# lambdaclass/mina_bridge

Measured on AMD Instinct MI355X. Metric: Mina state proofs verified/sec (batch), higher is better.
Workload: dtype u32x8-montgomery (255-bit prime fields, integer)

## Files before the change

### bindings/go/minaverify.go

```go
package minaverify

import "C"

import (
	"errors"
	"unsafe"
)

type Ctx struct{ p *C.mina_ctx }

func lastError() error { return errors.New(C.GoString(C.mina_last_error())) }

func New(device int) (*Ctx, error) {
	var p *C.mina_ctx
	if rc := C.mina_ctx_create(C.int(device), &p); rc != 0 {
		return nil, lastError()
	}
	return &Ctx{p}, nil
}

func (c *Ctx) Close() { C.mina_ctx_destroy(c.p) }

func (c *Ctx) SrsCreate(curve int, depth uint32) error {
	if rc := C.mina_srs_create(c.p, C.int(curve), C.uint32_t(depth)); rc != 0 {
		return lastError()
	}
	return nil
}

func (c *Ctx) SetStateDedup(on bool) error {
	v := C.int(0)
	if on {
		v = 1
	}
	if rc := C.mina_ctx_set_state_dedup(c.p, v); rc != 0 {
		return lastError()
	}
	return nil
}

func (c *Ctx) StateDedupStats() (states, distinct, collisions uint64, err error) {
	var a, b, d C.uint64_t
	if rc := C.mina_ctx_state_dedup_stats(c.p, &a, &b, &d); rc != 0 {
		return 0, 0, 0, lastError()
	}
	return uint64(a), uint64(b), uint64(d), nil
}

func ConfigureDedupStates(otherFlags uint32) { C.mina_verify_configure(C.uint32_t(otherFlags) | C.MINA_VERIFY_DEDUP_STATES) }

func ConfigurePackOnDevice(otherFlags uint32) { C.mina_verify_configure(C.uint32_t(otherFlags) | C.MINA_VERIFY_PACK_ON_DEVICE) }

func ConfigureAccountOnDevice(otherFlags uint32) { C.mina_verify_configure(C.uint32_t(otherFlags) | C.MINA_VERIFY_ACCOUNT_ON_DEVICE) }

func ConfigureGroupedSearch(otherFlags uint32) { C.mina_verify_configure(C.uint32_t(otherFlags) | C.MINA_VERIFY_GROUPED_SEARCH) }

func (c *Ctx) SetSearchGroups(groups uint32) error {
	if rc := C.mina_ctx_set_search_groups(c.p, C.uint32_t(groups)); rc != 0 {
		return lastError()
	}
	return nil
}

func (c *Ctx) SearchStats() (searches, rounds, parts uint64, err error) {
	var a, b, d C.uint64_t
	if rc := C.mina_ctx_search_stats(c.p, &a, &b, &d); rc != 0 {
		return 0, 0, 0, lastError()
	}
	return uint64(a), uint64(b), uint64(d), nil
}

func (c *Ctx) StateJobEachDev(jobs *C.mina_state_jobs, dVerdicts, dFlags unsafe.Pointer) error {
	if rc := C.mina_state_job_each_dev(c.p, jobs, dVerdicts, dFlags); rc != 0 {
		return lastError()
	}
	return nil
}

func (c *Ctx) MsmSegmentsDev(curve int, nTotal, nseg int, dBegin, dEnd, dBases, dScalars, dOut unsafe.Pointer) error {
	if rc := C.mina_msm_segments_dev(c.p, C.int(curve), C.size_t(nTotal), C.size_t(nseg), dBegin, dEnd, dBases, dScalars, dOut); rc != 0 {
		return lastError()
	}
	return nil
}

func (c *Ctx) BPolyFoldSegmentsDev(field int, k uint32, batch, nseg int, dBegin, dEnd, dChals, dWeights, dOut unsafe.Pointer) error {
	if rc := C.mina_b_poly_fold_segments_dev(c.p, C.int(field), C.uint32_t(k), C.size_t(batch), C.size_t(nseg), dBegin, dEnd, dChals, dWeights, dOut); rc != 0 {
		return lastError()
	}
	return nil
}

func (c *Ctx) SelftestFe29(field, op int, rows []uint32) ([]uint32, error) {
	n := len(rows) / (C.MINA_FE29_IN_OPERANDS*9 + 1)
	out := make([]uint32, n*(C.MINA_FE29_OUT_RESULTS*9+1)+1)
	if n == 0 {
		return out[:0], nil
	}
	if rc := C.mina_selftest_fe29(c.p, C.int(field), C.int(op), C.size_t(n), (*C.uint32_t)(unsafe.Pointer(&rows[0])), (*C.uint32_t)(unsafe.Pointer(&out[0]))); rc != 0 {
		return nil, lastError()
	}
	return out[:len(out)-1], nil
}

func (c *Ctx) SelftestFe32(field, op int, rows []uint32) ([]uint32, error) {
	n := len(rows) / (C.MINA_FE32_IN_OPERANDS*8 + 1)
	out := make([]uint32, n*(C.MINA_FE32_OUT_RESULTS*8+1)+1)
	if n == 0 {
		return out[:0], nil
	}
	if rc := C.mina_selftest_fe32(c.p, C.int(field), C.int(op), C.size_t(n), (*C.uint32_t)(unsafe.Pointer(&rows[0])), (*C.uint32_t)(unsafe.Pointer(&out[0]))); rc != 0 {
		return nil, lastError()
	}
	return out[:len(out)-1], nil
}

func (c *Ctx) AccumulatorCheckMulti(curve int, k uint32, pre, sg []byte) ([]bool, error) {
	n := len(sg) / 64
	out := make([]byte, n)
	rc := C.mina_accumulator_check_multi(c.p, C.int(curve), C.uint32_t(k), C.size_t(n),
		(*C.uint8_t)(unsafe.Pointer(&pre[0])), (*C.uint8_t)(unsafe.Pointer(&sg[0])), (*C.uint8_t)(unsafe.Pointer(&out[0])))
	if rc != 0 {
		return nil, lastError()
	}
	v := make([]bool, n)
	for i := range out {
		v[i] = out[i] != 0
	}
	return v, nil
}

func VerifyMinaState(proof, pub []byte) bool {
	if len(proof) == 0 || len(pub) == 0 {
		return false
	}
	return bool(C.mina_verify_state((*C.uint8_t)(unsafe.Pointer(&proof[0])), C.size_t(len(proof)), (*C.uint8_t)(unsafe.Pointer(&pub[0])), C.size_t(len(pub))))
}

func VerifyAccountInclusionFFI(proof, pub []byte) bool {
	if len(proof) == 0 || len(pub) == 0 {
		return false
	}
	return bool(C.mina_verify_account((*C.uint8_t)(unsafe.Pointer(&proof[0])), C.size_t(len(proof)), (*C.uint8_t)(unsafe.Pointer(&pub[0])), C.size_t(len(pub))))
}

func (c *Ctx) VerifyAccountInclusion(proof, pub, leafHash []byte) (bool, error) {
	var verdict C.uint8_t
	cp, cq := C.CBytes(proof), C.CBytes(pub)
	defer C.free(cp)
	defer C.free(cq)
	p, q := (*C.uint8_t)(cp), (*C.uint8_t)(cq)
	pl, ql := C.size_t(len(proof)), C.size_t(len(pub))
	rc := C.mina_verify_account_inclusion(c.p, 1, &p, &pl, &q, &ql, (*C.uint8_t)(unsafe.Pointer(&leafHash[0])), &verdict)
	if rc != 0 {
		return false, lastError()
	}
	return verdict == 1, nil
}
```

### bindings/rust/src/sys.rs

```rust
#![allow(non_camel_case_types)]
use std::os::raw::{c_char, c_int, c_void};

#[repr(C)] pub struct mina_ctx { _private: [u8; 0] }

#[repr(C)]
pub struct mina_ipa_opening {
    pub k: u32,
    pub lr: *const u8,
    pub delta: *const u8,
    pub sg: *const u8,
    pub z1: *const u8,
    pub z2: *const u8,
    pub n_evalpoints: u32,
    pub evalpoints: *const u8,
    pub n_comms: u32,
    pub comms: *const u8,
    pub combined_inner_product: *const u8,
    pub polyscale: *const u8,
    pub evalscale: *const u8,
    pub sponge_state: *const u8,
    pub sponge_mode: u32,
    pub sponge_count: u32,
}

// ... 125 lines not shown
    pub zk_rows: u32,
    pub n_domains: u32,
    pub domain_log2: *const u32,
    pub shifts: *const u8,
    pub constant_term: *const u8,
    pub constant_term_len: usize,
}

#[repr(C)]
pub struct mina_pickles_statements {
    pub n_old: u32,
    pub n_evals: u32,
    pub plonk: *const c_void,
    pub bulletproof_challenges: *const c_void,
    pub step_old_challenges: *const c_void,
    pub step_comms: *const c_void,
    pub wrap_old_challenges: *const c_void,
    pub wrap_sg: *const c_void,
    pub sponge_digest: *const c_void,
    pub prev_evals: *const c_void,
    pub prev_public_input: *const c_void,
    pub prev_ft_eval1: *const c_void,
    pub app_state: *const c_void,
    pub misc: *const c_void,
}

#[repr(C)]
pub struct mina_verify_tuning {
    pub struct_size: u32,
    pub chunk: u32,
    pub single_max: u32,
    pub slots: u32,
    pub window: u32,
    pub ahead: u32,
    pub early_min: u32,
    pub early_sub: u32,
    pub head_min: u32,
    pub split_max: u32,
    pub chain_cus: u32,
    pub cu_period: u32,
    pub acc_mask: u32,
    pub hash_piece_waves: u32,
    pub up_stream: u32,
    pub min_shard: u32,
    pub pace_us: u32,
    pub merge: u32,
    pub merge_batch_max: u32,
    pub linger_us: u32,
    pub max_jobs: u32,
    pub coop16_max: u32,
    pub coop8_max: u32,
    pub coop8_per_call: u32,
    pub transcript_coop8_max: u32,
    pub ipa_coop8_max: u32,
    pub kimchi_coop8_max: u32,
    pub bpoly_mfma: u32,
    pub pubcomm_direct: u32,
    pub ipa_shared_points: u32,
    pub kimchi_shared_digest: u32,
    pub ipa_side_stream: u32,
    pub search_fan: u32,
    pub search_full: u32,
    pub msm_fp29: u32,
    pub search_ctx: u32,
    pub dev_fork: u32,
    pub dev_chain_cus: u32,
    pub dev_piece_waves: u32,
    pub dev_hash_lds_kb: u32,
    pub dev_acc_lane: u32,
}

extern "C" {
    pub fn mina_ctx_create(device_id: c_int, out: *mut *mut mina_ctx) -> c_int;
    pub fn mina_ctx_destroy(ctx: *mut mina_ctx);
    pub fn mina_last_error() -> *const c_char;
    pub fn mina_ctx_synchronize(ctx: *mut mina_ctx) -> c_int;
    pub fn mina_ctx_stream(ctx: *mut mina_ctx) -> *mut c_void;
    pub fn mina_ctx_pin_lane(ctx: *mut mina_ctx, lane: c_int) -> c_int;
    pub fn mina_ctx_set_pipeline(ctx: *mut mina_ctx, lanes: c_int) -> c_int;
    pub fn mina_dev_malloc(ctx: *mut mina_ctx, bytes: usize, out: *mut *mut c_void) -> c_int;
    pub fn mina_dev_free(ctx: *mut mina_ctx, p: *mut c_void) -> c_int;
    pub fn mina_dev_upload(ctx: *mut mina_ctx, dst: *mut c_void, src: *const c_void, bytes: usize) -> c_int;
    pub fn mina_dev_download(ctx: *mut mina_ctx, dst: *mut c_void, src: *const c_void, bytes: usize) -> c_int;
    pub fn mina_prof_enable(ctx: *mut mina_ctx, stage_mask: c_int) -> c_int;
    pub fn mina_prof_read(ctx: *mut mina_ctx, buf: *mut c_char, cap: usize) -> c_int;
    pub fn mina_srs_create(ctx: *mut mina_ctx, curve: c_int, depth: u32) -> c_int;
    pub fn mina_srs_split_table(ctx: *mut mina_ctx, curve: c_int, on: c_int) -> c_int;
    pub fn mina_srs_load(ctx: *mut mina_ctx, curve: c_int, msgpack: *const u8, len: usize) -> c_int;
    pub fn mina_srs_depth(ctx: *mut mina_ctx, curve: c_int) -> u32;
    pub fn mina_srs_get_g(ctx: *mut mina_ctx, curve: c_int, first: u32, count: u32, out_affine: *mut u8) -> c_int;
    pub fn mina_srs_get_h(ctx: *mut mina_ctx, curve: c_int, out_affine: *mut u8) -> c_int;
    pub fn mina_srs_lagrange_basis(ctx: *mut mina_ctx, curve: c_int, log2_domain: u32, out_affine: *mut u8) -> c_int;
    pub fn mina_public_input_commitment(ctx: *mut mina_ctx, curve: c_int, log2_domain: u32, npub: usize, public_inputs: *const u8, out_affine: *mut u8) -> c_int;
    pub fn mina_public_input_commitment_batch(ctx: *mut mina_ctx, curve: c_int, log2_domain: u32, npub: usize, batch: usize, public_inputs: *const u8, out_affine: *mut u8) -> c_int;
    pub fn mina_srs_serialize(ctx: *mut mina_ctx, curve: c_int, out: *mut u8, cap: usize, len: *mut usize) -> c_int;
    pub fn mina_msm(ctx: *mut mina_ctx, curve: c_int, n: usize, bases_affine: *const u8, scalars: *const u8, out_affine: *mut u8) -> c_int;
    pub fn mina_msm_srs(ctx: *mut mina_ctx, curve: c_int, n: usize, scalars: *const u8, out_affine: *mut u8) -> c_int;
    pub fn mina_msm_srs_range(ctx: *mut mina_ctx, curve: c_int, first: u32, n: usize, scalars: *const u8, out_affine: *mut u8) -> c_int;
    pub fn mina_msm_srs_multi(ctx: *mut mina_ctx, curve: c_int, n: usize, nprob: usize, scalars: *const u8, out_affine: *mut u8) -> c_int;
    pub fn mina_msm_srs_dev(ctx: *mut mina_ctx, curve: c_int, n: usize, d_scalars: *const c_void, d_out: *mut c_void) -> c_int;
    pub fn mina_b_poly(ctx: *mut mina_ctx, field: c_int, k: u32, chals: *const u8, npoints: usize, xs: *const u8, out: *mut u8) -> c_int;
    pub fn mina_b_poly_coefficients(ctx: *mut mina_ctx, field: c_int, k: u32, chals: *const u8, out: *mut u8) -> c_int;
    pub fn mina_b_poly_fold(ctx: *mut mina_ctx, field: c_int, k: u32, batch: usize, chals: *const u8, weights: *const u8, out: *mut u8) -> c_int;
    pub fn mina_b_poly_fold_dev(ctx: *mut mina_ctx, field: c_int, k: u32, batch: usize, d_chals: *const c_void, d_weights: *const c_void, d_out: *mut c_void) -> c_int;
    pub fn mina_poseidon_set_params(ctx: *mut mina_ctx, field: c_int, params: *const u8) -> c_int;
    pub fn mina_poseidon_params_parse(field: c_int, text: *const c_char, len: usize, params_out: *mut u8) -> c_int;
    pub fn mina_poseidon_load_params(ctx: *mut mina_ctx, field: c_int, text: *const c_char, len: usize) -> c_int;
    pub fn mina_poseidon_load_params_file(ctx: *mut mina_ctx, field: c_int, path: *const c_char) -> c_int;
    pub fn mina_poseidon_permute(ctx: *mut mina_ctx, field: c_int, n: usize, states: *mut u8) -> c_int;
    pub fn mina_poseidon_permute_dev(ctx: *mut mina_ctx, field: c_int, n: usize, d_states: *mut c_void) -> c_int;
    pub fn mina_poseidon_hash(ctx: *mut mina_ctx, field: c_int, n: usize, len: usize, inputs: *const u8, out: *mut u8) -> c_int;
    pub fn mina_challenge_to_field(ctx: *mut mina_ctx, field: c_int, n: usize, chal128: *const u8, out: *mut u8) -> c_int;
    pub fn mina_merkle_roots(ctx: *mut mina_ctx, field: c_int, n: usize, depth: u32, leaves: *const u8, siblings: *const u8, dirs: *const u8, roots_out: *mut u8) -> c_int;
    pub fn mina_merkle_verify_batch(ctx: *mut mina_ctx, field: c_int, n: usize, depth: u32, leaves: *const u8, siblings: *const u8, dirs: *const u8, expected_roots: *const u8, verdicts: *mut u8) -> c_int;
    pub fn mina_fq_sponge_run(ctx: *mut mina_ctx, curve: c_int, batch: usize, tape: *const u8, tape_len: usize, init_state: *const u8, init_pos: *const u32, inputs: *const u8, outputs: *mut u8, final_state: *mut u8, final_pos: *mut u32) -> c_int;
    pub fn mina_to_group(ctx: *mut mina_ctx, curve: c_int, n: usize, t: *const u8, out_affine: *mut u8) -> c_int;
    pub fn mina_field_mul(ctx: *mut mina_ctx, field: c_int, n: usize, a: *const u8, b: *const u8, out: *mut u8) -> c_int;
    pub fn mina_field_inv(ctx: *mut mina_ctx, field: c_int, n: usize, a: *const u8, out: *mut u8) -> c_int;
    pub fn mina_field_sqrt(ctx: *mut mina_ctx, field: c_int, n: usize, a: *const u8, out: *mut u8, out_is_square: *mut u8) -> c_int;
    pub fn mina_selftest_group_law(ctx: *mut mina_ctx, curve: c_int, n: usize, p_affine: *const u8, q_affine: *const u8, out_serial: *mut u8, out_quad: *mut u8, same: *mut u8) -> c_int;
    pub fn mina_selftest_fe29(ctx: *mut mina_ctx, field: c_int, op: c_int, n: usize, rows_in: *const u32, rows_out: *mut u32) -> c_int;
    pub fn mina_selftest_fe32(ctx: *mut mina_ctx, field: c_int, op: c_int, n: usize, rows_in: *const u32, rows_out: *mut u32) -> c_int;
    pub fn mina_accumulator_check_batch(ctx: *mut mina_ctx, curve: c_int, k: u32, batch: usize, prechallenges: *const u8, sg: *const u8, rho: *const u8, verdicts: *mut u8) -> c_int;
    pub fn mina_accumulator_check_dev(ctx: *mut mina_ctx, curve: c_int, k: u32, batch: usize, d_prechallenges: *const c_void, d_sg: *const c_void, d_rho: *const c_void, d_verdict: *mut c_void) -> c_int;
    pub fn mina_accumulator_check_multi_dev(ctx: *mut mina_ctx, curve: c_int, k: u32, count: usize, d_prechallenges: *const c_void, d_sg: *const c_void, d_verdicts: *mut c_void) -> c_int;
    pub fn mina_accumulator_check_multi(ctx: *mut mina_ctx, curve: c_int, k: u32, count: usize, prechallenges: *const u8, sg: *const u8, verdicts: *mut u8) -> c_int;
    pub fn mina_combined_inner_product(field: c_int, n_polys: usize, n_points: usize, evals: *const u8, polyscale: *const u8, evalscale: *const u8, out: *mut u8) -> c_int;
    pub fn mina_ipa_batch_check(ctx: *mut mina_ctx, curve: c_int, batch: usize, openings: *const mina_ipa_opening, rand_base: *const u8, sg_rand_base: *const u8, verdict: *mut u8) -> c_int;
    pub fn mina_parse_state_pub_inputs(bytes: *const u8, len: usize, out: *mut mina_state_pub_inputs) -> c_int;
    pub fn mina_parse_account_pub_inputs(bytes: *const u8, len: usize, ledger_hash: *mut u8, encoded_offset: *mut usize, encoded_len: *mut usize) -> c_int;
    pub fn mina_parse_merkle_path(proof: *const u8, len: usize, max_depth: u32, siblings: *mut u8, dirs: *mut u8, depth: *mut u32, account_offset: *mut usize) -> c_int;
    pub fn mina_verify_account_inclusion(ctx: *mut mina_ctx, n: usize, proofs: *const *const u8, proof_lens: *const usize, pub_inputs: *const *const u8, pub_lens: *const usize, leaf_hashes: *const u8, verdicts: *mut u8) -> c_int;
    pub fn mina_consensus_project_window(p: *const mina_consensus_params, s: *const mina_consensus_state, next_global_slot: u32, out_window: *mut u32) -> c_int;
    pub fn mina_consensus_relative_min_window_density(p: *const mina_consensus_params, a: *const mina_consensus_state, b: *const mina_consensus_state, out: *mut u32) -> c_int;
    pub fn mina_consensus_is_short_range(a: *const mina_consensus_state, b: *const mina_consensus_state) -> c_int;
    pub fn mina_consensus_select_secure_chain(p: *const mina_consensus_params, tip: *const mina_consensus_state, candidate: *const mina_consensus_state, candidate_selected: *mut c_int) -> c_int;
    pub fn mina_protocol_state_pack(bytes: *const u8, len: usize, encoding: c_int, record: *mut u8, n_body_fields: *mut u32, info: *mut mina_protocol_state_info, consumed: *mut usize) -> c_int;
    pub fn mina_protocol_state_hash_batch(ctx: *mut mina_ctx, n: usize, records: *const u8, n_body_fields: *const u32, hashes_out: *mut u8, body_hashes_out: *mut u8) -> c_int;
    pub fn mina_protocol_state_dedup_dev(ctx: *mut mina_ctx, n: usize, d_records: *const c_void, d_nfields: *const c_void, d_rep: *mut c_void, d_counts: *mut c_void, fingerprint_bits: u32) -> c_int;
    pub fn mina_protocol_state_hash_batch_dedup(ctx: *mut mina_ctx, n: usize, records: *const u8, n_body_fields: *const u32, hashes_out: *mut u8, body_hashes_out: *mut u8, n_distinct: *mut usize) -> c_int;
    pub fn mina_ctx_set_state_dedup(ctx: *mut mina_ctx, on: c_int) -> c_int;
    pub fn mina_ctx_state_dedup_stats(ctx: *mut mina_ctx, states: *mut u64, distinct: *mut u64, collisions: *mut u64) -> c_int;
    pub fn mina_protocol_state_pack_dev(ctx: *mut mina_ctx, n: usize, d_blob: *const c_void, blob_len: usize, d_off: *const c_void, d_len: *const c_void, d_records: *mut c_void, d_nfields: *mut c_void, d_info: *mut c_void, d_status: *mut c_void) -> c_int;
    pub fn mina_state_frontend_dev(ctx: *mut mina_ctx, batch: usize, d_blob: *const c_void, blob_len: usize, d_begin: *const c_void, d_end: *const c_void, d_expected_hashes: *const c_void, d_ledger_hashes: *const c_void, d_and: *const c_void, d_records: *mut c_void, d_nfields: *mut c_void, d_precheck: *mut c_void, d_masks: *mut c_void) -> c_int;
    pub fn mina_protocol_state_hash_bytes(ctx: *mut mina_ctx, encoding: c_int, n: usize, states: *const *const u8, lens: *const usize, hashes_out: *mut u8) -> c_int;
    pub fn mina_state_jobs_prepare(ctx: *mut mina_ctx, log2_domain: u32, npub: u32) -> c_int;
    pub fn mina_state_job_batch_dev(ctx: *mut mina_ctx, jobs: *const mina_state_jobs, d_verdicts: *mut c_void, d_flags: *mut c_void) -> c_int;
    pub fn mina_state_job_fold_dev(ctx: *mut mina_ctx, jobs: *const mina_state_jobs, d_verdicts: *mut c_void, d_flags: *mut c_void, d_ipa_scalars: *mut c_void, d_ipa_point: *mut c_void, d_acc_scalars: *mut c_void, d_acc_point: *mut c_void) -> c_int;
    pub fn mina_state_job_batch(ctx: *mut mina_ctx, jobs: *const mina_state_jobs, verdicts: *mut u8) -> c_int;
    pub fn mina_state_job_each_dev(ctx: *mut mina_ctx, jobs: *const mina_state_jobs, d_verdicts: *mut c_void, d_flags: *mut c_void) -> c_int;
    pub fn mina_ctx_set_search_groups(ctx: *mut mina_ctx, groups: u32) -> c_int;
    pub fn mina_ctx_search_stats(ctx: *mut mina_ctx, searches: *mut u64, rounds: *mut u64, parts: *mut u64) -> c_int;
    pub fn mina_ctx_lane_streams(ctx: *mut mina_ctx, live: *mut u32, made_by_searches: *mut u64) -> c_int;
    pub fn mina_challenge_to_field_dev(ctx: *mut mina_ctx, field: c_int, n: usize, d_chal128: *const c_void, d_out: *mut c_void) -> c_int;
    pub fn mina_field_sum_rows_dev(ctx: *mut mina_ctx, field: c_int, rows: usize, m: usize, d_in: *const c_void, d_out: *mut c_void) -> c_int;
    pub fn mina_msm_srs_range_dev(ctx: *mut mina_ctx, curve: c_int, first: u32, n: usize, d_scalars: *const c_void, d_out: *mut c_void) -> c_int;
    pub fn mina_msm_dev(ctx: *mut mina_ctx, curve: c_int, n: usize, d_bases: *const c_void, d_scalars: *const c_void, d_out: *mut c_void) -> c_int;
    pub fn mina_points_sum_dev(ctx: *mut mina_ctx, curve: c_int, n: usize, d_records: *const c_void, d_out: *mut c_void) -> c_int;
    pub fn mina_point_records_equal_dev(ctx: *mut mina_ctx, d_a: *const c_void, d_b: *const c_void, d_verdict: *mut c_void) -> c_int;
    pub fn mina_msm_segments_dev(ctx: *mut mina_ctx, curve: c_int, n_total: usize, nseg: usize, d_seg_begin: *const c_void, d_seg_end: *const c_void, d_bases: *const c_void, d_scalars: *const c_void, d_out: *mut c_void) -> c_int;
    pub fn mina_b_poly_fold_segments_dev(ctx: *mut mina_ctx, field: c_int, k: u32, batch: usize, nseg: usize, d_seg_begin: *const c_void, d_seg_end: *const c_void, d_chals: *const c_void, d_weights: *const c_void, d_out: *mut c_void) -> c_int;
    pub fn mina_verifier_index_install(ctx: *mut mina_ctx, index: *const mina_verifier_index) -> c_int;
    pub fn mina_verifier_index_digest(ctx: *mut mina_ctx, out32: *mut u8) -> c_int;
    pub fn mina_polish_tokens_from_json(field: c_int, json: *const c_char, len: usize, enabled_features: u32, optional_present: u32, out: *mut u8, cap: usize, out_len: *mut usize) -> c_int;
    pub fn mina_verifier_index_load_json(ctx: *mut mina_ctx, index_json: *const c_char, index_len: usize, constant_term_json: *const c_char, ct_len: usize, perm_alpha_offset: u32) -> c_int;
    pub fn mina_kimchi_to_batch(ctx: *mut mina_ctx, proofs: *const mina_kimchi_proofs, out: *mut mina_kimchi_batch_out) -> c_int;
    pub fn mina_step_index_install(ctx: *mut mina_ctx, index: *const mina_step_index) -> c_int;
    pub fn mina_step_index_load_json(ctx: *mut mina_ctx, n_indexes: usize, index_jsons: *const *const c_char, index_lens: *const usize, constant_term_json: *const c_char, ct_len: usize, enabled_features: u32, optional_present: u32) -> c_int;
    pub fn mina_pickles_public_inputs_batch(ctx: *mut mina_ctx, st: *const mina_pickles_statements, batch: usize, public_inputs_out: *mut u8, ok: *mut u8) -> c_int;
    pub fn mina_pickles_public_input(ctx: *mut mina_ctx, wrap_proof: *const u8, len: usize, encoding: c_int, app_state: *const u8, public_input_out: *mut u8, derived_out: *mut u8) -> c_int;
    pub fn mina_wrap_proof_flatten(bytes: *const u8, len: usize, encoding: c_int, out: *mut u8, cap: usize, out_len: *mut usize, consumed: *mut usize) -> c_int;
    pub fn mina_state_proof_split(bytes: *const u8, len: usize, proof_len: *mut usize, state_offsets: *mut usize, state_lens: *mut usize) -> c_int;
    pub fn mina_verify_state(proof: *const u8, proof_len: usize, pub_input: *const u8, pub_len: usize) -> bool;
    pub fn mina_verify_state_batch(n: usize, proofs: *const *const u8, proof_lens: *const usize, pub_inputs: *const *const u8, pub_lens: *const usize, verdicts_out: *mut u8) -> c_int;
    pub fn mina_verify_state_checks(proof: *const u8, proof_len: usize, pub_input: *const u8, pub_len: usize, passed_mask: *mut u32, ran_mask: *mut u32) -> c_int;
    pub fn mina_verify_state_files(proof_path: *const c_char, pub_path: *const c_char) -> bool;
    pub fn mina_verify_account(proof: *const u8, proof_len: usize, pub_input: *const u8, pub_len: usize) -> bool;
    pub fn mina_verify_account_batch(n: usize, proofs: *const *const u8, proof_lens: *const usize, pub_inputs: *const *const u8, pub_lens: *const usize, verdicts_out: *mut u8) -> c_int;
    pub fn mina_verify_account_files(proof_path: *const c_char, pub_path: *const c_char) -> bool;
    pub fn verify_mina_state_ffi(proof_buffer: *const u8, proof_len: usize, pub_input_buffer: *const u8, pub_input_len: usize) -> bool;
    pub fn verify_account_inclusion_ffi(proof_buffer: *const u8, proof_len: usize, pub_input_buffer: *const u8, pub_input_len: usize) -> bool;
    pub fn verify_mina_state_ffi_u32(proof_buffer: *const u8, proof_len: u32, pub_input_buffer: *const u8, pub_input_len: u32) -> bool;
    pub fn verify_account_inclusion_ffi_u32(proof_buffer: *const u8, proof_len: u32, pub_input_buffer: *const u8, pub_input_len: u32) -> bool;
    pub fn mina_verify_account_checks(proof: *const u8, proof_len: usize, pub_input: *const u8, pub_len: usize, passed_mask: *mut u32, ran_mask: *mut u32) -> c_int;
    pub fn mina_verify_account_ctx(ctx: *mut mina_ctx, n: usize, proofs: *const *const u8, proof_lens: *const usize, pub_inputs: *const *const u8, pub_lens: *const usize, passed_masks: *mut u32, ran_masks: *mut u32) -> c_int;
    pub fn mina_account_hash_batch(ctx: *mut mina_ctx, encoding: c_int, n: usize, accounts: *const *const u8, lens: *const usize, hashes_out: *mut u8) -> c_int;
    pub fn mina_account_abi_encode(account: *const u8, len: usize, encoding: c_int, out: *mut u8, cap: usize, out_len: *mut usize) -> c_int;
    pub fn mina_account_frontend_dev(ctx: *mut mina_ctx, n: usize, d_blob: *const c_void, blob_len: usize, d_proof_off: *const c_void, d_proof_len: *const c_void, d_pub_off: *const c_void, d_pub_len: *const c_void, d_records: *mut c_void, d_nfields: *mut c_void, d_salt_idx: *mut c_void, d_siblings: *mut c_void, d_dirs: *mut c_void, d_depths: *mut c_void, d_ledger_hashes: *mut c_void, d_zk_marks: *mut c_void, d_zk_index: *mut c_void, d_zk_count: *mut c_void, d_bits: *mut c_void) -> c_int;
    pub fn mina_account_job_dev(ctx: *mut mina_ctx, n: usize, d_blob: *const c_void, blob_len: usize, d_proof_off: *const c_void, d_proof_len: *const c_void, d_pub_off: *const c_void, d_pub_len: *const c_void, d_passed: *mut c_void, d_ran: *mut c_void, d_account_hashes: *mut c_void, d_roots: *mut c_void) -> c_int;
    pub fn mina_verify_configure(flags: u32) -> c_int;
    pub fn mina_verify_tuning_default(out: *mut mina_verify_tuning);
    pub fn mina_verify_tuning_get(out: *mut mina_verify_tuning) -> c_int;
    pub fn mina_verify_configure_ex(tuning: *const mina_verify_tuning) -> c_int;
    pub fn mina_verify_retired_env() -> c_int;
    pub fn mina_verify_shutdown() -> c_int;
    pub fn mina_verify_global_ctx() -> *mut mina_ctx;
    pub fn mina_verify_set_network(devnet: c_int) -> c_int;
    pub fn mina_verify_device_count() -> c_int;
    pub fn mina_verify_device_ctx(i: c_int) -> *mut mina_ctx;
    pub fn mina_verify_install_verifier_index(index: *const mina_verifier_index) -> c_int;
    pub fn mina_verify_install_step_index(index: *const mina_step_index) -> c_int;
    pub fn mina_verify_set_poseidon_params(field: c_int, params: *const u8) -> c_int;
    pub fn mina_poseidon_params_name() -> *const c_char;
    pub fn mina_poseidon_install_default_params(ctx: *mut mina_ctx) -> c_int;
}
```

### include/mina_verify.h

```cpp
#ifndef MINA_VERIFY_H
#define MINA_VERIFY_H

#include <stddef.h>
#include <stdint.h>

#ifdef __cplusplus
extern "C" {
#endif

#define MINA_OK 0
#define MINA_ERR_ARG (-1)
#define MINA_ERR_HIP (-2)
#define MINA_ERR_STATE (-3)
#define MINA_ERR_FORMAT (-4)

#define MINA_FIELD_FP 0
#define MINA_FIELD_FQ 1
#define MINA_CURVE_PALLAS 0
#define MINA_CURVE_VESTA 1

typedef struct mina_ctx mina_ctx;

int mina_ctx_create(int device_id, mina_ctx **out);
void mina_ctx_destroy(mina_ctx *ctx);
// ... 129 lines not shown
#define MINA_FE32_MUL 5
#define MINA_FE32_SQR 6
#define MINA_FE32_DOT2 7
#define MINA_FE32_DOT3 8
#define MINA_FE32_TO_MONT 9
#define MINA_FE32_FROM_MONT 10
#define MINA_FE32_INV 11
#define MINA_FE32_SQRT 12
#define MINA_FE32_WORDS_CANONICAL 13
#define MINA_FE32_DBL_AFFINE 32
#define MINA_FE32_XYZZ_DBL 33
#define MINA_FE32_ADD_AFFINE 34
#define MINA_FE32_XYZZ_ADD 35
#define MINA_FE32_XYZZ_DBL_QUAD 36
#define MINA_FE32_XYZZ_ADD_QUAD 37
int mina_selftest_fe32(mina_ctx *ctx, int field, int op, size_t n, const uint32_t *rows_in , uint32_t *rows_out );

int mina_accumulator_check_batch(mina_ctx *ctx, int curve, uint32_t k, size_t batch,
                                 const uint8_t *prechallenges , const uint8_t *sg ,
                                 const uint8_t *rho , uint8_t *verdicts );

int mina_accumulator_check_dev(mina_ctx *ctx, int curve, uint32_t k, size_t batch, const void *d_prechallenges,
                               const void *d_sg, const void *d_rho, void *d_verdict);

int mina_accumulator_check_multi_dev(mina_ctx *ctx, int curve, uint32_t k, size_t count, const void *d_prechallenges,
                                     const void *d_sg, void *d_verdicts);
int mina_accumulator_check_multi(mina_ctx *ctx, int curve, uint32_t k, size_t count, const uint8_t *prechallenges ,
                                 const uint8_t *sg , uint8_t *verdicts );

typedef struct {
    uint32_t k;
    const uint8_t *lr;
    const uint8_t *delta;
    const uint8_t *sg;
    const uint8_t *z1, *z2;
    uint32_t n_evalpoints;
    const uint8_t *evalpoints;
    uint32_t n_comms;
    const uint8_t *comms;
    const uint8_t *combined_inner_product;
    const uint8_t *polyscale;
    const uint8_t *evalscale;
    const uint8_t *sponge_state;
    uint32_t sponge_mode;
    uint32_t sponge_count;
} mina_ipa_opening;

int mina_combined_inner_product(int field, size_t n_polys, size_t n_points, const uint8_t *evals ,
                                const uint8_t *polyscale, const uint8_t *evalscale, uint8_t *out );

int mina_ipa_batch_check(mina_ctx *ctx, int curve, size_t batch, const mina_ipa_opening *openings,
                         const uint8_t *rand_base , const uint8_t *sg_rand_base ,
                         uint8_t *verdict );

typedef struct {
    uint8_t is_state_proof_from_devnet;
    uint8_t bridge_tip_state_hash[32];
    uint8_t candidate_chain_state_hashes[16][32];
    uint8_t candidate_chain_ledger_hashes[16][32];
} mina_state_pub_inputs;
int mina_parse_state_pub_inputs(const uint8_t *bytes, size_t len, mina_state_pub_inputs *out);
int mina_parse_account_pub_inputs(const uint8_t *bytes, size_t len, uint8_t *ledger_hash , size_t *encoded_offset,
                                  size_t *encoded_len);
int mina_parse_merkle_path(const uint8_t *proof, size_t len, uint32_t max_depth, uint8_t *siblings ,
                           uint8_t *dirs , uint32_t *depth, size_t *account_offset);
int mina_verify_account_inclusion(mina_ctx *ctx, size_t n, const uint8_t *const *proofs, const size_t *proof_lens,
                                  const uint8_t *const *pub_inputs, const size_t *pub_lens, const uint8_t *leaf_hashes ,
                                  uint8_t *verdicts );

#define MINA_MAX_SUB_WINDOWS 16
typedef struct {
    uint32_t slots_per_sub_window;
    uint32_t sub_windows_per_window;
} mina_consensus_params;
typedef struct {
    uint32_t blockchain_length;
    uint32_t epoch_count;
    uint32_t curr_global_slot;
    uint32_t min_window_density;
    uint32_t sub_window_densities[MINA_MAX_SUB_WINDOWS];
    uint8_t staking_lock_checkpoint[32];
    uint8_t next_lock_checkpoint[32];
    uint8_t last_vrf_output_hash[32];
    uint8_t state_hash[32];
} mina_consensus_state;
int mina_consensus_project_window(const mina_consensus_params *p, const mina_consensus_state *s, uint32_t next_global_slot,
                                  uint32_t *out_window );
int mina_consensus_relative_min_window_density(const mina_consensus_params *p, const mina_consensus_state *a,
                                               const mina_consensus_state *b, uint32_t *out);
int mina_consensus_is_short_range(const mina_consensus_state *a, const mina_consensus_state *b);
int mina_consensus_select_secure_chain(const mina_consensus_params *p, const mina_consensus_state *tip,
                                       const mina_consensus_state *candidate, int *candidate_selected);

#define MINA_PSTATE_SLOTS 64
#define MINA_STATES_PER_PROOF 17
#define MINA_ENC_BINPROT 0
#define MINA_ENC_BINCODE 1
typedef struct {
    uint8_t previous_state_hash[32];
    uint8_t genesis_state_hash[32];
    uint8_t snarked_ledger_hash[32];
    uint32_t n_body_fields;
    uint32_t k, slots_per_epoch, slots_per_sub_window, sub_windows_per_window, grace_period_slots, delta;
    mina_consensus_state consensus;
} mina_protocol_state_info;
int mina_protocol_state_pack(const uint8_t *bytes, size_t len, int encoding, uint8_t *record ,
                             uint32_t *n_body_fields, mina_protocol_state_info *info , size_t *consumed);
int mina_protocol_state_hash_batch(mina_ctx *ctx, size_t n, const uint8_t *records ,
                                   const uint32_t *n_body_fields , uint8_t *hashes_out , uint8_t *body_hashes_out );
int mina_protocol_state_dedup_dev(mina_ctx *ctx, size_t n, const void *d_records, const void *d_nfields, void *d_rep, void *d_counts, uint32_t fingerprint_bits);
int mina_protocol_state_hash_batch_dedup(mina_ctx *ctx, size_t n, const uint8_t *records , const uint32_t *n_body_fields ,
                                         uint8_t *hashes_out , uint8_t *body_hashes_out , size_t *n_distinct);
int mina_ctx_set_state_dedup(mina_ctx *ctx, int on);
int mina_ctx_state_dedup_stats(mina_ctx *ctx, uint64_t *states, uint64_t *distinct, uint64_t *collisions);
int mina_protocol_state_pack_dev(mina_ctx *ctx, size_t n, const void *d_blob, size_t blob_len, const void *d_off , const void *d_len ,
                                 void *d_records, void *d_nfields, void *d_info , void *d_status );
int mina_state_frontend_dev(mina_ctx *ctx, size_t batch, const void *d_blob, size_t blob_len,
                            const void *d_begin, const void *d_end ,
                            const void *d_expected_hashes ,
                            const void *d_ledger_hashes , const void *d_and ,
                            void *d_records, void *d_nfields, void *d_precheck , void *d_masks );
int mina_protocol_state_hash_bytes(mina_ctx *ctx, int encoding, size_t n, const uint8_t *const *states, const size_t *lens,
                                   uint8_t *hashes_out );

struct mina_kimchi_proofs;
typedef struct {
    size_t batch;
    int with_states;
    const void *state_records;
    const void *state_nfields;
    const void *expected_hashes;
    const void *precheck;
    uint32_t log2_domain, npub, pub_comm_slot;
    const void *public_inputs;
    int with_ipa;
    uint32_t k, n_evalpoints, n_comms;
    const void *sponge_state , *sponge_pos , *cip , *lr , *delta ,
               *sg , *z1, *z2 , *evalpoints , *evalscale, *polyscale , *comms ;
    const void *rand_base, *sg_rand_base;
    const struct mina_kimchi_proofs *kimchi;
    int with_accumulator;
    uint32_t acc_k;
    const void *acc_prechallenges , *acc_sg , *acc_rho ;
} mina_state_jobs;
int mina_state_jobs_prepare(mina_ctx *ctx, uint32_t log2_domain, uint32_t npub);
int mina_state_job_batch_dev(mina_ctx *ctx, const mina_state_jobs *jobs, void *d_verdicts, void *d_flags);
int mina_state_job_fold_dev(mina_ctx *ctx, const mina_state_jobs *jobs, void *d_verdicts, void *d_flags, void *d_ipa_scalars, void *d_ipa_point,
                            void *d_acc_scalars, void *d_acc_point);
int mina_state_job_batch(mina_ctx *ctx, const mina_state_jobs *jobs, uint8_t *verdicts );
int mina_state_job_each_dev(mina_ctx *ctx, const mina_state_jobs *jobs, void *d_verdicts , void *d_flags );
int mina_ctx_set_search_groups(mina_ctx *ctx, uint32_t groups);
int mina_ctx_search_stats(mina_ctx *ctx, uint64_t *searches, uint64_t *rounds, uint64_t *parts);
int mina_ctx_lane_streams(mina_ctx *ctx, uint32_t *live, uint64_t *made_by_searches);

int mina_challenge_to_field_dev(mina_ctx *ctx, int field, size_t n, const void *d_chal128 , void *d_out );
int mina_field_sum_rows_dev(mina_ctx *ctx, int field, size_t rows, size_t m, const void *d_in , void *d_out );
int mina_msm_srs_range_dev(mina_ctx *ctx, int curve, uint32_t first, size_t n, const void *d_scalars, void *d_out );
int mina_msm_dev(mina_ctx *ctx, int curve, size_t n, const void *d_bases , const void *d_scalars , void *d_out );
int mina_points_sum_dev(mina_ctx *ctx, int curve, size_t n, const void *d_records , void *d_out );
int mina_point_records_equal_dev(mina_ctx *ctx, const void *d_a, const void *d_b, void *d_verdict );
int mina_msm_segments_dev(mina_ctx *ctx, int curve, size_t n_total, size_t nseg, const void *d_seg_begin, const void *d_seg_end ,
                          const void *d_bases , const void *d_scalars , void *d_out );
int mina_b_poly_fold_segments_dev(mina_ctx *ctx, int field, uint32_t k, size_t batch, size_t nseg, const void *d_seg_begin,
                                  const void *d_seg_end , const void *d_chals ,
                                  const void *d_weights , void *d_out );

struct mina_pickles_statements;
#define MINA_TOK_ALPHA 0
#define MINA_TOK_BETA 1
#define MINA_TOK_GAMMA 2
#define MINA_TOK_JOINT_COMBINER 3
#define MINA_TOK_ENDO_COEFFICIENT 4
#define MINA_TOK_MDS 5
#define MINA_TOK_LITERAL 6
#define MINA_TOK_CELL 7
#define MINA_TOK_DUP 8
#define MINA_TOK_POW 9
#define MINA_TOK_ADD 10
#define MINA_TOK_MUL 11
#define MINA_TOK_SUB 12
#define MINA_TOK_VANISHES_ON_ZK_ROWS 13
#define MINA_TOK_UNNORMALIZED_LAGRANGE 14
#define MINA_TOK_STORE 15
#define MINA_TOK_LOAD 16
#define MINA_TOK_SKIP_IF 17
#define MINA_TOK_SKIP_IF_NOT 18
typedef struct {
    uint32_t log2_domain;
    uint32_t zk_rows;
    uint32_t perm_alpha_offset;
    const uint8_t *shifts;
    const uint8_t *sigma_comm;
    const uint8_t *coefficients_comm;
    const uint8_t *selector_comm;
    const uint8_t *constant_term;
    size_t constant_term_len;
} mina_verifier_index;
int mina_verifier_index_install(mina_ctx *ctx, const mina_verifier_index *index);
int mina_verifier_index_digest(mina_ctx *ctx, uint8_t *out32);
#define MINA_FEATURES_RUNTIME 0xffffffffu
int mina_polish_tokens_from_json(int field, const char *json, size_t len, uint32_t enabled_features, uint32_t optional_present, uint8_t *out,
                                 size_t cap, size_t *out_len);
int mina_verifier_index_load_json(mina_ctx *ctx, const char *index_json, size_t index_len, const char *constant_term_json, size_t ct_len,
                                  uint32_t perm_alpha_offset );
typedef struct mina_kimchi_proofs {
    size_t batch;
    uint32_t n_prev, npub;
    const void *public_inputs;
    const void *prev_chals;
    const void *prev_comms;
    const void *w_comm , *z_comm , *t_comm ;
    const void *evals;
    const void *ft_eval1;
    const struct mina_pickles_statements *statements;
    const void *prev_prechallenges;
} mina_kimchi_proofs;
typedef struct {
    uint8_t *sponge_state ; uint32_t *sponge_pos ; uint8_t *cip , *evalpoints ,
            *polyscale , *evalscale , *comms , *ft_eval0 ;
    uint8_t *malformed;
} mina_kimchi_batch_out;
int mina_kimchi_to_batch(mina_ctx *ctx, const mina_kimchi_proofs *proofs, mina_kimchi_batch_out *out);

typedef struct {
    uint32_t zk_rows;
    uint32_t n_domains;
    const uint32_t *domain_log2;
    const uint8_t *shifts;
    const uint8_t *constant_term;
    size_t constant_term_len;
} mina_step_index;
int mina_step_index_install(mina_ctx *ctx, const mina_step_index *index);
int mina_step_index_load_json(mina_ctx *ctx, size_t n_indexes, const char *const *index_jsons, const size_t *index_lens, const char *constant_term_json,
                              size_t ct_len, uint32_t enabled_features, uint32_t optional_present);
typedef struct mina_pickles_statements {
    uint32_t n_old;
    uint32_t n_evals;
    const void *plonk;
    const void *bulletproof_challenges;
    const void *step_old_challenges;
    const void *step_comms;
    const void *wrap_old_challenges;
    const void *wrap_sg;
    const void *sponge_digest;
    const void *prev_evals;
    const void *prev_public_input;
    const void *prev_ft_eval1;
    const void *app_state;
    const void *misc;
} mina_pickles_statements;
int mina_pickles_public_inputs_batch(mina_ctx *ctx, const mina_pickles_statements *st, size_t batch, uint8_t *public_inputs_out ,
                                     uint8_t *ok );
int mina_pickles_public_input(mina_ctx *ctx, const uint8_t *wrap_proof, size_t len, int encoding, const uint8_t *app_state ,
                              uint8_t *public_input_out, uint8_t *derived_out);

int mina_wrap_proof_flatten(const uint8_t *bytes, size_t len, int encoding, uint8_t *out, size_t cap, size_t *out_len, size_t *consumed );
int mina_state_proof_split(const uint8_t *bytes, size_t len, size_t *proof_len, size_t *state_offsets , size_t *state_lens );

#define MINA_CHECK_FORMAT 1u
#define MINA_CHECK_LEDGER 2u
#define MINA_CHECK_CHAIN 4u
#define MINA_CHECK_CONSENSUS 8u
#define MINA_CHECK_ACCUMULATOR 16u
#define MINA_CHECK_KIMCHI 32u
#define MINA_CHECK_ACCOUNT_ABI 64u
#define MINA_CHECK_MERKLE 128u
#define MINA_VERIFY_ALLOW_MISSING_KIMCHI 1u
#define MINA_VERIFY_ALLOW_UNBOUND_STATEMENT 2u
#define MINA_VERIFY_ALLOW_SURROGATE 4u
#define MINA_VERIFY_DEDUP_STATES 8u
#define MINA_VERIFY_PACK_ON_DEVICE 16u
#define MINA_VERIFY_ACCOUNT_ON_DEVICE 32u
#define MINA_VERIFY_GROUPED_SEARCH 64u
#include <stdbool.h>
bool mina_verify_state(const uint8_t *proof, size_t proof_len, const uint8_t *pub_input, size_t pub_len);
int mina_verify_state_batch(size_t n, const uint8_t *const *proofs, const size_t *proof_lens, const uint8_t *const *pub_inputs,
                            const size_t *pub_lens, uint8_t *verdicts_out );
int mina_verify_state_checks(const uint8_t *proof, size_t proof_len, const uint8_t *pub_input, size_t pub_len, uint32_t *passed_mask, uint32_t *ran_mask);
bool mina_verify_state_files(const char *proof_path, const char *pub_path);
bool mina_verify_account(const uint8_t *proof, size_t proof_len, const uint8_t *pub_input, size_t pub_len);
int mina_verify_account_batch(size_t n, const uint8_t *const *proofs, const size_t *proof_lens, const uint8_t *const *pub_inputs,
                              const size_t *pub_lens, uint8_t *verdicts_out);
bool mina_verify_account_files(const char *proof_path, const char *pub_path);
#define MINA_FFI_MAX_PROOF_SIZE (48u * 1024u)
#define MINA_FFI_MAX_PUB_INPUT_SIZE (6u * 1024u)
bool verify_mina_state_ffi(const uint8_t *proof_buffer, size_t proof_len, const uint8_t *pub_input_buffer, size_t pub_input_len);
bool verify_account_inclusion_ffi(const uint8_t *proof_buffer, size_t proof_len, const uint8_t *pub_input_buffer, size_t pub_input_len);
bool verify_mina_state_ffi_u32(const uint8_t *proof_buffer, uint32_t proof_len, const uint8_t *pub_input_buffer, uint32_t pub_input_len);
bool verify_account_inclusion_ffi_u32(const uint8_t *proof_buffer, uint32_t proof_len, const uint8_t *pub_input_buffer, uint32_t pub_input_len);
int mina_verify_account_checks(const uint8_t *proof, size_t proof_len, const uint8_t *pub_input, size_t pub_len, uint32_t *passed_mask, uint32_t *ran_mask);
int mina_verify_account_ctx(mina_ctx *ctx, size_t n, const uint8_t *const *proofs, const size_t *proof_lens, const uint8_t *const *pub_inputs,
                            const size_t *pub_lens, uint32_t *passed_masks, uint32_t *ran_masks);
int mina_account_hash_batch(mina_ctx *ctx, int encoding, size_t n, const uint8_t *const *accounts, const size_t *lens, uint8_t *hashes_out );
int mina_account_abi_encode(const uint8_t *account, size_t len, int encoding, uint8_t *out, size_t cap, size_t *out_len);
int mina_account_frontend_dev(mina_ctx *ctx, size_t n, const void *d_blob, size_t blob_len, const void *d_proof_off, const void *d_proof_len, const void *d_pub_off,
                              const void *d_pub_len, void *d_records, void *d_nfields, void *d_salt_idx ,
                              void *d_siblings , void *d_dirs , void *d_depths , void *d_ledger_hashes ,
                              void *d_zk_marks , void *d_zk_index , void *d_zk_count , void *d_bits );
int mina_account_job_dev(mina_ctx *ctx, size_t n, const void *d_blob, size_t blob_len, const void *d_proof_off, const void *d_proof_len, const void *d_pub_off,
                         const void *d_pub_len, void *d_passed , void *d_ran , void *d_account_hashes, void *d_roots);
int mina_verify_configure(uint32_t flags);
typedef struct mina_verify_tuning {
    uint32_t struct_size;
    uint32_t chunk;
    uint32_t single_max;
    uint32_t slots;
// ... 58 lines not shown
```

### mina_bridge_amd/csrc/api_core.hip

```cpp
#include "ctx.h"
#include "sponge.cuh"
#include "msm.cuh"

#include <sys/random.h>
#include <atomic>
#include <condition_variable>
#include <deque>
#include <mutex>

template <int F> static fe_t host_modulus() { fe_t p; for (int i = 0; i < 8; ++i) p.v[i] = modulus_limb<F>(i); return p; }
static void fe_shr1(fe_t &a) { for (int i = 0; i < 7; ++i) a.v[i] = (a.v[i] >> 1) | (a.v[i + 1] << 31); a.v[7] >>= 1; }
static fe_t fe_sub_small(const fe_t &a, uint32_t k) { fe_t r = a; uint64_t br = k; for (int i = 0; i < 8 && br; ++i) { uint64_t t = (uint64_t)r.v[i] - br; r.v[i] = (uint32_t)t; br = (t >> 32) & 1u; } return r; }
static fe_t fe_div3(const fe_t &a) { fe_t r; uint64_t rem = 0; for (int i = 7; i >= 0; --i) { uint64_t cur = (rem << 32) | a.v[i]; r.v[i] = (uint32_t)(cur / 3); rem = cur % 3; } return r; }

template <int F> static FieldK make_field_consts() {
    FieldK k;
    fe_t p = host_modulus<F>();
    fe_t a = fe_zero(); a.v[0] = 1;
    for (int i = 0; i < 512; ++i) { a = fe_add<F>(a, a); if (i == 255) k.one = a; }
    k.r2 = a;
    fe_t pm1 = fe_sub_small(p, 1);
    k.pm2 = fe_sub_small(p, 2);
    k.pm1d2 = pm1; fe_shr1(k.pm1d2);
    k.half = k.pm1d2;
    fe_t t = pm1; for (int i = 0; i < 32; ++i) fe_shr1(t);
    k.tm1d2 = fe_sub_small(t, 1); fe_shr1(k.tm1d2);
    fe_t five = fe_zero(); five.v[0] = 5; k.five = fe_to_mont<F>(five, k.r2);
    k.root = fe_pow<F>(k.five, t, k.one);
    fe_t three = fe_zero(); three.v[0] = 3; three = fe_to_mont<F>(three, k.r2);
    fe_t six = fe_zero(); six.v[0] = 6; k.bw_fu = fe_to_mont<F>(six, k.r2);
    fe_t two = fe_dbl<F>(k.one);
    fe_sqrt<F>(k.bw_s, fe_neg<F>(three), k);
    k.bw_c = fe_mul<F>(fe_sub<F>(k.bw_s, k.one), fe_inv<F>(two, k));
    k.bw_inv3 = fe_inv<F>(three, k);
    fe_t w = fe_pow<F>(k.five, fe_div3(pm1), k.one);
    k.endo = fe_sqr<F>(w);
    k.inv2 = fe_inv<F>(two, k);
    k.two255 = k.one; for (int i = 0; i < 255; ++i) k.two255 = fe_dbl<F>(k.two255);
    { fe_t t = fe_zero(); t.v[0] = 32; k.m32 = fe_to_mont<F>(t, k.r2); }
    return k;
}


extern "C" int mina_ctx_create(int device_id, mina_ctx **out) {
    if (!out) return fail(MINA_ERR_ARG, "out is null");
    *out = nullptr;
    int ndev = 0;
    HIPC(hipGetDeviceCount(&ndev));
    if (ndev <= 0) return fail(MINA_ERR_HIP, "no HIP device: libminaverify has no CPU fallback");
    if (device_id < 0 || device_id >= ndev) return fail(MINA_ERR_ARG, "bad device id");
    HIPC(hipSetDevice(device_id));
    mina_ctx *c = new mina_ctx();
    c->device = device_id;
    hipError_t e = hipStreamCreateWithFlags(&c->lanes[0].stream, hipStreamNonBlocking);
    if (e != hipSuccess) { delete c; return fail(MINA_ERR_HIP, "hipStreamCreate failed"); }
    c->use_lane0();
    c->fk[FIELD_FP] = make_field_consts<FIELD_FP>();
    c->fk[FIELD_FQ] = make_field_consts<FIELD_FQ>();
    c->state_frontend = mb_state_frontend_on_lane;
    c->account_on_device = mb_verify_account_dev_on;
    c->state_job_each = mb_state_job_each_host;
    *out = c;
    return MINA_OK;
}

int mb_ctx_create_view(mina_ctx *parent, mina_ctx **out) {
    if (!parent || !out) return fail(MINA_ERR_ARG, "null argument");
    int rc = mina_ctx_create(parent->device, out);
    if (rc) return rc;
    (*out)->is_view = true;
    mb_ctx_refresh_view(*out, parent);
    return MINA_OK;
}
void mb_ctx_refresh_view(mina_ctx *v, mina_ctx *p) {
    for (int i = 0; i < 2; ++i) {
        v->fk[i] = p->fk[i];
        SrsState &a = v->srs[i]; const SrsState &b = p->srs[i];
        a.depth = b.depth; a.c = b.c; a.W = b.W;
        a.table.alias(b.table); a.table29.alias(b.table29); a.table29s.alias(b.table29s); a.h.alias(b.h);
        if (a.srs_gen != b.srs_gen || a.lagrange_log2 != b.lagrange_log2 || (a.lagrange_host.empty() && !b.lagrange_host.empty())) { a.lagrange_host = b.lagrange_host; a.lagrange_log2 = b.lagrange_log2; a.srs_gen = b.srs_gen; }
        a.lagrange_table.alias(b.lagrange_table); a.lagrange_table_n = b.lagrange_table_n; a.lagrange_table_log2 = b.lagrange_table_log2;
        a.lagrange_digits.alias(b.lagrange_digits); a.lagrange_digits29.alias(b.lagrange_digits29); a.lagrange_digits_n = b.lagrange_digits_n;
        v->pparams[i].alias(p->pparams[i]); v->have_pparams[i] = p->have_pparams[i]; v->pparams_surrogate[i] = p->pparams_surrogate[i]; v->pparams_rows1[i] = p->pparams_rows1[i];
        v->merkle_salts[i].alias(p->merkle_salts[i]); v->merkle_depth[i] = p->merkle_depth[i];
    }
    v->kimchi_index.alias(p->kimchi_index); v->kimchi_tokens.alias(p->kimchi_tokens); v->kimchi_literals.alias(p->kimchi_literals);
    v->have_kimchi = p->have_kimchi; v->kimchi_log2 = p->kimchi_log2; memcpy(v->kimchi_digest, p->kimchi_digest, sizeof v->kimchi_digest); memcpy(v->kimchi_comms_host, p->kimchi_comms_host, sizeof v->kimchi_comms_host);
    v->pickles_index.alias(p->pickles_index); v->pickles_tokens.alias(p->pickles_tokens); v->pickles_literals.alias(p->pickles_literals);
    v->have_pickles_dev = p->have_pickles_dev; v->pickles_ms_valid = p->pickles_ms_valid;
    if (v->step_host && v->step_host_free && v->step_host != p->step_host) v->step_host_free(v->step_host);
    v->step_host = p->step_host; v->step_host_free = nullptr;
    v->state_salts.alias(p->state_salts); v->have_state_salts = p->have_state_salts;
}

extern "C" void mina_ctx_destroy(mina_ctx *c) {
    if (!c) return;
    (void)hipSetDevice(c->device);
    for (int i = 0; i < MB_MAX_LANES; ++i) if (c->lanes[i].stream) (void)hipStreamSynchronize(c->lanes[i].stream);
    for (int i = 0; i < 2; ++i) { c->srs[i].table.release(); c->srs[i].table29.release(); c->srs[i].table29s.release(); c->srs[i].h.release(); c->srs[i].lagrange_table.release(); c->srs[i].lagrange_digits.release(); c->srs[i].lagrange_digits29.release(); c->pparams[i].release(); c->merkle_salts[i].release(); }
    c->state_salts.release(); c->acct_defaults.release(); c->dedup_totals.release(); c->kimchi_index.release(); c->kimchi_tokens.release(); c->kimchi_literals.release();
    c->pickles_index.release(); c->pickles_tokens.release(); c->pickles_literals.release();
    if (c->step_host && c->step_host_free) c->step_host_free(c->step_host);
    c->step_host = nullptr;
    for (int i = 0; i < MB_MAX_LANES; ++i) c->lanes[i].release_all();
    for (auto &r : c->prof.recs) { (void)hipEventDestroy(r.a); (void)hipEventDestroy(r.b); }
    for (int i = 0; i < MB_MAX_LANES; ++i) {
        Lane &L = c->lanes[i];
        if (L.aux) { (void)hipStreamSynchronize(L.aux); (void)hipStreamDestroy(L.aux); (void)hipEventDestroy(L.ev_fork); (void)hipEventDestroy(L.ev_join); }
        if (L.ev_leg) (void)hipEventDestroy(L.ev_leg);
        if (L.stream) (void)hipStreamDestroy(L.stream);
    }
    delete c;
}

__attribute__((constructor)) static void mb_default_hw_queues() { setenv("GPU_MAX_HW_QUEUES", "16", 0); }

extern "C" int mina_ctx_synchronize(mina_ctx *c) {
    if (!c) return fail(MINA_ERR_ARG, "null ctx");
    HIPC(hipSetDevice(c->device));
    for (int i = 0; i < c->nlanes; ++i) HIPC(hipStreamSynchronize(c->lanes[i].stream));
    return MINA_OK;
}
extern "C" void *mina_ctx_stream(mina_ctx *c) { return c ? (void *)c->lanes[c->pinned >= 0 ? c->pinned : 0].stream : nullptr; }
extern "C" int mina_ctx_pin_lane(mina_ctx *c, int lane) {
    if (!c) return fail(MINA_ERR_ARG, "null ctx");
    if (lane >= c->nlanes) return fail(MINA_ERR_ARG, "lane outside the pipeline (mina_ctx_set_pipeline)");
    c->pinned = lane < 0 ? -1 : lane;
    return MINA_OK;
}

extern "C" int mina_ctx_set_pipeline(mina_ctx *c, int lanes) {
    if (!c) return fail(MINA_ERR_ARG, "null ctx");
    if (lanes < 1 || lanes > MB_PIPE_LANES) return fail(MINA_ERR_ARG, "lanes must be in 1..32");
    HIPC(hipSetDevice(c->device));
    for (int i = 0; i < c->nlanes; ++i) HIPC(hipStreamSynchronize(c->lanes[i].stream));
    for (int i = 0; i < lanes; ++i)
        if (!c->lanes[i].stream) HIPC(hipStreamCreateWithFlags(&c->lanes[i].stream, hipStreamNonBlocking));
    c->nlanes = lanes; c->rr = 0; c->pinned = -1; c->use_lane0();
    return MINA_OK;
}

extern "C" int mina_to_group(mina_ctx *c, int curve, size_t n, const uint8_t *t, uint8_t *out) {
    if (!c || (n && (!t || !out))) return fail(MINA_ERR_ARG, "null argument");
    if (curve != 0 && curve != 1) return fail(MINA_ERR_ARG, "bad curve");
    if (n == 0) return MINA_OK;
    HIPC(hipSetDevice(c->device));
    c->use_lane0();
    int rc;
    if ((rc = h2d(c, c->L->tmp_a, t, n * 32))) return rc;
    if ((rc = c->L->tmp_b.ensure(n * 64))) return rc;
    const int F = base_field_of(curve);
    DISPATCH_FIELD(F, { to_group_kernel<F_><<<cdiv(n, 128), 128, 0, c->L->stream>>>((uint32_t)n, c->fk[F_], c->L->tmp_a.as<uint32_t>(), c->L->tmp_b.as<uint32_t>()); });
    return d2h_sync(c, out, c->L->tmp_b, n * 64);
}

extern "C" int mina_field_mul(mina_ctx *c, int field, size_t n, const uint8_t *a, const uint8_t *b, uint8_t *out) {
    if (!c || (n && (!a || !b || !out))) return fail(MINA_ERR_ARG, "null argument");
    if (bad_field(field)) return fail(MINA_ERR_ARG, "bad field");
    if (n == 0) return MINA_OK;
    HIPC(hipSetDevice(c->device));
    c->use_lane0();
    int rc;
    if ((rc = h2d(c, c->L->tmp_a, a, n * 32))) return rc;
    if ((rc = h2d(c, c->L->tmp_b, b, n * 32))) return rc;
    if ((rc = c->L->tmp_c.ensure(n * 32))) return rc;
    DISPATCH_FIELD(field, { field_mul_kernel<F_><<<cdiv(n, 256), 256, 0, c->L->stream>>>((uint32_t)n, c->fk[F_], c->L->tmp_a.as<uint32_t>(), c->L->tmp_b.as<uint32_t>(), c->L->tmp_c.as<uint32_t>()); });
    return d2h_sync(c, out, c->L->tmp_c, n * 32);
}
extern "C" int mina_field_inv(mina_ctx *c, int field, size_t n, const uint8_t *a, uint8_t *out) {
    if (!c || (n && (!a || !out))) return fail(MINA_ERR_ARG, "null argument");
    if (bad_field(field)) return fail(MINA_ERR_ARG, "bad field");
    if (n == 0) return MINA_OK;
    HIPC(hipSetDevice(c->device));
    c->use_lane0();
    int rc;
    if ((rc = h2d(c, c->L->tmp_a, a, n * 32))) return rc;
    if ((rc = c->L->tmp_c.ensure(n * 32))) return rc;
    DISPATCH_FIELD(field, { field_inv_kernel<F_><<<cdiv(n, 256), 256, 0, c->L->stream>>>((uint32_t)n, c->fk[F_], c->L->tmp_a.as<uint32_t>(), c->L->tmp_c.as<uint32_t>()); });
    return d2h_sync(c, out, c->L->tmp_c, n * 32);
}
extern "C" int mina_field_sqrt(mina_ctx *c, int field, size_t n, const uint8_t *a, uint8_t *out, uint8_t *ok) {
    if (!c || (n && (!a || !out || !ok))) return fail(MINA_ERR_ARG, "null argument");
    if (bad_field(field)) return fail(MINA_ERR_ARG, "bad field");
    if (n == 0) return MINA_OK;
    HIPC(hipSetDevice(c->device));
    c->use_lane0();
    int rc;
    if ((rc = h2d(c, c->L->tmp_a, a, n * 32))) return rc;
    if ((rc = c->L->tmp_c.ensure(n * 32))) return rc;
    if ((rc = c->L->tmp_d.ensure(n))) return rc;
    DISPATCH_FIELD(field, { field_sqrt_kernel<F_><<<cdiv(n, 256), 256, 0, c->L->stream>>>((uint32_t)n, c->fk[F_], c->L->tmp_a.as<uint32_t>(), c->L->tmp_c.as<uint32_t>(), c->L->tmp_d.as<uint8_t>()); });
    HIPC(hipMemcpyAsync(ok, c->L->tmp_d.p, n, hipMemcpyDeviceToHost, c->L->stream));
    return d2h_sync(c, out, c->L->tmp_c, n * 32);
}


static const char *PROF_NAMES[PS_COUNT] = {"msm_digits", "msm_scan", "msm_scatter", "msm_accumulate", "msm_bucket_sum", "msm_segsum",
                                           "msm_reduce2d", "msm_finish", "bpoly_tables", "bpoly_fold", "bpoly_finish", "pstate_hash", "ipa_transcript", "kimchi_to_batch", "pickles_statement",
                                           "pstate_hash1"};
void mb_prof_begin(mina_ctx *c, int stage) {
    ProfState &p = c->prof;
    if (p.used == p.recs.size()) {
        ProfState::Rec r; r.stage = stage;
        if (hipEventCreate(&r.a) != hipSuccess || hipEventCreate(&r.b) != hipSuccess) return;
        p.recs.push_back(r);
    }
    p.recs[p.used].stage = stage;
    (void)hipEventRecord(p.recs[p.used].a, c->L->stream);
}
void mb_prof_end(mina_ctx *c, int stage) {
    ProfState &p = c->prof;
    if (p.used >= p.recs.size() || p.recs[p.used].stage != stage) return;
    (void)hipEventRecord(p.recs[p.used].b, c->L->stream);
    ++p.used;
}
extern "C" int mina_prof_enable(mina_ctx *c, int stage_mask) {
    if (!c) return fail(MINA_ERR_ARG, "null ctx");
    c->prof.mask = stage_mask; c->prof.used = 0;
    return MINA_OK;
}
extern "C" int mina_prof_read(mina_ctx *c, char *buf, size_t cap) {
    if (!c || !buf || cap < 8) return fail(MINA_ERR_ARG, "bad argument");
    HIPC(hipSetDevice(c->device));
    for (int i = 0; i < c->nlanes; ++i) HIPC(hipStreamSynchronize(c->lanes[i].stream));
    double tot[PS_COUNT] = {0}; int cnt[PS_COUNT] = {0};
    for (size_t i = 0; i < c->prof.used; ++i) {
        float ms = 0;
        if (hipEventElapsedTime(&ms, c->prof.recs[i].a, c->prof.recs[i].b) == hipSuccess) { tot[c->prof.recs[i].stage] += ms; cnt[c->prof.recs[i].stage]++; }
    }
    c->prof.used = 0;
    std::string o = "{";
    bool first = true;
    for (int s = 0; s < PS_COUNT; ++s) {
        if (!cnt[s]) continue;
        char tmp[128]; snprintf(tmp, sizeof tmp, "%s\"%s\": [%d, %.6f]", first ? "" : ", ", PROF_NAMES[s], cnt[s], tot[s]);
        o += tmp; first = false;
    }
    o += "}";
    if (o.size() + 1 > cap) return fail(MINA_ERR_ARG, "buffer too small");
    memcpy(buf, o.c_str(), o.size() + 1);
    return MINA_OK;
}

template <int F>
__global__ void __launch_bounds__(256)
group_law_selftest_kernel(uint32_t n, FieldK fk, const uint32_t *__restrict__ pw, const uint32_t *__restrict__ qw,
                          uint32_t *__restrict__ out_serial, uint32_t *__restrict__ out_quad, uint32_t *__restrict__ same) {
    const uint32_t gid = blockIdx.x * blockDim.x + threadIdx.x, i = gid >> 2, rho = gid & 3;
    const bool live = i < n; const uint32_t ii = live ? i : 0;
    auto ld = [&](const uint32_t *w) { affine_t a; for (int k = 0; k < 8; ++k) { a.x.v[k] = w[(size_t)ii * 16 + k]; a.y.v[k] = w[(size_t)ii * 16 + 8 + k]; }
                                       a.x = fe_to_mont<F>(a.x, fk.r2); a.y = fe_to_mont<F>(a.y, fk.r2); return a; };
    const affine_t P = ld(pw), Q = ld(qw);
    const xyzz_t xp = xyzz_from_affine<F>(P, fk.one), xq = xyzz_from_affine<F>(Q, fk.one);
    auto eq = [](const xyzz_t &a, const xyzz_t &b) { return fe_eq(a.x, b.x) && fe_eq(a.y, b.y) && fe_eq(a.zz, b.zz) && fe_eq(a.zzz, b.zzz); };
    xyzz_t s = xp, c = xp; bool ok = true;
    xyzz_add<F>(s, xq);            xyzz_add_quad<F>(c, xq);            ok &= eq(s, c);
    { xyzz_t t = s; xyzz_add<F>(s, t); t = c; xyzz_add_quad<F>(c, t); } ok &= eq(s, c);
    xyzz_add<F>(s, xq);            xyzz_add_quad<F>(c, xq);            ok &= eq(s, c);
    s = xyzz_dbl<F>(s);            c = xyzz_dbl_quad<F>(c);            ok &= eq(s, c);
    { xyzz_t t = s; xyzz_add<F>(t, xp); xyzz_t u = c; xyzz_add_quad<F>(u, xp);
      xyzz_add<F>(s, t); xyzz_add_quad<F>(c, u); } ok &= eq(s, c);
    { xyzz_t t = s; t.y = fe_neg<F>(t.y); xyzz_t z = s; xyzz_add<F>(z, t); xyzz_t u = c; u.y = fe_neg<F>(u.y); xyzz_t z2 = c; xyzz_add_quad<F>(z2, u);
      ok &= xyzz_is_inf(z) && xyzz_is_inf(z2); }
    auto st = [&](const xyzz_t &t, uint32_t *o) {
        if (xyzz_is_inf(t)) { for (int k = 0; k < 16; ++k) o[(size_t)i * 16 + k] = 0; return; }
        fe_t zi = fe_inv<F>(fe_mul<F>(t.zz, t.zzz), fk);
        fe_t x = fe_from_mont<F>(fe_mul<F>(t.x, fe_mul<F>(zi, t.zzz))), y = fe_from_mont<F>(fe_mul<F>(t.y, fe_mul<F>(zi, t.zz)));
        for (int k = 0; k < 8; ++k) { o[(size_t)i * 16 + k] = x.v[k]; o[(size_t)i * 16 + 8 + k] = y.v[k]; } };
    if (live && rho == 0) { st(s, out_serial); st(c, out_quad); same[i] = ok ? 1u : 0u; }
}

extern "C" int mina_selftest_group_law(mina_ctx *c, int curve, size_t n, const uint8_t *p, const uint8_t *q, uint8_t *out_serial,
                                       uint8_t *out_quad, uint8_t *same) {
    if (!c || (n && (!p || !q || !out_serial || !out_quad || !same))) return fail(MINA_ERR_ARG, "null argument");
    if (curve != 0 && curve != 1) return fail(MINA_ERR_ARG, "bad curve");
    if (n == 0) return MINA_OK;
    HIPC(hipSetDevice(c->device));
    c->use_lane0();
    int rc;
    if ((rc = h2d(c, c->L->tmp_a, p, n * 64))) return rc;
    if ((rc = h2d(c, c->L->tmp_b, q, n * 64))) return rc;
    if ((rc = c->L->tmp_c.ensure(n * 64))) return rc;
    if ((rc = c->L->tmp_d.ensure(n * 64 + n * 4))) return rc;
    uint32_t *d_quad = c->L->tmp_d.as<uint32_t>(), *d_same = d_quad + n * 16;
    DISPATCH_FIELD(base_field_of(curve), {
        group_law_selftest_kernel<F_><<<cdiv(n * 4, 256), 256, 0, c->L->stream>>>((uint32_t)n, c->fk[F_], c->L->tmp_a.as<uint32_t>(), c->L->tmp_b.as<uint32_t>(),
                                                                              c->L->tmp_c.as<uint32_t>(), d_quad, d_same);
    });
    std::vector<uint32_t> sm(n);
    HIPC(hipMemcpyAsync(out_quad, d_quad, n * 64, hipMemcpyDeviceToHost, c->L->stream));
    HIPC(hipMemcpyAsync(sm.data(), d_same, n * 4, hipMemcpyDeviceToHost, c->L->stream));
    if ((rc = d2h_sync(c, out_serial, c->L->tmp_c, n * 64))) return rc;
    for (size_t i = 0; i < n; ++i) same[i] = sm[i] ? 1 : 0;
    return MINA_OK;
}

extern "C" int mina_dev_malloc(mina_ctx *c, size_t bytes, void **out) {
    if (!c || !out) return fail(MINA_ERR_ARG, "null argument");
    *out = nullptr;
    HIPC(hipSetDevice(c->device));
    if (hipMalloc(out, bytes ? bytes : 4) != hipSuccess) return fail(MINA_ERR_HIP, "hipMalloc failed");
    return MINA_OK;
}
extern "C" int mina_dev_free(mina_ctx *c, void *p) {
    if (!c) return fail(MINA_ERR_ARG, "null argument");
    HIPC(hipSetDevice(c->device));
    if (p) HIPC(hipFree(p));
    return MINA_OK;
}
extern "C" int mina_dev_upload(mina_ctx *c, void *dst, const void *src, size_t bytes) {
    if (!c || (bytes && (!dst || !src))) return fail(MINA_ERR_ARG, "null argument");
    HIPC(hipSetDevice(c->device));
    if (bytes) HIPC(hipMemcpy(dst, src, bytes, hipMemcpyHostToDevice));
    return MINA_OK;
}
extern "C" int mina_dev_download(mina_ctx *c, void *dst, const void *src, size_t bytes) {
    if (!c || (bytes && (!dst || !src))) return fail(MINA_ERR_ARG, "null argument");
    int rc = mina_ctx_synchronize(c);
    if (rc) return rc;
    if (bytes) HIPC(hipMemcpy(dst, src, bytes, hipMemcpyDeviceToHost));
    return MINA_OK;
}
```

### mina_bridge_amd/csrc/api_srs.hip

```cpp
#include <atomic>
#include "ctx.h"
#include "msm.cuh"
#include "lagrange.cuh"
#include <type_traits>
#include <vector>

template <int F> static int build_tables(mina_ctx *c, SrsState &s) {
    const FieldK &fk = c->fk[F];
    msm_build_table_kernel<F><<<cdiv(s.depth, 256), 256, 0, c->L->stream>>>(s.depth, s.depth, s.c, s.W, fk.one, fk.pm2, s.table.as<affine_t>());
    HIPC(hipGetLastError());
    const size_t npts = (size_t)s.W * s.depth;
    msm_table29_kernel<F><<<cdiv(npts, 256), 256, 0, c->L->stream>>>(npts, s.table.as<affine_t>(), fk.m32, s.table29.as<affine_t>());
    HIPC(hipGetLastError());
    HIPC(hipStreamSynchronize(c->L->stream));
    s.table29s.release();
    return MINA_OK;
}
extern "C" int mina_srs_split_table(mina_ctx *c, int curve, int on) {
    if (!c) return fail(MINA_ERR_ARG, "null ctx");
    if (curve != 0 && curve != 1) return fail(MINA_ERR_ARG, "bad curve");
    SrsState &s = c->srs[curve];
    if (s.depth == 0) return fail(MINA_ERR_STATE, "SRS not loaded for this curve");
    HIPC(hipSetDevice(c->device));
    for (int i = 0; i < c->nlanes; ++i) HIPC(hipStreamSynchronize(c->lanes[i].stream));
    if (!on) { s.table29s.release(); return MINA_OK; }
    if (s.table29s.p) return MINA_OK;
    c->use_lane0();
    const size_t npts = (size_t)s.W * s.depth;
    int rc;
    if ((rc = s.table29s.ensure(npts * sizeof(tab29_t)))) return rc;
    DISPATCH_FIELD(base_field_of(curve), { msm_table29s_kernel<F_><<<cdiv(npts, 256), 256, 0, c->L->stream>>>(npts, s.table.as<affine_t>(), c->fk[F_].m32, s.table29s.as<tab29_t>()); });
    HIPC(hipGetLastError());
    HIPC(hipStreamSynchronize(c->L->stream));
    return MINA_OK;
}

static int srs_alloc(mina_ctx *c, int curve, uint32_t depth) {
    SrsState &s = c->srs[curve];
    s.depth = 0; s.c = 16; s.W = 16;
    s.lagrange_log2 = -1; s.lagrange_host.clear();
    s.lagrange_table_log2 = -1; s.lagrange_table_n = 0; s.lagrange_digits_n = 0;
    static std::atomic<uint64_t> gen{0};
    s.srs_gen = ++gen;
    int rc;
    if ((rc = s.table.ensure((size_t)s.W * depth * sizeof(affine_t)))) return rc;
    if ((rc = s.table29.ensure((size_t)s.W * depth * sizeof(affine_t)))) return rc;
    if ((rc = s.h.ensure(sizeof(affine_t)))) return rc;
    return MINA_OK;
}

extern "C" int mina_srs_create(mina_ctx *c, int curve, uint32_t depth) {
    if (!c) return fail(MINA_ERR_ARG, "null ctx");
    if (curve != 0 && curve != 1) return fail(MINA_ERR_ARG, "bad curve");
    if (depth == 0 || depth > (1u << 20)) return fail(MINA_ERR_ARG, "depth must be in 1..2^20");
    HIPC(hipSetDevice(c->device));
    c->use_lane0();
    int rc = srs_alloc(c, curve, depth);
    if (rc) return rc;
    SrsState &s = c->srs[curve];
    const int F = base_field_of(curve);
    DISPATCH_FIELD(F, {
        srs_create_kernel<F_><<<cdiv((size_t)depth + 1, 256), 256, 0, c->L->stream>>>(depth, c->fk[F_], s.table.as<affine_t>(), s.h.as<affine_t>());
    });
    HIPC(hipGetLastError());
    s.depth = depth;
    DISPATCH_FIELD(F, { rc = build_tables<F_>(c, s); });
    if (rc) s.depth = 0;
    return rc;
}

extern "C" int mina_srs_load(mina_ctx *c, int curve, const uint8_t *d, size_t len) {
    if (!c || !d) return fail(MINA_ERR_ARG, "null argument");
    if (curve != 0 && curve != 1) return fail(MINA_ERR_ARG, "bad curve");
    if (len < 3 || d[0] != 0x92) return fail(MINA_ERR_FORMAT, "not an SRS MessagePack blob");
    uint32_t n; size_t hdr;
    if ((d[1] & 0xf0) == 0x90) { n = d[1] & 0x0f; hdr = 2; }
    else if (d[1] == 0xdc && len >= 4) { n = ((uint32_t)d[2] << 8) | d[3]; hdr = 4; }
    else if (d[1] == 0xdd && len >= 6) { n = ((uint32_t)d[2] << 24) | ((uint32_t)d[3] << 16) | ((uint32_t)d[4] << 8) | d[5]; hdr = 6; }
    else return fail(MINA_ERR_FORMAT, "not an SRS MessagePack blob");
    if (n == 0 || n > (1u << 20) || len != hdr + (size_t)(n + 1) * 35) return fail(MINA_ERR_FORMAT, "bad SRS length");
    std::vector<uint8_t> blobs((size_t)(n + 1) * 33);
    for (size_t i = 0; i <= n; ++i) {
        const uint8_t *e = d + hdr + i * 35;
        if (e[0] != 0xc4 || e[1] != 33) return fail(MINA_ERR_FORMAT, "bad point header");
        memcpy(&blobs[i * 33], e + 2, 33);
    }
    HIPC(hipSetDevice(c->device));
    c->use_lane0();
    int rc = srs_alloc(c, curve, n);
    if (rc) return rc;
    SrsState &s = c->srs[curve];
    if ((rc = c->L->tmp_a.ensure(blobs.size()))) return rc;
    if ((rc = c->L->tmp_b.ensure(4))) return rc;
    HIPC(hipMemcpyAsync(c->L->tmp_a.p, blobs.data(), blobs.size(), hipMemcpyHostToDevice, c->L->stream));
    HIPC(hipMemsetAsync(c->L->tmp_b.p, 0, 4, c->L->stream));
    const int F = base_field_of(curve);
    DISPATCH_FIELD(F, {
        decompress_kernel<F_><<<cdiv(n, 256), 256, 0, c->L->stream>>>(n, c->fk[F_], c->L->tmp_a.as<uint8_t>(), s.table.as<affine_t>(), c->L->tmp_b.as<uint32_t>());
        decompress_kernel<F_><<<1, 64, 0, c->L->stream>>>(1, c->fk[F_], c->L->tmp_a.as<uint8_t>() + (size_t)n * 33, s.h.as<affine_t>(), c->L->tmp_b.as<uint32_t>());
    });
    uint32_t bad = 0;
    HIPC(hipMemcpyAsync(&bad, c->L->tmp_b.p, 4, hipMemcpyDeviceToHost, c->L->stream));
    HIPC(hipStreamSynchronize(c->L->stream));
    if (bad) return fail(MINA_ERR_FORMAT, "SRS contains a point that is not on the curve");
    s.depth = n;
    DISPATCH_FIELD(F, { rc = build_tables<F_>(c, s); });
    if (rc) s.depth = 0;
    return rc;
}

extern "C" uint32_t mina_srs_depth(mina_ctx *c, int curve) {
    if (!c || (curve != 0 && curve != 1)) return 0;
    return c->srs[curve].depth;
}

extern "C" int mina_srs_get_g(mina_ctx *c, int curve, uint32_t first, uint32_t count, uint8_t *out) {
    if (!c || !out) return fail(MINA_ERR_ARG, "null argument");
    if (curve != 0 && curve != 1) return fail(MINA_ERR_ARG, "bad curve");
    SrsState &s = c->srs[curve];
    if (s.depth == 0) return fail(MINA_ERR_STATE, "SRS not loaded");
    if ((uint64_t)first + count > s.depth) return fail(MINA_ERR_ARG, "range outside SRS");
    if (count == 0) return MINA_OK;
    HIPC(hipSetDevice(c->device));
    c->use_lane0();
    int rc;
    if ((rc = c->L->tmp_a.ensure((size_t)count * 64))) return rc;
    const int F = base_field_of(curve);
    DISPATCH_FIELD(F, { points_from_mont_kernel<F_><<<cdiv(count, 256), 256, 0, c->L->stream>>>(count, s.table.as<affine_t>() + first, c->L->tmp_a.as<uint32_t>()); });
    HIPC(hipMemcpyAsync(out, c->L->tmp_a.p, (size_t)count * 64, hipMemcpyDeviceToHost, c->L->stream));
    HIPC(hipStreamSynchronize(c->L->stream));
    return MINA_OK;
}

extern "C" int mina_srs_get_h(mina_ctx *c, int curve, uint8_t *out) {
    if (!c || !out) return fail(MINA_ERR_ARG, "null argument");
    if (curve != 0 && curve != 1) return fail(MINA_ERR_ARG, "bad curve");
    SrsState &s = c->srs[curve];
    if (s.depth == 0) return fail(MINA_ERR_STATE, "SRS not loaded");
    HIPC(hipSetDevice(c->device));
    c->use_lane0();
    int rc;
    if ((rc = c->L->tmp_a.ensure(64))) return rc;
    const int F = base_field_of(curve);
    DISPATCH_FIELD(F, { points_from_mont_kernel<F_><<<1, 64, 0, c->L->stream>>>(1, s.h.as<affine_t>(), c->L->tmp_a.as<uint32_t>()); });
    HIPC(hipMemcpyAsync(out, c->L->tmp_a.p, 64, hipMemcpyDeviceToHost, c->L->stream));
    HIPC(hipStreamSynchronize(c->L->stream));
    return MINA_OK;
}

extern "C" int mina_srs_serialize(mina_ctx *c, int curve, uint8_t *out, size_t cap, size_t *len) {
    if (!c || !len) return fail(MINA_ERR_ARG, "null argument");
    if (curve != 0 && curve != 1) return fail(MINA_ERR_ARG, "bad curve");
    SrsState &s = c->srs[curve];
    if (s.depth == 0) return fail(MINA_ERR_STATE, "SRS not loaded");
    const size_t hdr = s.depth < 16 ? 2 : (s.depth < 65536 ? 4 : 6);
    const size_t need = hdr + (size_t)(s.depth + 1) * 35;
    *len = need;
    if (!out || cap < need) return fail(MINA_ERR_ARG, "output buffer too small");
    HIPC(hipSetDevice(c->device));
    c->use_lane0();
    int rc;
    if ((rc = c->L->tmp_a.ensure((size_t)(s.depth + 1) * 33))) return rc;
    const int F = base_field_of(curve);
    DISPATCH_FIELD(F, {
        compress_kernel<F_><<<cdiv(s.depth, 256), 256, 0, c->L->stream>>>(s.depth, c->fk[F_], s.table.as<affine_t>(), c->L->tmp_a.as<uint8_t>());
        compress_kernel<F_><<<1, 64, 0, c->L->stream>>>(1, c->fk[F_], s.h.as<affine_t>(), c->L->tmp_a.as<uint8_t>() + (size_t)s.depth * 33);
    });
    std::vector<uint8_t> blobs((size_t)(s.depth + 1) * 33);
    HIPC(hipMemcpyAsync(blobs.data(), c->L->tmp_a.p, blobs.size(), hipMemcpyDeviceToHost, c->L->stream));
    HIPC(hipStreamSynchronize(c->L->stream));
    out[0] = 0x92;
    if (hdr == 2) out[1] = (uint8_t)(0x90 | s.depth);
    else if (hdr == 4) { out[1] = 0xdc; out[2] = (uint8_t)(s.depth >> 8); out[3] = (uint8_t)s.depth; }
    else { out[1] = 0xdd; out[2] = (uint8_t)(s.depth >> 24); out[3] = (uint8_t)(s.depth >> 16); out[4] = (uint8_t)(s.depth >> 8); out[5] = (uint8_t)s.depth; }
    for (size_t i = 0; i <= s.depth; ++i) {
        uint8_t *e = out + hdr + i * 35;
        e[0] = 0xc4; e[1] = 33; memcpy(e + 2, &blobs[i * 33], 33);
// ... 191 lines not shown
```

### mina_bridge_amd/csrc/api_state.hip

```cpp
#include <chrono>
#include <optional>
#include "ctx.h"
#include "msm.cuh"
#include "sponge.cuh"
#include "lagrange.cuh"
#include "wire_state.h"
#include "state_dedup.cuh"

namespace mb {

template <int F> __device__ __forceinline__ fe_t ld_fe(const uint32_t *p) { fe_t r; for (int i = 0; i < 8; ++i) r.v[i] = p[i]; return r; }

template <int F, int LANES>
__device__ __forceinline__ void pstate_sponge(const bool live, const bool writer, const uint32_t e, const uint32_t sp, const uint32_t *__restrict__ rec, const uint32_t nf,
                                              const FieldK &fk, const PoseidonParams *__restrict__ pp, const fe_t *__restrict__ salts, uint32_t *__restrict__ out_hash,
                                              uint32_t *__restrict__ out_body) {
#if defined(__HIP_DEVICE_COMPILE__)
    if constexpr (LANES == 3) {
        const TriPos tp = tri_pos();
        const PoseidonParams29 *__restrict__ q = pparams29_of(pp);
        auto field29 = [&](const uint32_t *w, bool take) {
            fe_t v = fe_zero();
            if (take) v = ld_fe<F>(w);
            return fe29_mul_sg<F>(fe29_from_words(v), q->absorb);
// ... 327 lines not shown
    if ((rc = d2h_sync(c, hashes_out, L.tmp_c, n * 32))) return rc;
    if (n_distinct) *n_distinct = m;
    return MINA_OK;
}
extern "C" int mina_protocol_state_hash_batch_dedup(mina_ctx *c, size_t n, const uint8_t *records, const uint32_t *n_body_fields, uint8_t *hashes_out,
                                                    uint8_t *body_hashes_out, size_t *n_distinct) {
    return pstate_hash_batch(c, n, records, n_body_fields, hashes_out, body_hashes_out, true, n_distinct);
}
extern "C" int mina_protocol_state_hash_batch(mina_ctx *c, size_t n, const uint8_t *records, const uint32_t *n_body_fields, uint8_t *hashes_out,
                                              uint8_t *body_hashes_out) {
    return pstate_hash_batch(c, n, records, n_body_fields, hashes_out, body_hashes_out, false, nullptr);
}

extern "C" int mina_protocol_state_hash_bytes(mina_ctx *c, int encoding, size_t n, const uint8_t *const *states, const size_t *lens, uint8_t *hashes_out) {
    if (!c || (n && (!states || !lens || !hashes_out))) return fail(MINA_ERR_ARG, "null argument");
    std::vector<uint8_t> rec(n * MINA_PSTATE_SLOTS * 32); std::vector<uint32_t> nf(n);
    for (size_t i = 0; i < n; ++i) {
        if (!states[i]) return fail(MINA_ERR_ARG, "null state");
        int rc = mina_protocol_state_pack(states[i], lens[i], encoding, &rec[i * MINA_PSTATE_SLOTS * 32], &nf[i], nullptr, nullptr);
        if (rc) return rc;
    }
    return mina_protocol_state_hash_batch(c, n, rec.data(), nf.data(), hashes_out, nullptr);
}

int mb_pickles_check(mina_ctx *c, const mina_pickles_statements *s);
int mb_pickles_statements_dev(mina_ctx *c, size_t batch, const mina_pickles_statements *s, uint32_t *d_pub, uint32_t *d_ok);
size_t mb_pickles_sections(const mina_pickles_statements *s, const void ***slots, size_t *strides, mina_pickles_statements *copy);
static int check_jobs(mina_ctx *c, const mina_state_jobs *j) {
    if (!c || !j) return fail(MINA_ERR_ARG, "null argument");
    if (j->batch == 0 || j->batch > 65536) return fail(MINA_ERR_ARG, "batch must be in 1..65536");
    if (j->with_states && (!j->state_records || !j->state_nfields || !j->expected_hashes)) return fail(MINA_ERR_ARG, "null protocol-state section");
    if (j->with_ipa) {
        if (!j->lr || !j->delta || !j->sg || !j->z1 || !j->z2 || !j->rand_base || !j->sg_rand_base) return fail(MINA_ERR_ARG, "null IPA section");
        if (j->kimchi) {
            const mina_kimchi_proofs &kp = *j->kimchi;
            if (!c->have_kimchi) return fail(MINA_ERR_STATE, "no verifier index installed");
            if (kp.batch != j->batch || j->k != c->kimchi_log2 || j->log2_domain != c->kimchi_log2 || j->n_evalpoints != 2 || j->n_comms != kp.n_prev + 45 || kp.npub != j->npub || kp.n_prev > 8)
                return fail(MINA_ERR_ARG, "kimchi section does not match the installed index / the job's shape");
            if ((kp.n_prev && ((!kp.prev_chals && !kp.prev_prechallenges && !(kp.statements && kp.n_prev == 2 && j->k == 15)) || !kp.prev_comms)) || !kp.w_comm || !kp.z_comm || !kp.t_comm || !kp.evals || !kp.ft_eval1 || (kp.npub && !kp.public_inputs && !kp.statements)) return fail(MINA_ERR_ARG, "null kimchi section");
            if (kp.statements) { if (kp.npub != 40) return fail(MINA_ERR_ARG, "statements derive exactly 40 public inputs"); int prc = mb_pickles_check(c, kp.statements); if (prc) return prc; }
        } else if (!j->sponge_state || !j->sponge_pos || !j->cip || !j->evalscale || !j->polyscale || (j->n_evalpoints && !j->evalpoints) || (j->n_comms && !j->comms))
            return fail(MINA_ERR_ARG, "null IPA section");
        if (j->k < 1 || j->k > 20 || ((size_t)1 << j->k) > c->srs[CURVE_PALLAS].depth) return fail(c->srs[CURVE_PALLAS].depth ? MINA_ERR_ARG : MINA_ERR_STATE, "Pallas SRS missing or 2^k exceeds its depth");
        if (j->n_comms > 4096 || j->n_evalpoints > 64) return fail(MINA_ERR_ARG, "too many commitments / evaluation points");
        if (!c->have_pparams[FIELD_FP]) return fail(MINA_ERR_STATE, "Poseidon constants not installed for Fp");
    }
    if (j->npub) {
        if (!j->public_inputs && !(j->kimchi && j->kimchi->statements)) return fail(MINA_ERR_ARG, "null public inputs");
        if (!j->with_ipa || (!j->kimchi && j->pub_comm_slot >= j->n_comms)) return fail(MINA_ERR_ARG, "public-input commitment needs an IPA section and a valid commitment slot");
        if (j->log2_domain > 20 || ((uint64_t)1 << j->log2_domain) > c->srs[CURVE_PALLAS].depth || j->npub > 4096 || j->npub > ((uint64_t)1 << j->log2_domain)) return fail(MINA_ERR_ARG, "bad domain / npub");
    }
    if (j->with_accumulator) {
        if (!j->acc_prechallenges || !j->acc_sg || (j->batch > 1 && !j->acc_rho)) return fail(MINA_ERR_ARG, "null accumulator section");
        if (j->acc_k < 1 || j->acc_k > 20 || ((size_t)1 << j->acc_k) > c->srs[CURVE_VESTA].depth) return fail(c->srs[CURVE_VESTA].depth ? MINA_ERR_ARG : MINA_ERR_STATE, "Vesta SRS missing or 2^k exceeds its depth");
    }
    return MINA_OK;
}

int mb_ensure_lagrange_table(mina_ctx *c, int curve, uint32_t log2_domain, uint32_t npub);
int mb_lagrange_sums_dev(mina_ctx *c, int curve, uint32_t npub, size_t batch, const uint32_t *d_scalars, void *d_out_xyzz);
namespace mb {
struct KimchiIn { const uint32_t *pub, *prev_chals, *prev_comms, *w_comm, *z_comm, *t_comm, *evals, *ft_eval1, *pubcomm; };
struct KimchiOut { uint32_t *sponge_state, *sponge_pos, *cip, *evalpoints, *polyscale, *evalscale, *comms, *ft_eval0; };
}
int mb_kimchi_to_batch_dev(mina_ctx *c, size_t batch, uint32_t n_prev, uint32_t npub, const mb::KimchiIn &in, const mb::KimchiOut &out, uint32_t *d_bad, mb::IpaExpand *expand,
                           const void *pf_digest, uint32_t pf_stride);
void mb_pickles_kimchi_digest(mina_ctx *c, const mina_pickles_statements *s, const void **first, uint32_t *stride);

int mb_pubcomm_dev(mina_ctx *c, size_t batch, uint32_t log2_domain, uint32_t npub, const uint32_t *d_pub, uint32_t *d_out16) {
    Lane &L = *c->L;
    SrsState &s = c->srs[CURVE_PALLAS];
    int rc;
    if ((rc = L.st_pub_xyzz.ensure(batch * sizeof(xyzz_t)))) return rc;
    if (npub == 0) {
        HIPC(hipMemsetAsync(L.st_pub_xyzz.p, 0, batch * sizeof(xyzz_t), L.stream));
    } else {
        if (s.lagrange_table_log2 != (int)log2_domain || s.lagrange_table_n < npub) return fail(MINA_ERR_STATE, "call mina_state_jobs_prepare(log2_domain, npub) first");
        if ((rc = mb_lagrange_sums_dev(c, CURVE_PALLAS, npub, batch, d_pub, L.st_pub_xyzz.p))) return rc;
    }
    mb::pubcomm_finish16_kernel<FIELD_FP><<<cdiv(batch, 64), 64, 0, L.stream>>>((uint32_t)batch, c->fk[FIELD_FP], s.h.as<affine_t>(), L.st_pub_xyzz.as<xyzz_t>(), d_out16);
    HIPC(hipGetLastError());
    return MINA_OK;
}

extern "C" int mina_state_jobs_prepare(mina_ctx *c, uint32_t log2_domain, uint32_t npub) {
    if (!c) return fail(MINA_ERR_ARG, "null argument");
    HIPC(hipSetDevice(c->device));
    c->use_lane0();
    int rc;
    if ((rc = ensure_state_salts(c))) return rc;
    if (npub && (rc = mb_ensure_lagrange_table(c, CURVE_PALLAS, log2_domain, npub))) return rc;
    return MINA_OK;
}

static int leg_fork(Lane &from, Lane &to) {
    if (!to.stream) HIPC(hipStreamCreateWithFlags(&to.stream, hipStreamNonBlocking));
    if (!from.ev_leg) HIPC(hipEventCreateWithFlags(&from.ev_leg, hipEventDisableTiming));
    HIPC(hipEventRecord(from.ev_leg, from.stream));
    HIPC(hipStreamWaitEvent(to.stream, from.ev_leg, 0));
    return MINA_OK;
}
static int leg_join(Lane &leg, Lane &into) {
    if (!leg.ev_leg) HIPC(hipEventCreateWithFlags(&leg.ev_leg, hipEventDisableTiming));
    HIPC(hipEventRecord(leg.ev_leg, leg.stream));
    HIPC(hipStreamWaitEvent(into.stream, leg.ev_leg, 0));
    return MINA_OK;
}
int mb_state_hashes_early(mina_ctx *c, Lane *LS, size_t ns_total, size_t lo, size_t cnt, const uint32_t *d_records, const uint32_t *d_nfields, hipEvent_t after, HashLaunch hash) {
    if (!LS || lo + cnt > ns_total) return fail(MINA_ERR_ARG, "bad early state range");
    if (!c->have_state_salts) return fail(MINA_ERR_STATE, "call mina_state_jobs_prepare first");
    if (!LS->stream) HIPC(hipStreamCreateWithFlags(&LS->stream, hipStreamNonBlocking));
    int rc;
    if ((rc = LS->st_hashes.ensure(ns_total * 32))) return rc;
    if (after) HIPC(hipStreamWaitEvent(LS->stream, after, 0));
    Lane *const L0 = c->L;
    c->L = LS;
    rc = pstate_hash_dev(c, cnt, ns_total, hash, d_records + lo * MINA_PSTATE_SLOTS * 8, d_nfields + lo, LS->st_hashes.as<uint32_t>() + lo * 8, nullptr);
    c->L = L0;
    return rc;
}


static int state_leg(mina_ctx *c, const mina_state_jobs *j, Lane &S, const StateJobPlan &plan) {
    c->L = &S;
    const size_t B = j->batch;
    int rc;
    if (j->with_states) {
        const size_t ns = B * MINA_STATES_PER_PROOF;
        if ((rc = S.st_hashes.ensure(ns * 32))) return rc;
        const size_t early = std::min(plan.hashed_early, ns);
        const uint32_t *rec = (const uint32_t *)j->state_records, *nf = (const uint32_t *)j->state_nfields;
        if (c->state_dedup && early == 0) {
            if ((rc = pstate_hash_dedup_dev(c, ns, ns, plan.hash, rec, nf, S.st_hashes.as<uint32_t>(), nullptr, true))) return rc;
        } else if (early < ns && (rc = pstate_hash_dev(c, ns - early, ns, plan.hash, rec + early * MINA_PSTATE_SLOTS * 8, nf + early, S.st_hashes.as<uint32_t>() + early * 8, nullptr))) return rc;
        mb::pstate_chain_check_kernel<<<cdiv(B, 64), 64, 0, S.stream>>>((uint32_t)B, S.st_hashes.as<uint32_t>(), (const uint32_t *)j->expected_hashes, rec, (const uint8_t *)j->precheck, S.st_ok.as<uint32_t>());
    } else {
        if (j->precheck) return fail(MINA_ERR_ARG, "precheck needs the protocol-state section");
        mb::fill_u32_kernel<<<cdiv(B, 256), 256, 0, S.stream>>>((uint32_t)B, 1u, S.st_ok.as<uint32_t>());
    }
    HIPC(hipGetLastError());
    return MINA_OK;
}

static int accumulator_leg(mina_ctx *c, const mina_state_jobs *j, Lane &A, const FoldExport *fx, StateJobCarry &v) {
    c->L = &A;
    if (!j->with_accumulator) return MINA_OK;
    const size_t B = j->batch;
    int rc;
    if ((rc = A.st_flags.ensure(16 * 4))) return rc;
    v.acc_v = A.st_flags.as<uint32_t>() + 8;
    return mb_accumulator_check_dev(c, CURVE_VESTA, j->acc_k, B, (const uint32_t *)j->acc_prechallenges, (const uint32_t *)j->acc_sg, B > 1 ? (const uint32_t *)j->acc_rho : nullptr, v.acc_v, fx);
}

static int wrap_leg(mina_ctx *c, const mina_state_jobs *j, Lane &L, const FoldExport *fx, StateJobCarry &v) {
    c->L = &L;
    const size_t B = j->batch;
    int rc;
    if ((rc = L.st_flags.ensure(16 * 4))) return rc;
    const uint32_t *pub = (const uint32_t *)j->public_inputs, *comm_override = nullptr;
    if (j->kimchi && j->kimchi->statements) {
        if ((rc = L.pk_pub.ensure(B * 40 * 32)) || (rc = L.pk_ok.ensure(B * 4))) return rc;
        if ((rc = mb_pickles_statements_dev(c, B, j->kimchi->statements, L.pk_pub.as<uint32_t>(), L.pk_ok.as<uint32_t>()))) return rc;
        pub = L.pk_pub.as<uint32_t>(); v.stmt_ok = L.pk_ok.as<uint32_t>();
    }
    if (j->npub || j->kimchi) {
        if ((rc = L.st_pubcomm.ensure(B * 64))) return rc;
        if ((rc = mb_pubcomm_dev(c, B, j->log2_domain, j->npub, pub, L.st_pubcomm.as<uint32_t>()))) return rc;
        comm_override = L.st_pubcomm.as<uint32_t>();
    }
    if (!j->with_ipa) return MINA_OK;
    mb::IpaShape sh; sh.batch = (uint32_t)B; sh.k = j->k; sh.npts = j->n_evalpoints; sh.ncomms = j->n_comms; sh.per = 2 * j->k + j->n_comms + 4;
    auto W = [](const void *p) { return (const uint32_t *)p; };
    v.ipa_v = L.st_flags.as<uint32_t>() + 4;
    if (!j->kimchi) {
        sh.override_slot = j->npub ? j->pub_comm_slot : 0xffffffffu;
        mb::IpaDevIn in{W(j->sponge_state), W(j->sponge_pos), W(j->cip), W(j->lr), W(j->delta), W(j->sg), W(j->z1), W(j->z2), W(j->evalpoints), W(j->evalscale),
                        W(j->polyscale), W(j->comms), comm_override, W(j->rand_base), W(j->sg_rand_base)};
        return mb_ipa_batch_check_dev(c, CURVE_PALLAS, sh, in, v.ipa_v, fx);
    }
    const mina_kimchi_proofs &kp = *j->kimchi;
    if ((rc = L.kc_state.ensure(B * 96)) || (rc = L.kc_pos.ensure(B * 8)) || (rc = L.kc_cip.ensure(B * 32)) || (rc = L.kc_pts.ensure(B * 64)) ||
        (rc = L.kc_v.ensure(B * 32)) || (rc = L.kc_u.ensure(B * 32)) || (rc = L.kc_comms.ensure(B * (size_t)j->n_comms * 64))) return rc;
    v.kimchi_bad = L.st_flags.as<uint32_t>() + 12;
    HIPC(hipMemsetAsync(v.kimchi_bad, 0, 4, L.stream));
    const uint32_t *prev_chals = W(kp.prev_chals);
    const bool from_statement = !kp.prev_chals && !kp.prev_prechallenges && kp.statements && kp.n_prev == 2 && j->k == 15;
    const void *pre = from_statement ? kp.statements->wrap_old_challenges : kp.prev_prechallenges;
    const void *pf_digest = nullptr; uint32_t pf_stride = 0;
    if (from_statement && mb_tune().kimchi_shared_digest) mb_pickles_kimchi_digest(c, kp.statements, &pf_digest, &pf_stride);
    if (pre && kp.n_prev) {
        const size_t cnt = B * kp.n_prev * j->k;
        if ((rc = L.kc_pch.ensure(cnt * 32))) return rc;
        challenge_to_field_kernel<FIELD_FQ><<<cdiv(cnt, 64), 64, 0, L.stream>>>((uint32_t)cnt, c->fk[FIELD_FQ], W(pre), L.kc_pch.as<uint32_t>());
        prev_chals = L.kc_pch.as<uint32_t>();
    }
    mb::KimchiIn in{pub, prev_chals, W(kp.prev_comms), W(kp.w_comm), W(kp.z_comm), W(kp.t_comm), W(kp.evals), W(kp.ft_eval1), comm_override};
    mb::KimchiOut out{L.kc_state.as<uint32_t>(), L.kc_pos.as<uint32_t>(), L.kc_cip.as<uint32_t>(), L.kc_pts.as<uint32_t>(), L.kc_v.as<uint32_t>(), L.kc_u.as<uint32_t>(),
                      L.kc_comms.as<uint32_t>(), nullptr};
    mb::IpaExpand ex;
    if ((rc = mb_kimchi_to_batch_dev(c, B, kp.n_prev, kp.npub, in, out, v.kimchi_bad, &ex, pf_digest, pf_stride))) return rc;
    sh.expand_slot = kp.n_prev + 1; sh.per += mb::IPA_EXPAND - 1;
    if (mb_tune().ipa_shared_points && kp.n_prev + 45 <= 64) {
        uint64_t m = 0;
        for (uint32_t i = kp.n_prev + 3; i < kp.n_prev + 9; ++i) m |= (uint64_t)1 << i;
        for (uint32_t i = kp.n_prev + 24; i < kp.n_prev + 45; ++i) m |= (uint64_t)1 << i;
        sh.shared_lo = (uint32_t)m; sh.shared_hi = (uint32_t)(m >> 32); sh.shared_h = 1; sh.shared_expand0 = 1; sh.nshared = 29;
    }
    mb::IpaDevIn iin{out.sponge_state, out.sponge_pos, out.cip, W(j->lr), W(j->delta), W(j->sg), W(j->z1), W(j->z2), out.evalpoints, out.evalscale, out.polyscale,
                     out.comms, nullptr, W(j->rand_base), W(j->sg_rand_base)};
    iin.expand = ex;
    return mb_ipa_batch_check_dev(c, CURVE_PALLAS, sh, iin, v.ipa_v, fx);
}

int mb_state_jobs_on_lane(mina_ctx *c, const mina_state_jobs *j, uint32_t *d_verdicts, uint32_t *d_flags, const StateJobPlan &plan) {
    const uint32_t phase = plan.phase;
    if (phase != MB_JOB_ALL && !plan.carry) return fail(MINA_ERR_ARG, "a split job needs a carry");
    Lane *const L0 = c->L;
    struct Restore { mina_ctx *c; Lane *l0; ~Restore() { c->L = l0; } } restore{c, L0};
    Lane *LI = L0, *LA = L0, *LS = L0;
    int rc;
    if (plan.wrap && plan.acc && plan.wrap != L0 && plan.acc != L0 && plan.wrap != plan.acc) {
        LI = plan.wrap; LA = plan.acc;
        if (plan.states && plan.states != L0 && plan.states != LI) LS = plan.states;
        if ((phase & MB_JOB_LEGS) && ((rc = leg_fork(*L0, *LI)) || (rc = leg_fork(*L0, *LA)))) return rc;
        if ((phase & MB_JOB_FINISH) && LS != L0 && (rc = leg_fork(*L0, *LS))) return rc;
    }
    const size_t B = j->batch;
    StateJobCarry v;
    const bool acc_ahead = plan.acc_first && LA == LS && LS != L0 && phase == MB_JOB_ALL;
    if (acc_ahead && (rc = accumulator_leg(c, j, *LA, plan.fold_export, v))) return rc;
    if ((rc = LS->st_ok.ensure(B * 4))) return rc;
    if ((phase & MB_JOB_FINISH) && (rc = state_leg(c, j, *LS, plan))) return rc;
    if (phase & MB_JOB_LEGS) {
        if (LA == LI && (rc = accumulator_leg(c, j, *LA, plan.fold_export, v))) return rc;
        if ((rc = wrap_leg(c, j, *LI, plan.fold_export, v))) return rc;
        if (LA != LI && !acc_ahead && (rc = accumulator_leg(c, j, *LA, plan.fold_export, v))) return rc;
    }
    if (phase == MB_JOB_LEGS) { *plan.carry = v; return MINA_OK; }
    if (phase == MB_JOB_FINISH) v = *plan.carry;
    if (LI != L0 && ((rc = leg_join(*LI, *L0)) || (rc = leg_join(*LA, *L0)) || (LS != L0 && (rc = leg_join(*LS, *L0))))) return rc;
    mb::state_job_verdict_kernel<<<cdiv(B, 64), 64, 0, L0->stream>>>((uint32_t)B, LS->st_ok.as<uint32_t>(), v.ipa_v, v.acc_v, v.kimchi_bad, v.stmt_ok, d_verdicts, d_flags, plan.d_stmt_out);
    HIPC(hipGetLastError());
    return MINA_OK;
}

static int dev_fork_lanes(mina_ctx *c, size_t leg_states, StateJobPlan &plan) {
    const mina_verify_tuning tu = mb_tune();
    const int li = (int)(c->L - c->lanes);
    if (!(tu.dev_fork & 1u) || c->nlanes > MB_DEV_FORK_MAX || li < 0 || li >= MB_DEV_FORK_MAX) return MINA_OK;
    const int in_flight = c->pinned >= 0 ? 1 : c->nlanes;
    Lane *h = &c->lanes[MB_DEV_HELPER0 + 3 * li];
    if (!h[0].stream || !h[1].stream || !h[2].stream) {
        const uint32_t mode = c->dev_fork_made ? c->dev_fork_made : tu.dev_fork;
        c->dev_fork_made = mode;
        int ncu = 0; (void)hipDeviceGetAttribute(&ncu, hipDeviceAttributeMultiprocessorCount, c->device);
        int prio_lo = 0, prio_hi = 0; (void)hipDeviceGetStreamPriorityRange(&prio_lo, &prio_hi);
        auto make = [&](Lane &ln, bool chain, bool masked, int prio) -> int {
            if (ln.stream) return MINA_OK;
            if (masked && tu.dev_chain_cus > 0 && tu.dev_chain_cus < (uint32_t)ncu && ncu <= 256) {
                uint32_t mk[8] = {0, 0, 0, 0, 0, 0, 0, 0};
                for (uint32_t b2 = 0; b2 < (uint32_t)ncu; ++b2) if ((b2 < tu.dev_chain_cus) == chain) mk[b2 >> 5] |= 1u << (b2 & 31);
                if (hipExtStreamCreateWithCUMask(&ln.stream, 8, mk) == hipSuccess) return MINA_OK;
                (void)hipGetLastError(); ln.stream = nullptr;
            }
            if (prio_lo != prio_hi && (mode & 4u)) HIPC(hipStreamCreateWithPriority(&ln.stream, hipStreamNonBlocking, prio));
            else HIPC(hipStreamCreateWithFlags(&ln.stream, hipStreamNonBlocking));
            return MINA_OK;
        };
        int rc;
        if ((rc = make(h[0], true, (mode & 2u) != 0, prio_hi)) || (rc = make(h[1], true, false, (prio_lo + prio_hi) / 2)) || (rc = make(h[2], false, (mode & 2u) != 0, prio_lo))) return rc;
    }
    plan.wrap = &h[0]; plan.acc = tu.dev_acc_lane ? &h[2] : &h[1]; plan.states = &h[2];
    plan.acc_first = tu.dev_acc_lane == 2;
    uint32_t piece = tu.dev_piece_waves;
    if (piece == 0 && in_flight >= 2) piece = (hash_one_lane(c, leg_states) ? 12288u : 6144u) / (uint32_t)in_flight;
    if (piece == 0xffffffffu) piece = 0;
    plan.hash.piece_waves = piece;
    uint32_t lds_kb = tu.dev_hash_lds_kb;
    if (lds_kb == 0 && in_flight == 1) lds_kb = 41;
    if (lds_kb == 0xffffffffu || lds_kb > 160) lds_kb = 0;
    plan.hash.lds_bytes = lds_kb * 1024u;
    return MINA_OK;
}

extern "C" int mina_state_job_batch_dev(mina_ctx *c, const mina_state_jobs *jobs, void *d_verdicts, void *d_flags) {
    int rc = check_jobs(c, jobs);
    if (rc) return rc;
    if (!d_verdicts) return fail(MINA_ERR_ARG, "null argument");
    if (!c->have_state_salts && jobs->with_states) return fail(MINA_ERR_STATE, "call mina_state_jobs_prepare first");
    HIPC(hipSetDevice(c->device));
    c->next_lane();
    StateJobPlan plan;
    if ((rc = dev_fork_lanes(c, jobs->with_states ? jobs->batch * MINA_STATES_PER_PROOF : 0, plan))) return rc;
    return mb_state_jobs_on_lane(c, jobs, (uint32_t *)d_verdicts, (uint32_t *)d_flags, plan);
}

extern "C" int mina_state_job_fold_dev(mina_ctx *c, const mina_state_jobs *jobs, void *d_verdicts, void *d_flags, void *d_ipa_scalars, void *d_ipa_point,
                                       void *d_acc_scalars, void *d_acc_point) {
    int rc = check_jobs(c, jobs);
    if (rc) return rc;
    if (!d_verdicts || !d_ipa_scalars || !d_ipa_point || !d_acc_scalars || !d_acc_point) return fail(MINA_ERR_ARG, "null argument");
    if (jobs->batch < 2 || !jobs->with_ipa || !jobs->with_accumulator || !jobs->acc_rho) return fail(MINA_ERR_ARG, "the exchange variant needs >= 2 proofs and both folded legs");
    if (!c->have_state_salts && jobs->with_states) return fail(MINA_ERR_STATE, "call mina_state_jobs_prepare first");
    HIPC(hipSetDevice(c->device));
    c->next_lane();
    const FoldExport fe{(uint32_t *)d_ipa_scalars, (uint32_t *)d_ipa_point, (uint32_t *)d_acc_scalars, (uint32_t *)d_acc_point};
    StateJobPlan plan; plan.fold_export = &fe;
    if ((rc = dev_fork_lanes(c, jobs->with_states ? jobs->batch * MINA_STATES_PER_PROOF : 0, plan))) return rc;
    return mb_state_jobs_on_lane(c, jobs, (uint32_t *)d_verdicts, (uint32_t *)d_flags, plan);
}

namespace {
struct Section { const void **slot; size_t bytes; };
}
static int state_job_each(mina_ctx *c, Lane &L, const mina_state_jobs &d, uint8_t *verdicts, uint32_t *flags) {
    c->L = &L;
    const size_t B = d.batch, k = d.k, m = d.n_comms, np = d.n_evalpoints;
    int rc;
    if ((rc = L.st_verdicts.ensure(2 * B * 4 + 16))) return rc;
    uint32_t *dv = L.st_verdicts.as<uint32_t>(), *df = dv + B, *ds = df + 4;
    StateJobPlan plan; plan.d_stmt_out = ds;
    if (B <= 1024 && c->nlanes == 1 && &L == &c->lanes[0]) { plan.wrap = &c->lanes[1]; plan.acc = &c->lanes[2]; }
    if ((rc = mb_state_jobs_on_lane(c, &d, dv, df, plan))) return rc;
    std::vector<uint32_t> hv(2 * B + 4);
    if ((rc = d2h_sync(c, hv.data(), L.st_verdicts, (2 * B + 4) * 4))) return rc;
    if (flags) memcpy(flags, &hv[B], 16);
    std::vector<uint8_t> stmt_each(B); for (size_t b = 0; b < B; ++b) stmt_each[b] = hv[B + 4 + b] ? 1 : 0;
    const bool ipa_ok = hv[B] != 0, acc_ok = hv[B + 2] != 0;
    if (ipa_ok && acc_ok) { for (size_t b = 0; b < B; ++b) verdicts[b] = hv[b] ? 1 : 0; return MINA_OK; }
    std::vector<uint8_t> ipa_each(B, 1), acc_each(B, 1), chain_each(B, 1);
    {
        mina_state_jobs only = d; only.with_ipa = 0; only.with_accumulator = 0; only.npub = 0; only.kimchi = nullptr;
        if (only.with_states) {
            if ((rc = mb_state_jobs_on_lane(c, &only, dv, df))) return rc;
            if ((rc = d2h_sync(c, hv.data(), L.st_verdicts, B * 4))) return rc;
            for (size_t b = 0; b < B; ++b) chain_each[b] = hv[b] ? 1 : 0;
        }
    }
    mina_kimchi_proofs kslice{}; mina_pickles_statements sslice{};
    auto slice = [&](const mina_state_jobs &src, size_t lo, size_t cnt) {
        mina_state_jobs s = src; s.batch = cnt; s.with_states = 0; s.precheck = nullptr;
        auto adv = [&](const void *&p, size_t stride) { if (p) p = (const uint8_t *)p + lo * stride; };
        if (s.kimchi) {
            kslice = *s.kimchi; kslice.batch = cnt; s.kimchi = &kslice;
            adv(kslice.public_inputs, (size_t)kslice.npub * 32); adv(kslice.prev_chals, (size_t)kslice.n_prev * k * 32); adv(kslice.prev_prechallenges, (size_t)kslice.n_prev * k * 16); adv(kslice.prev_comms, (size_t)kslice.n_prev * 64);
            adv(kslice.w_comm, 15 * 64); adv(kslice.z_comm, 64); adv(kslice.t_comm, 7 * 64); adv(kslice.evals, 43 * 64); adv(kslice.ft_eval1, 32);
            if (kslice.statements) {
                const void **slots[12]; size_t strides[12];
                mb_pickles_sections(kslice.statements, slots, strides, &sslice);
                kslice.statements = &sslice;
                for (int i = 0; i < 12; ++i) adv(*slots[i], strides[i]);
            }
        }
        adv(s.public_inputs, (size_t)s.npub * 32);
        adv(s.sponge_state, 96); adv(s.sponge_pos, 8); adv(s.cip, 32); adv(s.lr, 2 * k * 64); adv(s.delta, 64); adv(s.sg, 64); adv(s.z1, 32); adv(s.z2, 32);
        adv(s.evalpoints, np * 32); adv(s.evalscale, 32); adv(s.polyscale, 32); adv(s.comms, m * 64);
        adv(s.acc_prechallenges, (size_t)s.acc_k * 16); adv(s.acc_sg, 64); adv(s.acc_rho, 32);
        return s;
    };
    const bool rows_ok = hv[B + 1] == 0 && c->ipa_rows && c->ipa_rows_batch == B && !mb_tune().search_full;
    auto search = [&](bool ipa_leg, std::vector<uint8_t> &each) -> int {
        const size_t FAN = std::min<size_t>(MB_PIPE_LANES, std::max<size_t>(2, (size_t)mb_tune().search_fan));
        static const bool timing = getenv("MINA_VERIFY_TIMING") != nullptr;
        struct Restore {
            mina_ctx *c; std::vector<size_t> made;
            ~Restore() { for (size_t i : made) if (c->lanes[i].stream) { (void)hipStreamSynchronize(c->lanes[i].stream); (void)hipStreamDestroy(c->lanes[i].stream); c->lanes[i].stream = nullptr; } c->use_lane0(); }
        } restore{c, {}};
        for (size_t i = 0; i < FAN; ++i)
            if (!c->lanes[i].stream) { HIPC(hipStreamCreateWithFlags(&c->lanes[i].stream, hipStreamNonBlocking)); restore.made.push_back(i); ++c->search_streams_made; }
        std::vector<std::pair<size_t, size_t>> failing{{0, B}};
        while (!failing.empty()) {
            std::vector<std::pair<size_t, size_t>> parts;
            for (auto [lo, cnt] : failing) {
                if (cnt == 1) { each[lo] = 0; continue; }
                const size_t np_ = std::min(FAN, cnt);
                for (size_t q = 0; q < np_; ++q) { const size_t a = lo + cnt * q / np_, e = lo + cnt * (q + 1) / np_; parts.push_back({a, e - a}); }
            }
            failing.clear();
            const auto t_round = std::chrono::steady_clock::now();
            for (size_t base = 0; base < parts.size(); base += FAN) {
                const size_t w = std::min(FAN, parts.size() - base);
                uint32_t *flags_at[MB_PIPE_LANES];
                for (size_t q = 0; q < w; ++q) {
                    const auto [lo, cnt] = parts[base + q];
                    c->L = &c->lanes[q];
                    int r = c->L->st_verdicts.ensure(2 * cnt * 4 + 16);
                    if (r) return r;
                    uint32_t *v = c->L->st_verdicts.as<uint32_t>();
                    flags_at[q] = v + cnt;
                    if (ipa_leg && rows_ok) { if ((r = mb_ipa_recheck_rows(c, lo, cnt, flags_at[q]))) return r; continue; }
                    mina_state_jobs sj = slice(d, lo, cnt);
                    if (ipa_leg) sj.with_accumulator = 0; else { sj.with_ipa = 0; sj.npub = 0; sj.kimchi = nullptr; }
                    if ((r = mb_state_jobs_on_lane(c, &sj, v, flags_at[q]))) return r;
                }
                for (size_t q = 0; q < w; ++q) {
                    uint32_t f[4];
                    HIPC(hipStreamSynchronize(c->lanes[q].stream));
                    HIPC(hipMemcpy(f, flags_at[q], 16, hipMemcpyDeviceToHost));
                    if (!(ipa_leg ? f[0] != 0 : f[2] != 0)) failing.push_back(parts[base + q]);
                }
            }
            if (timing) fprintf(stderr, "mina_state_job_batch: culprit search (%s), %zu parts -> %zu failing, %.2f ms\n", ipa_leg ? "opening" : "accumulator", parts.size(), failing.size(),
                                std::chrono::duration<double, std::milli>(std::chrono::steady_clock::now() - t_round).count());
        }
        return MINA_OK;
    };
    auto grouped = [&](bool ipa_leg, std::vector<uint8_t> &each) -> int {
        c->L = &L;
        const size_t G = c->search_groups;
        const int curve = ipa_leg ? CURVE_PALLAS : CURVE_VESTA;
        const size_t cap = mb_search_parts_cap(c, curve, ipa_leg ? d.k : d.acc_k);
        const uint32_t per = ipa_leg ? c->ipa_rows_per : 1;
        int r;
        if (!ipa_leg && (r = mb_accumulator_parts_prepare(c, CURVE_VESTA, d.acc_k, B, (const uint32_t *)d.acc_prechallenges, (const uint32_t *)d.acc_sg))) return r;
        ++c->gs_searches;
        std::vector<std::pair<size_t, size_t>> failing{{0, B}};
        while (!failing.empty()) {
            std::vector<uint32_t> lo, cnt;
            for (auto [l, n] : failing) {
                if (n == 1) { each[l] = 0; continue; }
                const size_t g = std::min(G, n);
                for (size_t q = 0; q < g; ++q) { const size_t a = l + n * q / g, e = l + n * (q + 1) / g; lo.push_back((uint32_t)a); cnt.push_back((uint32_t)(e - a)); }
            }
            failing.clear();
            const size_t nparts = lo.size();
            if (nparts == 0) break;
            ++c->gs_rounds; c->gs_parts += nparts;
            if ((r = L.gs_flags.ensure(nparts * 4)) || (r = L.host_stage.ensure(nparts * 16))) return r;
            uint32_t *fl = L.gs_flags.as<uint32_t>();
            for (size_t base = 0; base < nparts;) {
                size_t w = std::min(cap, nparts - base);
                auto longest = [&](size_t w_) { uint32_t x = 0; for (size_t q = 0; q < w_; ++q) x = std::max(x, cnt[base + q]); return x; };
                while (w > 1 && !mb_msm_segments_fit(longest(w) * per, w)) w = (w + 1) / 2;
                r = ipa_leg ? mb_ipa_recheck_rows_parts(c, w, &lo[base], &cnt[base], fl + base, base * 16)
                            : mb_accumulator_check_parts(c, CURVE_VESTA, d.acc_k, B, (const uint32_t *)d.acc_rho, w, &lo[base], &cnt[base], fl + base, base * 16);
                if (r) return r;
                base += w;
            }
            std::vector<uint32_t> f(nparts);
            if ((r = d2h_sync(c, f.data(), L.gs_flags, nparts * 4))) return r;
            for (size_t p = 0; p < nparts; ++p) if (!f[p]) failing.push_back({lo[p], cnt[p]});
        }
        return MINA_OK;
    };
    const bool in_groups = c->search_groups >= 2 && !mb_tune().search_full;
    if (!ipa_ok) { rc = (in_groups && rows_ok) ? grouped(true, ipa_each) : search(true, ipa_each); c->L = &L; if (rc) return rc; }
    if (!acc_ok) { rc = (in_groups && B > 1 && d.acc_rho) ? grouped(false, acc_each) : search(false, acc_each); c->L = &L; if (rc) return rc; }
    for (size_t b = 0; b < B; ++b) verdicts[b] = (chain_each[b] && ipa_each[b] && acc_each[b] && stmt_each[b]) ? 1 : 0;
    return MINA_OK;
}

extern "C" int mina_state_job_batch(mina_ctx *c, const mina_state_jobs *jobs, uint8_t *verdicts) {
    int rc = check_jobs(c, jobs);
    if (rc) return rc;
    if (!verdicts) return fail(MINA_ERR_ARG, "null argument");
    HIPC(hipSetDevice(c->device));
    c->use_lane0();
    if ((rc = mina_state_jobs_prepare(c, jobs->log2_domain, jobs->npub))) return rc;
    c->use_lane0();
    Lane &L = *c->L;
    mina_state_jobs d = *jobs;
    const size_t B = jobs->batch, k = jobs->k, m = jobs->n_comms, np = jobs->n_evalpoints, S = MINA_STATES_PER_PROOF;
    std::vector<Section> secs;
    auto add = [&](const void *&slot, size_t bytes) { if (slot && bytes) secs.push_back({&slot, bytes}); };
    if (d.with_states) { add(d.state_records, B * S * MINA_PSTATE_SLOTS * 32); add(d.state_nfields, B * S * 4); add(d.expected_hashes, B * S * 32); add(d.precheck, B); }
    if (d.npub) add(d.public_inputs, B * d.npub * 32);
    mina_kimchi_proofs kd{}; mina_pickles_statements sd{};
    if (d.with_ipa && d.kimchi) {
        kd = *d.kimchi; d.kimchi = &kd;
        kd.public_inputs = nullptr;
        add(kd.prev_chals, B * kd.n_prev * k * 32); add(kd.prev_prechallenges, B * kd.n_prev * k * 16); add(kd.prev_comms, B * kd.n_prev * 64); add(kd.w_comm, B * 15 * 64); add(kd.z_comm, B * 64);
        add(kd.t_comm, B * 7 * 64); add(kd.evals, B * 43 * 64); add(kd.ft_eval1, B * 32);
        if (kd.statements) {
            const void **slots[12]; size_t strides[12];
            mb_pickles_sections(kd.statements, slots, strides, &sd);
            kd.statements = &sd;
            for (int i = 0; i < 12; ++i) add(*slots[i], B * strides[i]);
        }
        d.sponge_state = d.sponge_pos = d.cip = d.evalpoints = d.evalscale = d.polyscale = d.comms = nullptr;
    }
    if (d.with_ipa) {
        add(d.sponge_state, B * 96); add(d.sponge_pos, B * 8); add(d.cip, B * 32); add(d.lr, B * 2 * k * 64); add(d.delta, B * 64); add(d.sg, B * 64);
        add(d.z1, B * 32); add(d.z2, B * 32); add(d.evalpoints, B * np * 32); add(d.evalscale, B * 32); add(d.polyscale, B * 32); add(d.comms, B * m * 64);
        add(d.rand_base, 32); add(d.sg_rand_base, 32);
    }
    if (d.with_accumulator) { add(d.acc_prechallenges, B * d.acc_k * 16); add(d.acc_sg, B * 64); add(d.acc_rho, B * 32); }
    size_t total = 0;
    std::vector<size_t> offs;
    for (auto &s : secs) { offs.push_back(total); total += (s.bytes + 255) & ~(size_t)255; }
    if ((rc = L.host_stage.ensure(total + B * 4))) return rc;
    uint8_t *blob = (uint8_t *)L.host_stage.p;
    for (size_t i = 0; i < secs.size(); ++i) memcpy(blob + offs[i], *secs[i].slot, secs[i].bytes);
    if ((rc = L.st_in.ensure(total))) return rc;
    HIPC(hipMemcpyAsync(L.st_in.p, blob, total, hipMemcpyHostToDevice, L.stream));
    for (size_t i = 0; i < secs.size(); ++i) *secs[i].slot = L.st_in.as<uint8_t>() + offs[i];
    if (d.kimchi) kd.public_inputs = d.public_inputs;
    return state_job_each(c, L, d, verdicts, nullptr);
}

int mb_state_job_each_host(mina_ctx *c, const mina_state_jobs *jobs, uint8_t *verdicts) {
    int rc = check_jobs(c, jobs);
    if (rc) return rc;
    if (!verdicts) return fail(MINA_ERR_ARG, "null argument");
    HIPC(hipSetDevice(c->device));
    c->use_lane0();
    if ((rc = mina_state_jobs_prepare(c, jobs->log2_domain, jobs->npub))) return rc;
    c->use_lane0();
    return state_job_each(c, *c->L, *jobs, verdicts, nullptr);
}

extern "C" int mina_state_job_each_dev(mina_ctx *c, const mina_state_jobs *jobs, void *d_verdicts, void *d_flags) {
    int rc = check_jobs(c, jobs);
    if (rc) return rc;
    if (!d_verdicts) return fail(MINA_ERR_ARG, "null argument");
    if (((uintptr_t)d_verdicts | (uintptr_t)d_flags) & 3u) return fail(MINA_ERR_ARG, "verdicts and flags are 32-bit words: 4-byte alignment");
    if (!c->have_state_salts && jobs->with_states) return fail(MINA_ERR_STATE, "call mina_state_jobs_prepare first");
    HIPC(hipSetDevice(c->device));
    c->next_lane();
    Lane &L = *c->L;
    const size_t B = jobs->batch;
    std::vector<uint8_t> each(B);
    std::vector<uint32_t> words(B + 4);
    if ((rc = state_job_each(c, L, *jobs, each.data(), &words[B]))) { c->L = &L; return rc; }
    c->L = &L;
    for (size_t b = 0; b < B; ++b) words[b] = each[b];
    HIPC(hipMemcpyAsync(d_verdicts, words.data(), B * 4, hipMemcpyHostToDevice, L.stream));
    if (d_flags) HIPC(hipMemcpyAsync(d_flags, &words[B], 16, hipMemcpyHostToDevice, L.stream));
    HIPC(hipStreamSynchronize(L.stream));
    return MINA_OK;
}

extern "C" int mina_ctx_set_search_groups(mina_ctx *c, uint32_t groups) {
    if (!c) return fail(MINA_ERR_ARG, "null argument");
    if (groups == 1 || groups > 128) return fail(MINA_ERR_ARG, "search groups: 0 (off) or 2 .. 128");
    c->search_groups = groups;
    return MINA_OK;
}

extern "C" int mina_ctx_lane_streams(mina_ctx *c, uint32_t *live, uint64_t *made_by_searches) {
    if (!c || !live || !made_by_searches) return fail(MINA_ERR_ARG, "null argument");
    uint32_t n = 0;
    for (int i = 0; i < MB_MAX_LANES; ++i) n += (c->lanes[i].stream ? 1u : 0u) + (c->lanes[i].aux ? 1u : 0u);
    *live = n; *made_by_searches = c->search_streams_made;
    return MINA_OK;
}

extern "C" int mina_ctx_search_stats(mina_ctx *c, uint64_t *searches, uint64_t *rounds, uint64_t *parts) {
    if (!c || !searches || !rounds || !parts) return fail(MINA_ERR_ARG, "null argument");
    *searches = c->gs_searches; *rounds = c->gs_rounds; *parts = c->gs_parts;
    return MINA_OK;
}
```

### mina_bridge_amd/csrc/ctx.h

```cpp
#pragma once
#include <hip/hip_runtime.h>

#include <cstdio>
#include <cstdlib>
#include <cstring>
#include <array>
#include <functional>
#include <memory>
#include <mutex>
#include <thread>
#include <algorithm>
#include <string>
#include <type_traits>
#include <utility>
#include <vector>

#include "../../include/mina_verify.h"
#include "groupmap.cuh"

using namespace mb;

struct mina_ctx;
int mb_ctx_create_view(mina_ctx *parent, mina_ctx **out);
void mb_ctx_refresh_view(mina_ctx *view, mina_ctx *parent);
int mb_fail(int code, const std::string &msg);
mina_verify_tuning mb_tune();
#define fail mb_fail

#define HIPC(expr)                                                                                 \
    do {                                                                                           \
        hipError_t e__ = (expr);                                                                   \
        if (e__ != hipSuccess)                                                                     \
            return fail(MINA_ERR_HIP, std::string(#expr) + ": " + hipGetErrorString(e__));         \
    } while (0)

struct DevBuf {
    void *p = nullptr; size_t cap = 0;
    bool borrowed = false;
    int ensure(size_t bytes) {
        if (bytes <= cap) return MINA_OK;
        if (p) { if (!borrowed && hipFree(p) != hipSuccess) return MINA_ERR_HIP; p = nullptr; cap = 0; borrowed = false; }
        size_t want = bytes + bytes / 8 + 256;
        if (hipMalloc(&p, want) != hipSuccess) return fail(MINA_ERR_HIP, "hipMalloc failed");
        cap = want; return MINA_OK;
    }
    void release() { if (p && !borrowed) (void)hipFree(p); p = nullptr; cap = 0; borrowed = false; }
    void alias(const DevBuf &o) { release(); p = o.p; cap = o.cap; borrowed = o.p != nullptr; }
    template <class T> T *as() { return reinterpret_cast<T *>(p); }
};

struct PinnedBuf {
    void *p = nullptr; size_t cap = 0;
    int ensure(size_t bytes) {
        if (bytes <= cap) return MINA_OK;
        if (p) { (void)hipHostFree(p); p = nullptr; cap = 0; }
        size_t want = bytes + bytes / 4 + 4096;
        if (hipHostMalloc(&p, want, hipHostMallocDefault) != hipSuccess) return fail(MINA_ERR_HIP, "hipHostMalloc failed");
        cap = want; return MINA_OK;
    }
    void release() { if (p) (void)hipHostFree(p); p = nullptr; cap = 0; }
};

struct SrsState {
    uint32_t depth = 0;
    uint32_t c = 16, W = 16;
    DevBuf table;
    DevBuf table29;
    DevBuf table29s;
    DevBuf h;
    int lagrange_log2 = -1;
    std::vector<uint8_t> lagrange_host;
    uint64_t srs_gen = 0;
    DevBuf lagrange_table;
    uint32_t lagrange_table_n = 0;
    int lagrange_table_log2 = -1;
    DevBuf lagrange_digits;
    uint32_t lagrange_digits_n = 0;
    DevBuf lagrange_digits29;
};

struct MsmWorkspace {
    DevBuf scalars, points, points29 , ekey, eval, eoff, count, start, task_start, rem_pos, rem_bucket, info, sorted, partial, heavy, order, redo, ghist, stage, buckets, red_r, red_ws, red2_r, red2_w, set_total, out_words, out_xyzz, buckets29, seg_bad;
};

enum ProfStage : int { PS_DIGITS = 0, PS_SCAN, PS_SCATTER, PS_ACCUMULATE, PS_BUCKET_SUM, PS_REDUCE_A, PS_REDUCE_BC, PS_FINISH,
                       PS_BPOLY_TABLES, PS_BPOLY_FOLD, PS_BPOLY_FINISH, PS_STATE_HASH, PS_IPA_TRANSCRIPT, PS_KIMCHI, PS_PICKLES,
                       PS_STATE_HASH1 , PS_COUNT };
struct ProfState {
    int mask = 0;
    struct Rec { hipEvent_t a, b; int stage; };
    std::vector<Rec> recs; size_t used = 0;
};

struct Lane {
    hipStream_t stream = nullptr;
    hipStream_t aux = nullptr;
    hipEvent_t ev_fork = nullptr, ev_join = nullptr, ev_leg = nullptr;
    MsmWorkspace ws;
    DevBuf tmp_a, tmp_b, tmp_c, tmp_d;
    PinnedBuf host_stage;
    DevBuf bp_ltab, bp_htab, bp_partial, bp_ldig, bp_hdig, bp_colsum;
    DevBuf ipa_chals, ipa_folded, ipa_xyzz_a, ipa_xyzz_b, ipa_points, ipa_scalars, ipa_sigma, ipa_in_a, ipa_in_b, ipa_in_c, ipa_verdict, ipa_xfer, ipa_shared, ipa_shared_off, acc_rho_scaled ;
    DevBuf st_ok, st_hashes, st_pub_xyzz, st_pubcomm, st_flags, st_in, st_verdicts;
    DevBuf dd_rep, dd_uniq, dd_table, dd_counts;
    DevBuf pk_off, pk_len, pk_status, pk_info, pk_fmt;
    DevBuf ac_ws, ac_in;
    DevBuf gs_tab, gs_folded, gs_xa, gs_xb, gs_chals, gs_points, gs_bad, gs_flags;
    DevBuf kc_state, kc_pos, kc_cip, kc_pts, kc_v, kc_u, kc_comms, kc_xfer, kc_pch, pk_xe, pk_pub, pk_ok;
    void release_all() {
        MsmWorkspace &w = ws;
        DevBuf *all[] = {&w.scalars, &w.points, &w.points29, &w.ekey, &w.eval, &w.eoff, &w.count, &w.start, &w.task_start, &w.rem_pos, &w.rem_bucket, &w.info, &w.sorted, &w.partial, &w.heavy, &w.order, &w.redo, &w.ghist, &w.stage,
                         &w.buckets, &w.buckets29, &w.seg_bad, &w.red_r, &w.red_ws, &w.red2_r, &w.red2_w, &w.set_total, &w.out_words, &w.out_xyzz, &tmp_a, &tmp_b, &tmp_c, &tmp_d,
                         &bp_ltab, &bp_htab, &bp_partial, &bp_ldig, &bp_hdig, &bp_colsum, &ipa_chals, &ipa_folded, &ipa_xyzz_a, &ipa_xyzz_b, &ipa_points, &ipa_scalars,
                         &ipa_sigma, &ipa_in_a, &ipa_in_b, &ipa_in_c, &ipa_verdict, &ipa_xfer, &ipa_shared, &ipa_shared_off, &acc_rho_scaled,
                         &st_ok, &st_hashes, &st_pub_xyzz, &st_pubcomm, &st_flags, &st_in, &st_verdicts,
                         &dd_rep, &dd_uniq, &dd_table, &dd_counts, &pk_off, &pk_len, &pk_status, &pk_info, &pk_fmt, &ac_ws, &ac_in,
                         &gs_tab, &gs_folded, &gs_xa, &gs_xb, &gs_chals, &gs_points, &gs_bad, &gs_flags,
                         &kc_state, &kc_pos, &kc_cip, &kc_pts, &kc_v, &kc_u, &kc_comms, &kc_xfer, &kc_pch, &pk_xe, &pk_pub, &pk_ok};
        for (DevBuf *b : all) b->release();
        host_stage.release();
    }
};
static constexpr int MB_PIPE_LANES = 32;
static constexpr int MB_DEV_FORK_MAX = 8;
static constexpr int MB_DEV_HELPER0 = MB_PIPE_LANES + 3 * 16;
static constexpr int MB_MAX_LANES = MB_DEV_HELPER0 + 3 * MB_DEV_FORK_MAX;
enum : int { MB_SALT_PSTATE_BODY = 0, MB_SALT_PSTATE, MB_SALT_ACCOUNT, MB_SALT_ZKAPP_ACCOUNT, MB_SALT_ZKAPP_URI, MB_SALT_SIDE_LOADED_VK, MB_N_PREFIX_SALTS };

struct mina_ctx {
    int device = 0;
    ProfState prof;
    Lane lanes[MB_MAX_LANES];
    int nlanes = 1;
    unsigned rr = 0;
    int pinned = -1;
    Lane *L = nullptr;
    Lane *ipa_rows = nullptr; uint32_t ipa_rows_batch = 0, ipa_rows_k = 0, ipa_rows_per = 0, ipa_rows_nshared = 0; int ipa_rows_curve = -1;
    FieldK fk[2];
    SrsState srs[2];
    DevBuf pparams[2]; bool have_pparams[2] = {false, false};
    DevBuf merkle_salts[2]; uint32_t merkle_depth[2] = {0, 0};
    DevBuf kimchi_index, kimchi_tokens, kimchi_literals; bool have_kimchi = false; uint32_t kimchi_log2 = 0; uint8_t kimchi_digest[32] = {0};
    uint8_t kimchi_comms_host[28 * 64] = {0};
    DevBuf pickles_index, pickles_tokens, pickles_literals; bool have_pickles_dev = false, pickles_ms_valid = false;
    void *step_host = nullptr; void (*step_host_free)(void *) = nullptr;
    bool pparams_surrogate[2] = {false, false};
    bool pparams_rows1[2] = {false, false};
    DevBuf state_salts; bool have_state_salts = false;
    bool is_view = false;
    bool state_dedup = false;
    DevBuf dedup_totals; uint64_t dedup_states = 0;
    int (*state_frontend)(mina_ctx *c, size_t batch, const void *d_blob, size_t blob_len, const void *d_begin, const void *d_end, const void *d_expected_hashes,
                          const void *d_ledger_hashes, const void *d_and, void *d_records, void *d_nfields, void *d_precheck, void *d_masks) = nullptr;
    DevBuf acct_defaults; bool have_acct_defaults = false;
    int (*account_on_device)(mina_ctx *c, size_t n, const uint8_t *const *proofs, const size_t *proof_lens, const uint8_t *const *pubs, const size_t *pub_lens,
                             uint32_t *passed, uint32_t *ran, Lane *lane, std::mutex *enq_mu) = nullptr;
    uint32_t search_groups = 0; uint64_t gs_searches = 0, gs_rounds = 0, gs_parts = 0;
    uint64_t search_streams_made = 0;
    int (*state_job_each)(mina_ctx *c, const mina_state_jobs *dev_jobs, uint8_t *verdicts) = nullptr;
    uint32_t dev_fork_made = 0;
    void use_lane0() { L = &lanes[0]; }
    void next_lane() { L = pinned >= 0 ? &lanes[pinned] : &lanes[rr++ % (unsigned)nlanes]; }
};

static inline int mb_ctx_state_dedup(mina_ctx *c, bool on) {
    if (on && !c->state_dedup) {
        for (int i = 0; i < c->nlanes; ++i) if (c->lanes[i].stream && hipStreamSynchronize(c->lanes[i].stream) != hipSuccess) return MINA_ERR_HIP;
        int rc = c->dedup_totals.ensure(16);
        if (rc) return rc;
        if (hipMemsetAsync(c->dedup_totals.p, 0, 16, c->lanes[0].stream) != hipSuccess || hipStreamSynchronize(c->lanes[0].stream) != hipSuccess) return MINA_ERR_HIP;
        c->dedup_states = 0;
    }
    c->state_dedup = on;
    return MINA_OK;
}

static constexpr size_t COOP8_MAX_GROUPS = 8192;
static inline bool use_coop8(const mina_ctx *c, size_t groups) {
    const mina_verify_tuning t = mb_tune();
    return groups * (size_t)((c && !t.coop8_per_call) ? c->nlanes : 1) <= (size_t)t.coop8_max;
}

static inline bool use_coop16(const mina_ctx *c, size_t proofs) {
    return proofs * (size_t)(c ? c->nlanes : 1) <= (size_t)mb_tune().coop16_max;
}

static inline bool use_coop8_transcripts(const mina_ctx *c, size_t batch, size_t per_call_limit) {
    const size_t lim = (size_t)mb_tune().transcript_coop8_max;
    const size_t in_flight = batch * (size_t)(c ? c->nlanes : 1);
    return lim ? in_flight <= lim : ((batch <= per_call_limit && in_flight <= 2048) || in_flight <= 2560);
}

static constexpr size_t HASH1_MIN_STATES = 65536;
static inline int hash_jobs_in_flight(const mina_ctx *c) { return c->pinned >= 0 ? 1 : c->nlanes; }
static inline bool hash_one_lane(const mina_ctx *c, size_t leg_states) {
    const int jobs = hash_jobs_in_flight(c);
    return c->pparams_rows1[FIELD_FP] && jobs >= 2 && leg_states * (size_t)jobs >= HASH1_MIN_STATES;
}
static inline size_t hash_piece_states(const mina_ctx *c, size_t leg_states, uint32_t piece_waves) { return (size_t)piece_waves * (hash_one_lane(c, leg_states) ? 64u : 21u); }

static inline int hash_lanes(const mina_ctx *c, size_t proofs, size_t sponges) { return use_coop16(c, proofs) ? 16 : (use_coop8(c, sponges) ? 8 : 3); }
static inline int pstate_hash_lanes(const mina_ctx *c, size_t n, size_t leg_states) {
    return hash_one_lane(c, leg_states) ? 1 : hash_lanes(c, (n + MINA_STATES_PER_PROOF - 1) / MINA_STATES_PER_PROOF, n);
}
static inline int transcript_lanes(const mina_ctx *c, size_t batch, size_t per_call_limit) {
    return use_coop16(c, batch) ? 16 : (use_coop8_transcripts(c, batch, per_call_limit) ? 8 : 3);
}
static inline int sponge_batch_lanes(size_t n) { return n <= COOP8_MAX_GROUPS ? 8 : 3; }
static inline int merkle_lanes(const mina_ctx *c, size_t paths) { return use_coop16(c, paths) ? 16 : sponge_batch_lanes(paths); }

enum : uint32_t { MB_JOB_LEGS = 1, MB_JOB_FINISH = 2, MB_JOB_ALL = 3 };
struct StateJobCarry { uint32_t *ipa_v = nullptr, *acc_v = nullptr, *kimchi_bad = nullptr; const uint32_t *stmt_ok = nullptr; };
struct HashLaunch { uint32_t piece_waves = 0, lds_bytes = 0; };
struct FoldExport { uint32_t *ipa_scalars = nullptr, *ipa_point = nullptr, *acc_scalars = nullptr, *acc_point = nullptr; };
struct StateJobPlan {
    Lane *wrap = nullptr, *acc = nullptr, *states = nullptr;
    uint32_t phase = MB_JOB_ALL; StateJobCarry *carry = nullptr;
    uint32_t *d_stmt_out = nullptr;
    size_t hashed_early = 0;
    HashLaunch hash;
    bool acc_first = false;
    const FoldExport *fold_export = nullptr;
};
int mb_state_jobs_on_lane(mina_ctx *c, const mina_state_jobs *j, uint32_t *d_verdicts, uint32_t *d_flags, const StateJobPlan &plan = {});
int mb_verify_account_on(mina_ctx *c, size_t n, const uint8_t *const *proofs, const size_t *proof_lens, const uint8_t *const *pubs, const size_t *pub_lens,
                         uint32_t *passed, uint32_t *ran, Lane *lane, std::mutex *enq_mu);
int mb_state_frontend_on_lane(mina_ctx *c, size_t batch, const void *d_blob, size_t blob_len, const void *d_begin, const void *d_end, const void *d_expected_hashes,
                              const void *d_ledger_hashes, const void *d_and, void *d_records, void *d_nfields, void *d_precheck, void *d_masks);
int mb_verify_account_dev_on(mina_ctx *c, size_t n, const uint8_t *const *proofs, const size_t *proof_lens, const uint8_t *const *pubs, const size_t *pub_lens,
                             uint32_t *passed, uint32_t *ran, Lane *lane, std::mutex *enq_mu);
int mb_state_job_each_host(mina_ctx *c, const mina_state_jobs *dev_jobs, uint8_t *verdicts);
int mb_state_hashes_early(mina_ctx *c, Lane *LS, size_t ns_total, size_t lo, size_t cnt, const uint32_t *d_records, const uint32_t *d_nfields, hipEvent_t after, HashLaunch hash);

struct MbPoolJob;
std::shared_ptr<MbPoolJob> mb_pool_submit(size_t n, std::function<void(size_t)> fn);
void mb_pool_wait(const std::shared_ptr<MbPoolJob> &job);
size_t mb_pool_threads();
template <class Fn> static inline void mb_parallel_for(size_t n, Fn fn) {
    if (n < 128 || mb_pool_threads() <= 1) { for (size_t i = 0; i < n; ++i) fn(i); return; }
    mb_pool_wait(mb_pool_submit(n, std::function<void(size_t)>(fn)));
}
bool mb_secure_random(void *buf, size_t n);

static inline int base_field_of(int curve) { return curve == CURVE_PALLAS ? FIELD_FP : FIELD_FQ; }
static inline int scalar_field_of(int curve) { return curve == CURVE_PALLAS ? FIELD_FQ : FIELD_FP; }
static inline bool bad_field(int f) { return f != 0 && f != 1; }

#define DISPATCH_FIELD(field, ...)                           \
    do { if ((field) == FIELD_FP) { constexpr int F_ = FIELD_FP; __VA_ARGS__; } else { constexpr int F_ = FIELD_FQ; __VA_ARGS__; } } while (0)
#define DISPATCH_CURVE(curve, ...)                           \
    do { if ((curve) == CURVE_PALLAS) { constexpr int C_ = CURVE_PALLAS; __VA_ARGS__; } else { constexpr int C_ = CURVE_VESTA; __VA_ARGS__; } } while (0)

template <int LN, int... FORMS, class Fn> static inline int with_lanes(int lanes, Fn &&f) {
    if (lanes == LN) return f(std::integral_constant<int, LN>{});
    if constexpr (sizeof...(FORMS) > 0) return with_lanes<FORMS...>(lanes, std::forward<Fn>(f));
    else return fail(MINA_ERR_ARG, "no kernel of the " + std::to_string(lanes) + "-lane form at this site");
}

static inline uint32_t cdiv(size_t a, size_t b) { return (uint32_t)((a + b - 1) / b); }


static inline int h2d(mina_ctx *c, DevBuf &b, const void *src, size_t bytes) {
    int rc = b.ensure(bytes ? bytes : 4);
    if (rc) return rc;
    if (bytes) HIPC(hipMemcpyAsync(b.p, src, bytes, hipMemcpyHostToDevice, c->L->stream));
    return MINA_OK;
}
static inline int d2h_sync(mina_ctx *c, void *dst, const DevBuf &b, size_t bytes) {
    if (bytes) HIPC(hipMemcpyAsync(dst, b.p, bytes, hipMemcpyDeviceToHost, c->L->stream));
    HIPC(hipGetLastError());
    HIPC(hipStreamSynchronize(c->L->stream));
    return MINA_OK;
}

static inline bool scalars_below_2_255(const uint8_t *scalars, size_t n) { for (size_t i = 0; i < n; ++i) if (scalars[i * 32 + 31] & 0x80) return false; return true; }

void mb_prof_begin(mina_ctx *c, int stage);
void mb_prof_end(mina_ctx *c, int stage);
struct ProfScope {
    mina_ctx *c; int stage;
    ProfScope(mina_ctx *c_, int s_) : c(c_), stage(s_) { if (c->prof.mask & (1 << stage)) mb_prof_begin(c, stage); }
    ~ProfScope() { if (c->prof.mask & (1 << stage)) mb_prof_end(c, stage); }
};

namespace mb {
struct IpaShape { uint32_t batch, k, npts, ncomms, per; uint32_t override_slot = 0xffffffffu, expand_slot = 0xffffffffu;
                  uint32_t shared_lo = 0, shared_hi = 0, shared_h = 0, shared_expand0 = 0, nshared = 0;
                  uint32_t pow_first = 0; };
static constexpr uint32_t IPA_EXPAND = 8;
struct IpaExpand {
    const affine_t *p0 = nullptr; const uint32_t *pts = nullptr; const fe_t *sc = nullptr; uint32_t stride = 0;
};
struct IpaDevIn {
    const uint32_t *state , *pos , *cip , *lr , *delta , *sg , *z1, *z2 ,
                   *pts , *r , *xi , *comms , *comm_override , *rb , *sb ;
    IpaExpand expand;
};
}
int mb_ipa_batch_check_dev(mina_ctx *c, int curve, mb::IpaShape sh, const mb::IpaDevIn &in, uint32_t *d_verdict , const FoldExport *fx = nullptr);
int mb_ipa_recheck_rows(mina_ctx *c, size_t lo, size_t cnt, uint32_t *d_verdict );
int mb_ipa_recheck_rows_parts(mina_ctx *c, size_t np, const uint32_t *lo, const uint32_t *cnt, uint32_t *d_flags, size_t stage_off );
int mb_accumulator_parts_prepare(mina_ctx *c, int curve, uint32_t k, size_t batch, const uint32_t *d_prechal, const uint32_t *d_sg_words);
int mb_accumulator_check_parts(mina_ctx *c, int curve, uint32_t k, size_t batch, const uint32_t *d_rho, size_t np, const uint32_t *lo, const uint32_t *cnt, uint32_t *d_flags, size_t stage_off);
size_t mb_search_parts_cap(mina_ctx *c, int curve, uint32_t k);
int mb_accumulator_check_dev(mina_ctx *c, int curve, uint32_t k, size_t batch, const uint32_t *d_prechal, const uint32_t *d_sg_words, const uint32_t *d_rho, uint32_t *d_verdict, const FoldExport *fx = nullptr);

struct xyzz_dev;
int mb_msm_fixed(mina_ctx *c, int curve, uint32_t n, const uint32_t *d_scalars, uint32_t *d_out_words, void *d_out_xyzz, uint32_t first = 0);
int mb_msm_table(mina_ctx *c, int curve, const void *d_table, uint32_t stride, uint32_t cbits, uint32_t W, uint32_t first, uint32_t n,
                 uint32_t nprob, const uint32_t *d_scalars, uint32_t *d_out_words, void *d_out_xyzz);
int mb_bpoly_single_from_prechallenges(mina_ctx *c, int field, uint32_t k, const uint32_t *d_prechal, uint32_t *d_out, uint32_t count);
int mb_bpoly_fold(mina_ctx *c, int field, uint32_t k, size_t batch, const uint32_t *d_chals, const uint32_t *d_weights, uint32_t *d_out);
int mb_msm_variable(mina_ctx *c, int curve, uint32_t n, const uint32_t *d_scalars, const void *d_points_mont,
                    uint32_t *d_out_words, void *d_out_xyzz);
int mb_read_segments(mina_ctx *c, size_t nseg, const void *d_begin, const void *d_end, size_t limit, uint32_t *max_len);
bool mb_msm_segments_fit(uint32_t max_len, size_t nseg);
int mb_msm_segments(mina_ctx *c, int curve, uint32_t n_total, size_t nseg, uint32_t max_len, const uint32_t *d_begin, const uint32_t *d_end,
                    const uint32_t *d_scalars, const void *d_points_mont, uint32_t *d_out_words, void *d_out_xyzz);
int mb_bpoly_fold_segments(mina_ctx *c, int field, uint32_t k, size_t batch, size_t nseg, uint32_t max_len, const uint32_t *d_begin, const uint32_t *d_end,
                           const uint32_t *d_chals, const uint32_t *d_weights, uint32_t *d_out);
```

### mina_bridge_amd/lib.py

```python
from __future__ import annotations

import ctypes
import os

import numpy as np

HERE = os.path.dirname(os.path.abspath(__file__))
LIB_PATH = os.path.join(HERE, "libminaverify.so")

FIELD_FP, FIELD_FQ = 0, 1
CURVE_PALLAS, CURVE_VESTA = 0, 1

EXPORTS = [
    "mina_ctx_create", "mina_ctx_destroy", "mina_last_error", "mina_ctx_synchronize", "mina_ctx_stream", "mina_ctx_pin_lane", "mina_ctx_set_pipeline", "mina_prof_enable", "mina_prof_read",
    "mina_dev_malloc", "mina_dev_free", "mina_dev_upload", "mina_dev_download",
    "mina_srs_create", "mina_srs_split_table", "mina_srs_load", "mina_srs_depth", "mina_srs_get_g", "mina_srs_get_h", "mina_srs_lagrange_basis", "mina_public_input_commitment", "mina_public_input_commitment_batch", "mina_combined_inner_product", "mina_srs_serialize",
    "mina_msm", "mina_msm_srs", "mina_msm_srs_range", "mina_msm_srs_multi", "mina_msm_srs_dev",
    "mina_b_poly", "mina_b_poly_coefficients", "mina_b_poly_fold", "mina_b_poly_fold_dev",
    "mina_poseidon_set_params", "mina_poseidon_params_parse", "mina_poseidon_load_params", "mina_poseidon_load_params_file", "mina_poseidon_permute", "mina_poseidon_permute_dev", "mina_poseidon_hash",
    "mina_challenge_to_field", "mina_fq_sponge_run", "mina_to_group", "mina_merkle_roots", "mina_merkle_verify_batch",
    "mina_field_mul", "mina_field_inv", "mina_field_sqrt", "mina_selftest_group_law", "mina_selftest_fe29", "mina_selftest_fe32",
    "mina_accumulator_check_batch", "mina_accumulator_check_dev", "mina_accumulator_check_multi_dev", "mina_accumulator_check_multi", "mina_ipa_batch_check",
    "mina_consensus_project_window", "mina_consensus_relative_min_window_density", "mina_consensus_is_short_range",
    "mina_protocol_state_pack", "mina_protocol_state_hash_batch", "mina_protocol_state_hash_bytes",
    "mina_protocol_state_dedup_dev", "mina_protocol_state_hash_batch_dedup", "mina_ctx_set_state_dedup", "mina_ctx_state_dedup_stats",
    "mina_protocol_state_pack_dev", "mina_state_frontend_dev", "mina_account_frontend_dev", "mina_account_job_dev",
    "mina_state_jobs_prepare", "mina_state_job_batch_dev", "mina_state_job_batch", "mina_state_job_fold_dev",
    "mina_challenge_to_field_dev", "mina_field_sum_rows_dev", "mina_msm_srs_range_dev", "mina_msm_dev", "mina_points_sum_dev", "mina_point_records_equal_dev",
    "mina_msm_segments_dev", "mina_b_poly_fold_segments_dev", "mina_state_job_each_dev", "mina_ctx_set_search_groups", "mina_ctx_search_stats", "mina_ctx_lane_streams",
    "mina_step_index_install", "mina_step_index_load_json", "mina_polish_tokens_from_json", "mina_verifier_index_load_json", "mina_pickles_public_input",
    "mina_verifier_index_install", "mina_verifier_index_digest", "mina_kimchi_to_batch", "mina_pickles_public_inputs_batch", "mina_wrap_proof_flatten", "mina_state_proof_split",
    "mina_verify_state", "mina_verify_state_batch", "mina_verify_state_checks", "mina_verify_state_files", "mina_verify_account", "mina_verify_account_batch",
    "mina_verify_account_files", "mina_verify_account_checks", "mina_verify_account_ctx", "mina_account_hash_batch", "mina_account_abi_encode", "mina_verify_configure", "mina_verify_shutdown", "mina_verify_global_ctx", "mina_poseidon_params_name",
    "mina_verify_device_count", "mina_verify_device_ctx", "mina_verify_set_network", "mina_verify_install_verifier_index", "mina_verify_install_step_index", "mina_verify_set_poseidon_params",
    "mina_poseidon_install_default_params",
    "verify_mina_state_ffi", "verify_account_inclusion_ffi", "verify_mina_state_ffi_u32", "verify_account_inclusion_ffi_u32",
    "mina_verify_tuning_default", "mina_verify_tuning_get", "mina_verify_configure_ex", "mina_verify_retired_env",
    "mina_consensus_select_secure_chain", "mina_parse_state_pub_inputs", "mina_parse_account_pub_inputs", "mina_parse_merkle_path", "mina_verify_account_inclusion",
]


class MinaError(RuntimeError):
    pass


class StatePubInputs(ctypes.Structure):
    _fields_ = [("is_state_proof_from_devnet", ctypes.c_uint8), ("bridge_tip_state_hash", ctypes.c_uint8 * 32),
                ("candidate_chain_state_hashes", (ctypes.c_uint8 * 32) * 16), ("candidate_chain_ledger_hashes", (ctypes.c_uint8 * 32) * 16)]


def combined_inner_product(field: int, evals, polyscale, evalscale, n_polys: int, n_points: int) -> np.ndarray:
    lib = load_library()
    ev = _u8(evals) if n_polys * n_points else np.zeros(32, np.uint8)
    out = np.empty(32, np.uint8)
    rc = lib.mina_combined_inner_product(field, ctypes.c_size_t(n_polys), ctypes.c_size_t(n_points), _p(ev), _p(_u8(polyscale)), _p(_u8(evalscale)), _p(out))
    if rc != 0:
        raise MinaError(f"mina_combined_inner_product failed ({rc}): {lib.mina_last_error().decode()}")
    return out


def parse_state_pub_inputs(data: bytes) -> dict:
    lib = load_library()
    out = StatePubInputs()
    b = _u8(data) if len(data) else np.zeros(1, np.uint8)
    rc = lib.mina_parse_state_pub_inputs(_p(b), ctypes.c_size_t(len(data)), ctypes.byref(out))
    if rc != 0:
        raise MinaError(f"mina_parse_state_pub_inputs failed ({rc}): {lib.mina_last_error().decode()}")
    return {"is_state_proof_from_devnet": bool(out.is_state_proof_from_devnet), "bridge_tip_state_hash": bytes(out.bridge_tip_state_hash),
            "candidate_chain_state_hashes": [bytes(h) for h in out.candidate_chain_state_hashes],
            "candidate_chain_ledger_hashes": [bytes(h) for h in out.candidate_chain_ledger_hashes]}


def parse_account_pub_inputs(data: bytes):
    lib = load_library()
    b = _u8(data) if len(data) else np.zeros(1, np.uint8)
    lh = np.empty(32, np.uint8); off = ctypes.c_size_t(0); ln = ctypes.c_size_t(0)
    rc = lib.mina_parse_account_pub_inputs(_p(b), ctypes.c_size_t(len(data)), _p(lh), ctypes.byref(off), ctypes.byref(ln))
    if rc != 0:
        raise MinaError(f"mina_parse_account_pub_inputs failed ({rc}): {lib.mina_last_error().decode()}")
    return lh.tobytes(), data[off.value: off.value + ln.value]


def parse_merkle_path(proof: bytes, max_depth: int = 64):
    lib = load_library()
    b = _u8(proof) if len(proof) else np.zeros(1, np.uint8)
    sib = np.empty(max_depth * 32, np.uint8); dirs = np.empty(max_depth, np.uint8)
    depth = ctypes.c_uint32(0); off = ctypes.c_size_t(0)
    rc = lib.mina_parse_merkle_path(_p(b), ctypes.c_size_t(len(proof)), ctypes.c_uint32(max_depth), _p(sib), _p(dirs), ctypes.byref(depth), ctypes.byref(off))
    if rc != 0:
        raise MinaError(f"mina_parse_merkle_path failed ({rc}): {lib.mina_last_error().decode()}")
    d = depth.value
    return sib[: d * 32].reshape(d, 32).copy(), dirs[:d].copy(), off.value


class ConsensusParams(ctypes.Structure):
    _fields_ = [("slots_per_sub_window", ctypes.c_uint32), ("sub_windows_per_window", ctypes.c_uint32)]


class ConsensusState(ctypes.Structure):
    _fields_ = [("blockchain_length", ctypes.c_uint32), ("epoch_count", ctypes.c_uint32), ("curr_global_slot", ctypes.c_uint32),
                ("min_window_density", ctypes.c_uint32), ("sub_window_densities", ctypes.c_uint32 * 16),
                ("staking_lock_checkpoint", ctypes.c_uint8 * 32), ("next_lock_checkpoint", ctypes.c_uint8 * 32),
                ("last_vrf_output_hash", ctypes.c_uint8 * 32), ("state_hash", ctypes.c_uint8 * 32)]

    @classmethod
    def make(cls, length, epoch, slot, min_density, window, staking_cp=b"", next_cp=b"", vrf=b"", state_hash=b""):
        s = cls()
        s.blockchain_length, s.epoch_count, s.curr_global_slot, s.min_window_density = length, epoch, slot, min_density
        for i, d in enumerate(window):
            s.sub_window_densities[i] = d
        for name, val in (("staking_lock_checkpoint", staking_cp), ("next_lock_checkpoint", next_cp), ("last_vrf_output_hash", vrf), ("state_hash", state_hash)):
            buf = bytes(val).ljust(32, b"\0")[:32]
            ctypes.memmove(getattr(s, name), buf, 32)
        return s


MAINNET_CONSENSUS = ConsensusParams(7, 11)


def consensus_project_window(state, next_slot, params=MAINNET_CONSENSUS):
    lib = load_library()
    out = (ctypes.c_uint32 * 16)()
    rc = lib.mina_consensus_project_window(ctypes.byref(params), ctypes.byref(state), ctypes.c_uint32(next_slot), out)
    if rc != 0:
        raise MinaError(f"mina_consensus_project_window failed ({rc}): {lib.mina_last_error().decode()}")
    return list(out)[: params.sub_windows_per_window]


def consensus_relative_min_window_density(a, b, params=MAINNET_CONSENSUS) -> int:
    lib = load_library()
    out = ctypes.c_uint32(0)
    rc = lib.mina_consensus_relative_min_window_density(ctypes.byref(params), ctypes.byref(a), ctypes.byref(b), ctypes.byref(out))
    if rc != 0:
        raise MinaError(f"mina_consensus_relative_min_window_density failed ({rc}): {lib.mina_last_error().decode()}")
    return out.value


def consensus_is_short_range(a, b) -> bool:
    return bool(load_library().mina_consensus_is_short_range(ctypes.byref(a), ctypes.byref(b)))


def consensus_select_secure_chain(tip, candidate, params=MAINNET_CONSENSUS) -> bool:
    lib = load_library()
    out = ctypes.c_int(0)
    rc = lib.mina_consensus_select_secure_chain(ctypes.byref(params), ctypes.byref(tip), ctypes.byref(candidate), ctypes.byref(out))
    if rc != 0:
        raise MinaError(f"mina_consensus_select_secure_chain failed ({rc}): {lib.mina_last_error().decode()}")
    return bool(out.value)


class IpaOpening(ctypes.Structure):
    _fields_ = [
        ("k", ctypes.c_uint32),
        ("lr", ctypes.c_void_p), ("delta", ctypes.c_void_p), ("sg", ctypes.c_void_p),
        ("z1", ctypes.c_void_p), ("z2", ctypes.c_void_p),
        ("n_evalpoints", ctypes.c_uint32), ("evalpoints", ctypes.c_void_p),
        ("n_comms", ctypes.c_uint32), ("comms", ctypes.c_void_p),
        ("combined_inner_product", ctypes.c_void_p), ("polyscale", ctypes.c_void_p), ("evalscale", ctypes.c_void_p),
        ("sponge_state", ctypes.c_void_p), ("sponge_mode", ctypes.c_uint32), ("sponge_count", ctypes.c_uint32),
    ]


PSTATE_SLOTS, STATES_PER_PROOF = 64, 17
ENC_BINPROT, ENC_BINCODE = 0, 1


class ProtocolStateInfo(ctypes.Structure):
    _fields_ = [("previous_state_hash", ctypes.c_uint8 * 32), ("genesis_state_hash", ctypes.c_uint8 * 32), ("snarked_ledger_hash", ctypes.c_uint8 * 32),
                ("n_body_fields", ctypes.c_uint32), ("k", ctypes.c_uint32), ("slots_per_epoch", ctypes.c_uint32), ("slots_per_sub_window", ctypes.c_uint32),
                ("sub_windows_per_window", ctypes.c_uint32), ("grace_period_slots", ctypes.c_uint32), ("delta", ctypes.c_uint32),
                ("consensus", ConsensusState)]


class StateJobs(ctypes.Structure):
    _fields_ = [
        ("batch", ctypes.c_size_t),
        ("with_states", ctypes.c_int), ("state_records", ctypes.c_void_p), ("state_nfields", ctypes.c_void_p), ("expected_hashes", ctypes.c_void_p),
        ("precheck", ctypes.c_void_p),
        ("log2_domain", ctypes.c_uint32), ("npub", ctypes.c_uint32), ("pub_comm_slot", ctypes.c_uint32), ("public_inputs", ctypes.c_void_p),
        ("with_ipa", ctypes.c_int), ("k", ctypes.c_uint32), ("n_evalpoints", ctypes.c_uint32), ("n_comms", ctypes.c_uint32),
        ("sponge_state", ctypes.c_void_p), ("sponge_pos", ctypes.c_void_p), ("cip", ctypes.c_void_p), ("lr", ctypes.c_void_p), ("delta", ctypes.c_void_p),
        ("sg", ctypes.c_void_p), ("z1", ctypes.c_void_p), ("z2", ctypes.c_void_p), ("evalpoints", ctypes.c_void_p), ("evalscale", ctypes.c_void_p),
# ... 712 lines not shown

    @staticmethod
    def pack_ipa_openings(openings: list):
        keep = []
        arr = (IpaOpening * len(openings))()

        def ptr(x):
            a = _u8(x)
            keep.append(a)
            return a.ctypes.data

        for i, o in enumerate(openings):
            e = arr[i]
            e.k = int(o["k"])
            e.lr, e.delta, e.sg = ptr(o["lr"]), ptr(o["delta"]), ptr(o["sg"])
            e.z1, e.z2 = ptr(o["z1"]), ptr(o["z2"])
            e.n_evalpoints = int(o["n_evalpoints"])
            e.evalpoints = ptr(o["evalpoints"])
            e.n_comms = int(o["n_comms"])
            e.comms = ptr(o["comms"])
            e.combined_inner_product = ptr(o["combined_inner_product"])
            e.polyscale, e.evalscale = ptr(o["polyscale"]), ptr(o["evalscale"])
            e.sponge_state = ptr(o["sponge_state"])
            e.sponge_mode, e.sponge_count = int(o["sponge_mode"]), int(o["sponge_count"])
        return arr, keep

    def ipa_batch_check(self, curve: int, openings, rand_base, sg_rand_base) -> bool:
        arr, keep = openings if isinstance(openings, tuple) else self.pack_ipa_openings(openings)
        rb, sb = _u8(rand_base), _u8(sg_rand_base)
        v = np.zeros(1, np.uint8)
        self._ck(self._lib.mina_ipa_batch_check(self._h, curve, ctypes.c_size_t(len(arr)), arr, _p(rb), _p(sb), _p(v)), "mina_ipa_batch_check")
        return bool(v[0])

    def protocol_state_hash_batch(self, records, nfields, want_body: bool = False):
        rec = _u8(records); nf = np.ascontiguousarray(nfields, dtype=np.uint32)
        n = nf.size
        assert rec.size == n * PSTATE_SLOTS * 32
        out = np.empty((n, 32), np.uint8); body = np.empty((n, 32), np.uint8) if want_body else None
        self._ck(self._lib.mina_protocol_state_hash_batch(self._h, ctypes.c_size_t(n), _p(rec), nf.ctypes.data_as(ctypes.c_void_p), _p(out), _p(body)),
                 "mina_protocol_state_hash_batch")
        return (out, body) if want_body else out

    def protocol_state_hash_batch_dedup(self, records, nfields, want_body: bool = False):
        rec = _u8(records); nf = np.ascontiguousarray(nfields, dtype=np.uint32)
        n = nf.size
        assert rec.size == n * PSTATE_SLOTS * 32
        out = np.empty((n, 32), np.uint8); body = np.empty((n, 32), np.uint8) if want_body else None
        m = ctypes.c_size_t(0)
        self._ck(self._lib.mina_protocol_state_hash_batch_dedup(self._h, ctypes.c_size_t(n), _p(rec), nf.ctypes.data_as(ctypes.c_void_p), _p(out), _p(body), ctypes.byref(m)),
                 "mina_protocol_state_hash_batch_dedup")
        return (out, body, int(m.value)) if want_body else (out, int(m.value))

    def protocol_state_dedup_dev(self, n: int, d_records: int, d_nfields: int, d_rep: int, d_counts: int, fingerprint_bits: int = 0):
        self._ck(self._lib.mina_protocol_state_dedup_dev(self._h, ctypes.c_size_t(n), ctypes.c_void_p(d_records), ctypes.c_void_p(d_nfields), ctypes.c_void_p(d_rep),
                                                         ctypes.c_void_p(d_counts), ctypes.c_uint32(fingerprint_bits)), "mina_protocol_state_dedup_dev")

    def protocol_state_pack_dev(self, n: int, d_blob: int, blob_len: int, d_off: int, d_len: int, d_records: int, d_nfields: int, d_info: int, d_status: int):
        self._ck(self._lib.mina_protocol_state_pack_dev(self._h, ctypes.c_size_t(n), ctypes.c_void_p(d_blob), ctypes.c_size_t(blob_len), ctypes.c_void_p(d_off), ctypes.c_void_p(d_len),
                                                        ctypes.c_void_p(d_records), ctypes.c_void_p(d_nfields), ctypes.c_void_p(d_info or None), ctypes.c_void_p(d_status)),
                 "mina_protocol_state_pack_dev")

    def state_frontend_dev(self, batch: int, d_blob: int, blob_len: int, d_begin: int, d_end: int, d_expected_hashes: int, d_ledger_hashes: int, d_and: int,
                           d_records: int, d_nfields: int, d_precheck: int, d_masks: int = 0):
        self._ck(self._lib.mina_state_frontend_dev(self._h, ctypes.c_size_t(batch), ctypes.c_void_p(d_blob), ctypes.c_size_t(blob_len), ctypes.c_void_p(d_begin), ctypes.c_void_p(d_end),
                                                   ctypes.c_void_p(d_expected_hashes), ctypes.c_void_p(d_ledger_hashes), ctypes.c_void_p(d_and or None), ctypes.c_void_p(d_records),
                                                   ctypes.c_void_p(d_nfields), ctypes.c_void_p(d_precheck), ctypes.c_void_p(d_masks or None)), "mina_state_frontend_dev")

    def set_state_dedup(self, on: bool = True):
        self._ck(self._lib.mina_ctx_set_state_dedup(self._h, 1 if on else 0), "mina_ctx_set_state_dedup")

    def state_dedup_stats(self):
        from collections import namedtuple
        a, b, c_ = ctypes.c_uint64(0), ctypes.c_uint64(0), ctypes.c_uint64(0)
        self._ck(self._lib.mina_ctx_state_dedup_stats(self._h, ctypes.byref(a), ctypes.byref(b), ctypes.byref(c_)), "mina_ctx_state_dedup_stats")
        return namedtuple("StateDedupStats", "states distinct collisions")(int(a.value), int(b.value), int(c_.value))

    def protocol_state_hash_bytes(self, states: list, encoding: int = ENC_BINPROT) -> np.ndarray:
        n = len(states)
        arrs = [_u8(s) for s in states]
        PP = (ctypes.c_void_p * n)(*[a.ctypes.data for a in arrs]); PL = (ctypes.c_size_t * n)(*[len(s) for s in states])
        out = np.empty((n, 32), np.uint8)
        self._ck(self._lib.mina_protocol_state_hash_bytes(self._h, int(encoding), ctypes.c_size_t(n), PP, PL, _p(out)), "mina_protocol_state_hash_bytes")
        return out

    def account_hash_batch(self, accounts: list, encoding: int = ENC_BINPROT) -> np.ndarray:
        n = len(accounts)
        arrs, PP, PL = _ptr_arrays(accounts)
        out = np.empty((n, 32), np.uint8)
        self._ck(self._lib.mina_account_hash_batch(self._h, int(encoding), ctypes.c_size_t(n), PP, PL, _p(out)), "mina_account_hash_batch")
        return out

    def account_frontend_dev(self, n: int, d_blob: int, blob_len: int, d_proof_off: int, d_proof_len: int, d_pub_off: int, d_pub_len: int, d_records: int, d_nfields: int,
                             d_salt_idx: int, d_siblings: int, d_dirs: int, d_depths: int, d_ledger_hashes: int, d_zk_marks: int, d_zk_index: int, d_zk_count: int, d_bits: int):
        v = ctypes.c_void_p
        self._ck(self._lib.mina_account_frontend_dev(self._h, ctypes.c_size_t(n), v(d_blob), ctypes.c_size_t(blob_len), v(d_proof_off), v(d_proof_len), v(d_pub_off), v(d_pub_len),
                                                     v(d_records), v(d_nfields), v(d_salt_idx), v(d_siblings), v(d_dirs), v(d_depths), v(d_ledger_hashes), v(d_zk_marks), v(d_zk_index),
                                                     v(d_zk_count), v(d_bits)), "mina_account_frontend_dev")

    def account_job_dev(self, n: int, d_blob: int, blob_len: int, d_proof_off: int, d_proof_len: int, d_pub_off: int, d_pub_len: int, d_passed: int, d_ran: int,
                        d_account_hashes: int = 0, d_roots: int = 0):
        v = ctypes.c_void_p
        self._ck(self._lib.mina_account_job_dev(self._h, ctypes.c_size_t(n), v(d_blob), ctypes.c_size_t(blob_len), v(d_proof_off), v(d_proof_len), v(d_pub_off), v(d_pub_len),
                                                v(d_passed), v(d_ran), v(d_account_hashes or None), v(d_roots or None)), "mina_account_job_dev")

    def verify_account_checks(self, proofs: list, pubs: list):
        n = len(proofs)
        pa, PP, PL = _ptr_arrays(proofs); qa, QQ, QL = _ptr_arrays(pubs)
        passed = np.zeros(n, np.uint32); ran = np.zeros(n, np.uint32)
        self._ck(self._lib.mina_verify_account_ctx(self._h, ctypes.c_size_t(n), PP, PL, QQ, QL, passed.ctypes.data_as(ctypes.c_void_p), ran.ctypes.data_as(ctypes.c_void_p)),
                 "mina_verify_account_ctx")
        return passed, ran

    def challenge_to_field_dev(self, field: int, n: int, d_chal: int, d_out: int):
        self._ck(self._lib.mina_challenge_to_field_dev(self._h, field, ctypes.c_size_t(n), ctypes.c_void_p(d_chal), ctypes.c_void_p(d_out)), "mina_challenge_to_field_dev")

    def field_sum_rows_dev(self, field: int, rows: int, m: int, d_in: int, d_out: int):
        self._ck(self._lib.mina_field_sum_rows_dev(self._h, field, ctypes.c_size_t(rows), ctypes.c_size_t(m), ctypes.c_void_p(d_in), ctypes.c_void_p(d_out)), "mina_field_sum_rows_dev")

    def msm_srs_range_dev(self, curve: int, first: int, n: int, d_scalars: int, d_out: int):
        self._ck(self._lib.mina_msm_srs_range_dev(self._h, curve, ctypes.c_uint32(first), ctypes.c_size_t(n), ctypes.c_void_p(d_scalars), ctypes.c_void_p(d_out)), "mina_msm_srs_range_dev")

    def msm_dev(self, curve: int, n: int, d_bases: int, d_scalars: int, d_out: int):
        self._ck(self._lib.mina_msm_dev(self._h, curve, ctypes.c_size_t(n), ctypes.c_void_p(d_bases), ctypes.c_void_p(d_scalars), ctypes.c_void_p(d_out)), "mina_msm_dev")

    def points_sum_dev(self, curve: int, n: int, d_records: int, d_out: int):
        self._ck(self._lib.mina_points_sum_dev(self._h, curve, ctypes.c_size_t(n), ctypes.c_void_p(d_records), ctypes.c_void_p(d_out)), "mina_points_sum_dev")

    def point_records_equal_dev(self, d_a: int, d_b: int, d_verdict: int):
        self._ck(self._lib.mina_point_records_equal_dev(self._h, ctypes.c_void_p(d_a), ctypes.c_void_p(d_b), ctypes.c_void_p(d_verdict)), "mina_point_records_equal_dev")

    def msm_segments_dev(self, curve: int, n_total: int, nseg: int, d_seg_begin: int, d_seg_end: int, d_bases: int, d_scalars: int, d_out: int):
        v = ctypes.c_void_p
        self._ck(self._lib.mina_msm_segments_dev(self._h, curve, ctypes.c_size_t(n_total), ctypes.c_size_t(nseg), v(d_seg_begin), v(d_seg_end), v(d_bases or None),
                                                 v(d_scalars or None), v(d_out)), "mina_msm_segments_dev")

    def b_poly_fold_segments_dev(self, field: int, k: int, batch: int, nseg: int, d_seg_begin: int, d_seg_end: int, d_chals: int, d_weights: int, d_out: int):
        v = ctypes.c_void_p
        self._ck(self._lib.mina_b_poly_fold_segments_dev(self._h, field, ctypes.c_uint32(k), ctypes.c_size_t(batch), ctypes.c_size_t(nseg), v(d_seg_begin), v(d_seg_end),
                                                         v(d_chals), v(d_weights or None), v(d_out)), "mina_b_poly_fold_segments_dev")

    def set_search_groups(self, groups: int):
        self._ck(self._lib.mina_ctx_set_search_groups(self._h, ctypes.c_uint32(groups)), "mina_ctx_set_search_groups")

    def search_stats(self) -> dict:
        a, b, c = ctypes.c_uint64(0), ctypes.c_uint64(0), ctypes.c_uint64(0)
        self._ck(self._lib.mina_ctx_search_stats(self._h, ctypes.byref(a), ctypes.byref(b), ctypes.byref(c)), "mina_ctx_search_stats")
        return {"searches": a.value, "rounds": b.value, "parts": c.value}

    def lane_streams(self) -> dict:
        a, b = ctypes.c_uint32(0), ctypes.c_uint64(0)
        self._ck(self._lib.mina_ctx_lane_streams(self._h, ctypes.byref(a), ctypes.byref(b)), "mina_ctx_lane_streams")
        return {"live": a.value, "made_by_searches": b.value}

    def state_job_each_dev(self, jobs, d_verdicts: int, d_flags: int = 0):
        self._ck(self._lib.mina_state_job_each_dev(self._h, ctypes.byref(jobs), ctypes.c_void_p(d_verdicts), ctypes.c_void_p(d_flags or None)), "mina_state_job_each_dev")

    def state_jobs_prepare(self, log2_domain: int, npub: int):
        self._ck(self._lib.mina_state_jobs_prepare(self._h, ctypes.c_uint32(log2_domain), ctypes.c_uint32(npub)), "mina_state_jobs_prepare")

    @staticmethod
    def make_state_jobs(batch: int, arrays: dict, **scalars):
        j = StateJobs(); keep = []
        j.batch = batch
        kimchi = scalars.pop("kimchi", None)
        if kimchi is not None:
            j.kimchi = ctypes.addressof(kimchi[0]); keep.append(kimchi)
        for name, val in scalars.items():
            setattr(j, name, val)
        for name in StateJobs.POINTER_FIELDS:
            a = arrays.get(name)
            if a is None:
                continue
            a = np.ascontiguousarray(a); keep.append(a)
            setattr(j, name, a.ctypes.data)
        return j, keep

    @staticmethod
    def make_kimchi_proofs(batch: int, n_prev: int, npub: int, arrays: dict, statements=None):
        kp = KimchiProofs(); keep = []
        kp.batch, kp.n_prev, kp.npub = batch, n_prev, npub
        for name in KimchiProofs.POINTER_FIELDS:
            a = arrays.get(name)
            if a is None:
                continue
            a = np.ascontiguousarray(a); keep.append(a)
            setattr(kp, name, a.ctypes.data)
        if statements is not None:
            st, skeep = statements
            kp.statements = ctypes.addressof(st); keep.append((st, skeep))
        return kp, keep

    @staticmethod
    def make_pickles_statements(n_old: int, n_evals: int, arrays: dict):
        st = PicklesStatements(); keep = []
        st.n_old, st.n_evals = n_old, n_evals
        for name in PicklesStatements.POINTER_FIELDS:
            a = arrays.get(name)
            if a is None:
                continue
            if isinstance(a, int):
                setattr(st, name, a); continue
            a = np.ascontiguousarray(a); keep.append(a)
            setattr(st, name, a.ctypes.data)
        return st, keep

    def pickles_public_inputs_batch(self, statements, batch: int):
        st, _keep = statements
        pub = np.zeros((batch, 40, 32), np.uint8); ok = np.zeros(batch, np.uint8)
        self._ck(self._lib.mina_pickles_public_inputs_batch(self._h, ctypes.byref(st), ctypes.c_size_t(batch), _p(pub), _p(ok)), "mina_pickles_public_inputs_batch")
        return pub, ok

    @staticmethod
    def _verifier_index_struct(log2_domain: int, zk_rows: int, perm_alpha_offset: int, shifts, sigma_comm, coefficients_comm, selector_comm, constant_term: bytes):
        vi = VerifierIndex(); arrs = [_u8(shifts), _u8(sigma_comm), _u8(coefficients_comm), _u8(selector_comm), _u8(constant_term) if len(constant_term) else np.zeros(1, np.uint8)]
        vi.log2_domain, vi.zk_rows, vi.perm_alpha_offset = log2_domain, zk_rows, perm_alpha_offset
        vi.shifts, vi.sigma_comm, vi.coefficients_comm, vi.selector_comm, vi.constant_term = (a.ctypes.data for a in arrs)
        vi.constant_term_len = len(constant_term)
        return vi, arrs

    def verifier_index_install(self, *a):
        vi, keep = self._verifier_index_struct(*a)
        self._ck(self._lib.mina_verifier_index_install(self._h, ctypes.byref(vi)), "mina_verifier_index_install")

    @staticmethod
    def _step_index_struct(zk_rows: int, domains: list, shifts, constant_term: bytes):
        class StepIndex(ctypes.Structure):
            _fields_ = [("zk_rows", ctypes.c_uint32), ("n_domains", ctypes.c_uint32), ("domain_log2", ctypes.c_void_p), ("shifts", ctypes.c_void_p),
                        ("constant_term", ctypes.c_void_p), ("constant_term_len", ctypes.c_size_t)]
        d = np.ascontiguousarray(domains, dtype=np.uint32); sh = _u8(shifts); ct = _u8(constant_term) if len(constant_term) else np.zeros(1, np.uint8)
        return StepIndex(zk_rows, len(domains), d.ctypes.data, sh.ctypes.data, ct.ctypes.data, len(constant_term)), (d, sh, ct)

    def step_index_install(self, *a):
        si, keep = self._step_index_struct(*a)
        self._ck(self._lib.mina_step_index_install(self._h, ctypes.byref(si)), "mina_step_index_install")

    def verifier_index_load_json(self, index_json: str, constant_term_json: str, perm_alpha_offset: int = 21):
        a, b = index_json.encode(), constant_term_json.encode()
        self._ck(self._lib.mina_verifier_index_load_json(self._h, ctypes.c_char_p(a), ctypes.c_size_t(len(a)), ctypes.c_char_p(b), ctypes.c_size_t(len(b)), ctypes.c_uint32(perm_alpha_offset)),
                 "mina_verifier_index_load_json")

    def step_index_load_json(self, index_jsons: list, constant_term_json: str, enabled_features: int = 0, optional_present: int = 0):
        enc = [j.encode() for j in index_jsons]; ct = constant_term_json.encode()
        arr = (ctypes.c_char_p * len(enc))(*enc); lens = (ctypes.c_size_t * len(enc))(*map(len, enc))
        self._ck(self._lib.mina_step_index_load_json(self._h, ctypes.c_size_t(len(enc)), arr, lens, ctypes.c_char_p(ct), ctypes.c_size_t(len(ct)), ctypes.c_uint32(enabled_features),
                                                     ctypes.c_uint32(optional_present)), "mina_step_index_load_json")

    def poseidon_load_params(self, field: int, text: str):
        t = text.encode()
        self._ck(self._lib.mina_poseidon_load_params(self._h, int(field), ctypes.c_char_p(t), ctypes.c_size_t(len(t))), "mina_poseidon_load_params")

    def pickles_public_input(self, wrap_proof: bytes, encoding: int, app_state):
        b = _u8(wrap_proof); a = _u8(app_state)
        pub = np.zeros((40, 32), np.uint8); der = np.zeros((7, 32), np.uint8)
        self._ck(self._lib.mina_pickles_public_input(self._h, _p(b), ctypes.c_size_t(len(wrap_proof)), int(encoding), _p(a), _p(pub), _p(der)), "mina_pickles_public_input")
        return pub, der

    def verifier_index_digest(self) -> np.ndarray:
        out = np.empty(32, np.uint8)
        self._ck(self._lib.mina_verifier_index_digest(self._h, _p(out)), "mina_verifier_index_digest")
        return out

    def kimchi_to_batch(self, kimchi, k: int) -> dict:
        kp, keep = kimchi
        B, nc = kp.batch, kp.n_prev + 45
        o = {"sponge_state": np.zeros((B, 96), np.uint8), "sponge_pos": np.zeros((B, 2), np.uint32), "cip": np.zeros((B, 32), np.uint8),
             "evalpoints": np.zeros((B, 64), np.uint8), "polyscale": np.zeros((B, 32), np.uint8), "evalscale": np.zeros((B, 32), np.uint8),
             "comms": np.zeros((B, nc, 64), np.uint8), "ft_eval0": np.zeros((B, 32), np.uint8), "malformed": np.zeros(1, np.uint8)}
        out = KimchiBatchOut()
        for name in o:
            setattr(out, name, o[name].ctypes.data)
        self._ck(self._lib.mina_kimchi_to_batch(self._h, ctypes.byref(kp), ctypes.byref(out)), "mina_kimchi_to_batch")
        return o

    def state_job_batch(self, jobs) -> np.ndarray:
        j, keep = jobs
        out = np.zeros(j.batch, np.uint8)
        self._ck(self._lib.mina_state_job_batch(self._h, ctypes.byref(j), _p(out)), "mina_state_job_batch")
        return out

    def state_jobs_to_device(self, jobs):
        j, keep = jobs
        d = StateJobs(); ptrs = []
        ctypes.memmove(ctypes.byref(d), ctypes.byref(j), ctypes.sizeof(StateJobs))
        flat = []
        for x in keep:
            flat.extend(x[1] if isinstance(x, tuple) else [x])
        by_addr = {a.ctypes.data: a for a in flat}

        def up(addr):
            a = by_addr[addr]
            p = self.dev_malloc(max(a.nbytes, 4)); ptrs.append(p)
            self.dev_upload(p, a.view(np.uint8).reshape(-1))
            return p

        for name in StateJobs.POINTER_FIELDS:
            addr = getattr(j, name)
            if addr:
                setattr(d, name, up(addr))
        if j.kimchi:
            src = ctypes.cast(j.kimchi, ctypes.POINTER(KimchiProofs)).contents
            dk = KimchiProofs()
            ctypes.memmove(ctypes.byref(dk), ctypes.byref(src), ctypes.sizeof(KimchiProofs))
            for name in KimchiProofs.POINTER_FIELDS:
                addr = getattr(src, name)
                if addr:
                    setattr(dk, name, d.public_inputs if name == "public_inputs" and j.public_inputs == addr else up(addr))
# ... 13 lines not shown
```

Before: 280,900.

## Fit device-fork helper streams to hardware queue budget via shared role streams

Adds a stream budget, taken from GPU_MAX_HW_QUEUES (default 4, less one) or set through a new API. When the in-flight lanes times three helper streams would exceed that budget, whole state jobs run on a small shared set of role streams (hash, two wrap/accumulator streams) instead of per-lane helper streams. The aim is to avoid oversubscribing hardware queues, which would otherwise multiplex streams and serialize work. The trade-off is extra event chaining between lanes and less per-lane concurrency, and per-lane hash piece splitting is disabled in role mode.

```diff
diff --git a/bindings/go/minaverify.go b/bindings/go/minaverify.go
--- a/bindings/go/minaverify.go
+++ b/bindings/go/minaverify.go
@@ -57,6 +57,13 @@
 
 func (c *Ctx) SetSearchGroups(groups uint32) error {
 	if rc := C.mina_ctx_set_search_groups(c.p, C.uint32_t(groups)); rc != 0 {
+		return lastError()
+	}
+	return nil
+}
+
+func (c *Ctx) SetStreamBudget(n int) error {
+	if rc := C.mina_ctx_set_stream_budget(c.p, C.int(n)); rc != 0 {
 		return lastError()
 	}
 	return nil
diff --git a/bindings/rust/src/sys.rs b/bindings/rust/src/sys.rs
--- a/bindings/rust/src/sys.rs
+++ b/bindings/rust/src/sys.rs
@@ -301,6 +301,7 @@
     pub fn mina_ctx_set_search_groups(ctx: *mut mina_ctx, groups: u32) -> c_int;
     pub fn mina_ctx_search_stats(ctx: *mut mina_ctx, searches: *mut u64, rounds: *mut u64, parts: *mut u64) -> c_int;
     pub fn mina_ctx_lane_streams(ctx: *mut mina_ctx, live: *mut u32, made_by_searches: *mut u64) -> c_int;
+    pub fn mina_ctx_set_stream_budget(ctx: *mut mina_ctx, n: c_int) -> c_int;
     pub fn mina_challenge_to_field_dev(ctx: *mut mina_ctx, field: c_int, n: usize, d_chal128: *const c_void, d_out: *mut c_void) -> c_int;
     pub fn mina_field_sum_rows_dev(ctx: *mut mina_ctx, field: c_int, rows: usize, m: usize, d_in: *const c_void, d_out: *mut c_void) -> c_int;
     pub fn mina_msm_srs_range_dev(ctx: *mut mina_ctx, curve: c_int, first: u32, n: usize, d_scalars: *const c_void, d_out: *mut c_void) -> c_int;
diff --git a/include/mina_verify.h b/include/mina_verify.h
--- a/include/mina_verify.h
+++ b/include/mina_verify.h
@@ -305,6 +305,7 @@
 int mina_ctx_set_search_groups(mina_ctx *ctx, uint32_t groups);
 int mina_ctx_search_stats(mina_ctx *ctx, uint64_t *searches, uint64_t *rounds, uint64_t *parts);
 int mina_ctx_lane_streams(mina_ctx *ctx, uint32_t *live, uint64_t *made_by_searches);
+int mina_ctx_set_stream_budget(mina_ctx *ctx, int n);
 
 int mina_challenge_to_field_dev(mina_ctx *ctx, int field, size_t n, const void *d_chal128 , void *d_out );
 int mina_field_sum_rows_dev(mina_ctx *ctx, int field, size_t rows, size_t m, const void *d_in , void *d_out );
diff --git a/mina_bridge_amd/csrc/api_core.hip b/mina_bridge_amd/csrc/api_core.hip
--- a/mina_bridge_amd/csrc/api_core.hip
+++ b/mina_bridge_amd/csrc/api_core.hip
@@ -96,7 +96,9 @@
 extern "C" void mina_ctx_destroy(mina_ctx *c) {
     if (!c) return;
     (void)hipSetDevice(c->device);
-    for (int i = 0; i < MB_MAX_LANES; ++i) if (c->lanes[i].stream) (void)hipStreamSynchronize(c->lanes[i].stream);
+    for (int i = 0; i < MB_DEV_HELPER0; ++i) if (c->lanes[i].stream) (void)hipStreamSynchronize(c->lanes[i].stream);
+    for (hipStream_t s : c->fork_own) if (s) (void)hipStreamSynchronize(s);
+    for (hipStream_t s : c->role) if (s) (void)hipStreamSynchronize(s);
     for (int i = 0; i < 2; ++i) { c->srs[i].table.release(); c->srs[i].table29.release(); c->srs[i].table29s.release(); c->srs[i].h.release(); c->srs[i].lagrange_table.release(); c->srs[i].lagrange_digits.release(); c->srs[i].lagrange_digits29.release(); c->pparams[i].release(); c->merkle_salts[i].release(); }
     c->state_salts.release(); c->acct_defaults.release(); c->dedup_totals.release(); c->kimchi_index.release(); c->kimchi_tokens.release(); c->kimchi_literals.release();
     c->pickles_index.release(); c->pickles_tokens.release(); c->pickles_literals.release();
@@ -108,8 +110,11 @@
         Lane &L = c->lanes[i];
         if (L.aux) { (void)hipStreamSynchronize(L.aux); (void)hipStreamDestroy(L.aux); (void)hipEventDestroy(L.ev_fork); (void)hipEventDestroy(L.ev_join); }
         if (L.ev_leg) (void)hipEventDestroy(L.ev_leg);
-        if (L.stream) (void)hipStreamDestroy(L.stream);
-    }
+        if (L.ev_done) (void)hipEventDestroy(L.ev_done);
+        if (L.stream && i < MB_DEV_HELPER0) (void)hipStreamDestroy(L.stream);
+    }
+    for (hipStream_t s : c->fork_own) if (s) (void)hipStreamDestroy(s);
+    for (hipStream_t s : c->role) if (s) (void)hipStreamDestroy(s);
     delete c;
 }
 
@@ -118,7 +123,15 @@
 extern "C" int mina_ctx_synchronize(mina_ctx *c) {
     if (!c) return fail(MINA_ERR_ARG, "null ctx");
     HIPC(hipSetDevice(c->device));
-    for (int i = 0; i < c->nlanes; ++i) HIPC(hipStreamSynchronize(c->lanes[i].stream));
+    HIPC(mb_ctx_wait_all(c));
+    return MINA_OK;
+}
+extern "C" int mina_ctx_set_stream_budget(mina_ctx *c, int n) {
+    if (!c) return fail(MINA_ERR_ARG, "null ctx");
+    if (n > 31) return fail(MINA_ERR_ARG, "stream budget: at most 31 (32 hardware queues less the null stream's); <= 0 = the environment's");
+    HIPC(hipSetDevice(c->device));
+    HIPC(mb_ctx_wait_all(c));
+    c->stream_budget = n > 0 ? n : 0;
     return MINA_OK;
 }
 extern "C" void *mina_ctx_stream(mina_ctx *c) { return c ? (void *)c->lanes[c->pinned >= 0 ? c->pinned : 0].stream : nullptr; }
@@ -133,7 +146,7 @@
     if (!c) return fail(MINA_ERR_ARG, "null ctx");
     if (lanes < 1 || lanes > MB_PIPE_LANES) return fail(MINA_ERR_ARG, "lanes must be in 1..32");
     HIPC(hipSetDevice(c->device));
-    for (int i = 0; i < c->nlanes; ++i) HIPC(hipStreamSynchronize(c->lanes[i].stream));
+    HIPC(mb_ctx_wait_all(c));
     for (int i = 0; i < lanes; ++i)
         if (!c->lanes[i].stream) HIPC(hipStreamCreateWithFlags(&c->lanes[i].stream, hipStreamNonBlocking));
     c->nlanes = lanes; c->rr = 0; c->pinned = -1; c->use_lane0();
@@ -222,7 +235,7 @@
 extern "C" int mina_prof_read(mina_ctx *c, char *buf, size_t cap) {
     if (!c || !buf || cap < 8) return fail(MINA_ERR_ARG, "bad argument");
     HIPC(hipSetDevice(c->device));
-    for (int i = 0; i < c->nlanes; ++i) HIPC(hipStreamSynchronize(c->lanes[i].stream));
+    HIPC(mb_ctx_wait_all(c));
     double tot[PS_COUNT] = {0}; int cnt[PS_COUNT] = {0};
     for (size_t i = 0; i < c->prof.used; ++i) {
         float ms = 0;
diff --git a/mina_bridge_amd/csrc/api_srs.hip b/mina_bridge_amd/csrc/api_srs.hip
--- a/mina_bridge_amd/csrc/api_srs.hip
+++ b/mina_bridge_amd/csrc/api_srs.hip
@@ -22,7 +22,7 @@
     SrsState &s = c->srs[curve];
     if (s.depth == 0) return fail(MINA_ERR_STATE, "SRS not loaded for this curve");
     HIPC(hipSetDevice(c->device));
-    for (int i = 0; i < c->nlanes; ++i) HIPC(hipStreamSynchronize(c->lanes[i].stream));
+    HIPC(mb_ctx_wait_all(c));
     if (!on) { s.table29s.release(); return MINA_OK; }
     if (s.table29s.p) return MINA_OK;
     c->use_lane0();
diff --git a/mina_bridge_amd/csrc/api_state.hip b/mina_bridge_amd/csrc/api_state.hip
--- a/mina_bridge_amd/csrc/api_state.hip
+++ b/mina_bridge_amd/csrc/api_state.hip
@@ -503,10 +503,18 @@
     return mb_accumulator_check_dev(c, CURVE_VESTA, j->acc_k, B, (const uint32_t *)j->acc_prechallenges, (const uint32_t *)j->acc_sg, B > 1 ? (const uint32_t *)j->acc_rho : nullptr, v.acc_v, fx);
 }
 
-static int wrap_leg(mina_ctx *c, const mina_state_jobs *j, Lane &L, const FoldExport *fx, StateJobCarry &v) {
+static int wrap_leg(mina_ctx *c, const mina_state_jobs *j, Lane &L, const FoldExport *fx, StateJobCarry &v, hipStream_t stage2 = nullptr) {
     c->L = &L;
     const size_t B = j->batch;
     int rc;
+    auto to_stage2 = [&]() -> int {
+        if (!stage2 || stage2 == L.stream) return MINA_OK;
+        if (!L.ev_leg) HIPC(hipEventCreateWithFlags(&L.ev_leg, hipEventDisableTiming));
+        HIPC(hipEventRecord(L.ev_leg, L.stream));
+        HIPC(hipStreamWaitEvent(stage2, L.ev_leg, 0));
+        L.stream = stage2;
+        return MINA_OK;
+    };
     if ((rc = L.st_flags.ensure(16 * 4))) return rc;
     const uint32_t *pub = (const uint32_t *)j->public_inputs, *comm_override = nullptr;
     if (j->kimchi && j->kimchi->statements) {
@@ -519,7 +527,7 @@
         if ((rc = mb_pubcomm_dev(c, B, j->log2_domain, j->npub, pub, L.st_pubcomm.as<uint32_t>()))) return rc;
         comm_override = L.st_pubcomm.as<uint32_t>();
     }
-    if (!j->with_ipa) return MINA_OK;
+    if (!j->with_ipa) return to_stage2();
     mb::IpaShape sh; sh.batch = (uint32_t)B; sh.k = j->k; sh.npts = j->n_evalpoints; sh.ncomms = j->n_comms; sh.per = 2 * j->k + j->n_comms + 4;
     auto W = [](const void *p) { return (const uint32_t *)p; };
     v.ipa_v = L.st_flags.as<uint32_t>() + 4;
@@ -527,6 +535,7 @@
         sh.override_slot = j->npub ? j->pub_comm_slot : 0xffffffffu;
         mb::IpaDevIn in{W(j->sponge_state), W(j->sponge_pos), W(j->cip), W(j->lr), W(j->delta), W(j->sg), W(j->z1), W(j->z2), W(j->evalpoints), W(j->evalscale),
                         W(j->polyscale), W(j->comms), comm_override, W(j->rand_base), W(j->sg_rand_base)};
+        if ((rc = to_stage2())) return rc;
         return mb_ipa_batch_check_dev(c, CURVE_PALLAS, sh, in, v.ipa_v, fx);
     }
     const mina_kimchi_proofs &kp = *j->kimchi;
@@ -560,7 +569,36 @@
     mb::IpaDevIn iin{out.sponge_state, out.sponge_pos, out.cip, W(j->lr), W(j->delta), W(j->sg), W(j->z1), W(j->z2), out.evalpoints, out.evalscale, out.polyscale,
                      out.comms, nullptr, W(j->rand_base), W(j->sg_rand_base)};
     iin.expand = ex;
+    if ((rc = to_stage2())) return rc;
     return mb_ipa_batch_check_dev(c, CURVE_PALLAS, sh, iin, v.ipa_v, fx);
+}
+
+static int state_job_on_roles(mina_ctx *c, const mina_state_jobs *j, uint32_t *d_verdicts, uint32_t *d_flags, const StateJobPlan &plan, Lane &L0) {
+    Lane &LI = *plan.wrap, &LA = *plan.acc, &LS = *plan.states;
+    const hipStream_t H = plan.role_h, W1 = plan.role_w1, W2 = plan.role_w2;
+    int rc;
+    if (!L0.ev_done) HIPC(hipEventCreateWithFlags(&L0.ev_done, hipEventDisableTiming));
+    if (!L0.on_roles) {
+        HIPC(hipEventRecord(L0.ev_done, L0.stream));
+        L0.on_roles = true;
+    }
+    for (hipStream_t s : {H, W1, W2}) HIPC(hipStreamWaitEvent(s, L0.ev_done, 0));
+    LS.stream = H; LI.stream = W1; LA.stream = W2;
+    const size_t B = j->batch;
+    StateJobCarry v;
+    if ((rc = LS.st_ok.ensure(B * 4))) return rc;
+    if ((rc = state_leg(c, j, LS, plan))) return rc;
+    if ((rc = accumulator_leg(c, j, LA, plan.fold_export, v))) return rc;
+    if ((rc = wrap_leg(c, j, LI, plan.fold_export, v, W2))) return rc;
+    if (H != W2) {
+        if (!LS.ev_leg) HIPC(hipEventCreateWithFlags(&LS.ev_leg, hipEventDisableTiming));
+        HIPC(hipEventRecord(LS.ev_leg, H));
+        HIPC(hipStreamWaitEvent(W2, LS.ev_leg, 0));
+    }
+    mb::state_job_verdict_kernel<<<cdiv(B, 64), 64, 0, W2>>>((uint32_t)B, LS.st_ok.as<uint32_t>(), v.ipa_v, v.acc_v, v.kimchi_bad, v.stmt_ok, d_verdicts, d_flags, plan.d_stmt_out);
+    HIPC(hipGetLastError());
+    HIPC(hipEventRecord(L0.ev_done, W2));
+    return MINA_OK;
 }
 
 int mb_state_jobs_on_lane(mina_ctx *c, const mina_state_jobs *j, uint32_t *d_verdicts, uint32_t *d_flags, const StateJobPlan &plan) {
@@ -570,6 +608,11 @@
     struct Restore { mina_ctx *c; Lane *l0; ~Restore() { c->L = l0; } } restore{c, L0};
     Lane *LI = L0, *LA = L0, *LS = L0;
     int rc;
+    if (plan.role_h) {
+        if (phase != MB_JOB_ALL || !plan.role_w1 || !plan.role_w2 || !plan.wrap || !plan.acc || !plan.states || plan.wrap == plan.acc || plan.wrap == plan.states || plan.acc == plan.states ||
+            plan.wrap == L0 || plan.acc == L0 || plan.states == L0) return fail(MINA_ERR_ARG, "the role plan queues whole jobs on three helper lanes");
+        return state_job_on_roles(c, j, d_verdicts, d_flags, plan, *L0);
+    }
     if (plan.wrap && plan.acc && plan.wrap != L0 && plan.acc != L0 && plan.wrap != plan.acc) {
         LI = plan.wrap; LA = plan.acc;
         if (plan.states && plan.states != L0 && plan.states != LI) LS = plan.states;
@@ -601,30 +644,47 @@
     if (!(tu.dev_fork & 1u) || c->nlanes > MB_DEV_FORK_MAX || li < 0 || li >= MB_DEV_FORK_MAX) return MINA_OK;
     const int in_flight = c->pinned >= 0 ? 1 : c->nlanes;
     Lane *h = &c->lanes[MB_DEV_HELPER0 + 3 * li];
-    if (!h[0].stream || !h[1].stream || !h[2].stream) {
-        const uint32_t mode = c->dev_fork_made ? c->dev_fork_made : tu.dev_fork;
-        c->dev_fork_made = mode;
+    Lane &L0 = *c->L;
+    if (c->stream_budget_env < 0) c->stream_budget_env = env_stream_budget();
+    const StreamPlan sp = stream_plan(in_flight, c->stream_budget > 0 ? c->stream_budget : c->stream_budget_env);
+    const uint32_t mode = c->dev_fork_made ? c->dev_fork_made : tu.dev_fork;
+    c->dev_fork_made = mode;
+    int prio_lo = 0, prio_hi = 0;
+    auto make = [&](hipStream_t &st, bool chain, bool masked, int prio) -> int {
+        if (st) return MINA_OK;
         int ncu = 0; (void)hipDeviceGetAttribute(&ncu, hipDeviceAttributeMultiprocessorCount, c->device);
-        int prio_lo = 0, prio_hi = 0; (void)hipDeviceGetStreamPriorityRange(&prio_lo, &prio_hi);
-        auto make = [&](Lane &ln, bool chain, bool masked, int prio) -> int {
-            if (ln.stream) return MINA_OK;
-            if (masked && tu.dev_chain_cus > 0 && tu.dev_chain_cus < (uint32_t)ncu && ncu <= 256) {
-                uint32_t mk[8] = {0, 0, 0, 0, 0, 0, 0, 0};
-                for (uint32_t b2 = 0; b2 < (uint32_t)ncu; ++b2) if ((b2 < tu.dev_chain_cus) == chain) mk[b2 >> 5] |= 1u << (b2 & 31);
-                if (hipExtStreamCreateWithCUMask(&ln.stream, 8, mk) == hipSuccess) return MINA_OK;
-                (void)hipGetLastError(); ln.stream = nullptr;
-            }
-            if (prio_lo != prio_hi && (mode & 4u)) HIPC(hipStreamCreateWithPriority(&ln.stream, hipStreamNonBlocking, prio));
-            else HIPC(hipStreamCreateWithFlags(&ln.stream, hipStreamNonBlocking));
-            return MINA_OK;
-        };
-        int rc;
-        if ((rc = make(h[0], true, (mode & 2u) != 0, prio_hi)) || (rc = make(h[1], true, false, (prio_lo + prio_hi) / 2)) || (rc = make(h[2], false, (mode & 2u) != 0, prio_lo))) return rc;
-    }
-    plan.wrap = &h[0]; plan.acc = tu.dev_acc_lane ? &h[2] : &h[1]; plan.states = &h[2];
-    plan.acc_first = tu.dev_acc_lane == 2;
+        if (masked && tu.dev_chain_cus > 0 && tu.dev_chain_cus < (uint32_t)ncu && ncu <= 256) {
+            uint32_t mk[8] = {0, 0, 0, 0, 0, 0, 0, 0};
+            for (uint32_t b2 = 0; b2 < (uint32_t)ncu; ++b2) if ((b2 < tu.dev_chain_cus) == chain) mk[b2 >> 5] |= 1u << (b2 & 31);
+            if (hipExtStreamCreateWithCUMask(&st, 8, mk) == hipSuccess) return MINA_OK;
+            (void)hipGetLastError(); st = nullptr;
+        }
+        if (prio_lo != prio_hi && (mode & 4u)) HIPC(hipStreamCreateWithPriority(&st, hipStreamNonBlocking, prio));
+        else HIPC(hipStreamCreateWithFlags(&st, hipStreamNonBlocking));
+        return MINA_OK;
+    };
+    int rc;
+    if (sp.roles) {
+        if (!c->role[sp.streams - 1]) (void)hipDeviceGetStreamPriorityRange(&prio_lo, &prio_hi);
+        for (int i = 0; i < sp.streams; ++i) if ((rc = make(c->role[i], true, false, (i == 0 && sp.streams > 1) ? prio_lo : prio_hi))) return rc;
+        plan.role_h = c->role[0]; plan.role_w1 = c->role[sp.w1(li)]; plan.role_w2 = c->role[sp.w2(li)];
+        plan.wrap = &h[0]; plan.acc = &h[1]; plan.states = &h[2];
+    } else {
+        hipStream_t *own = &c->fork_own[3 * li];
+        if (!own[0] || !own[1] || !own[2]) {
+            (void)hipDeviceGetStreamPriorityRange(&prio_lo, &prio_hi);
+            if ((rc = make(own[0], true, (mode & 2u) != 0, prio_hi)) || (rc = make(own[1], true, false, (prio_lo + prio_hi) / 2)) || (rc = make(own[2], false, (mode & 2u) != 0, prio_lo))) return rc;
+        }
+        for (int q = 0; q < 3; ++q) h[q].stream = own[q];
+        if (L0.on_roles) {
+            HIPC(hipStreamWaitEvent(L0.stream, L0.ev_done, 0));
+            L0.on_roles = false;
+        }
+        plan.wrap = &h[0]; plan.acc = tu.dev_acc_lane ? &h[2] : &h[1]; plan.states = &h[2];
+        plan.acc_first = tu.dev_acc_lane == 2;
+    }
     uint32_t piece = tu.dev_piece_waves;
-    if (piece == 0 && in_flight >= 2) piece = (hash_one_lane(c, leg_states) ? 12288u : 6144u) / (uint32_t)in_flight;
+    if (piece == 0 && in_flight >= 2 && !sp.roles) piece = (hash_one_lane(c, leg_states) ? 12288u : 6144u) / (uint32_t)in_flight;
     if (piece == 0xffffffffu) piece = 0;
     plan.hash.piece_waves = piece;
     uint32_t lds_kb = tu.dev_hash_lds_kb;
@@ -891,7 +951,9 @@
 extern "C" int mina_ctx_lane_streams(mina_ctx *c, uint32_t *live, uint64_t *made_by_searches) {
     if (!c || !live || !made_by_searches) return fail(MINA_ERR_ARG, "null argument");
     uint32_t n = 0;
-    for (int i = 0; i < MB_MAX_LANES; ++i) n += (c->lanes[i].stream ? 1u : 0u) + (c->lanes[i].aux ? 1u : 0u);
+    for (int i = 0; i < MB_MAX_LANES; ++i) n += ((c->lanes[i].stream && i < MB_DEV_HELPER0) ? 1u : 0u) + (c->lanes[i].aux ? 1u : 0u);
+    for (hipStream_t s : c->fork_own) n += s ? 1u : 0u;
+    for (hipStream_t s : c->role) n += s ? 1u : 0u;
     *live = n; *made_by_searches = c->search_streams_made;
     return MINA_OK;
 }
diff --git a/mina_bridge_amd/csrc/ctx.h b/mina_bridge_amd/csrc/ctx.h
--- a/mina_bridge_amd/csrc/ctx.h
+++ b/mina_bridge_amd/csrc/ctx.h
@@ -96,6 +96,7 @@
     hipStream_t stream = nullptr;
     hipStream_t aux = nullptr;
     hipEvent_t ev_fork = nullptr, ev_join = nullptr, ev_leg = nullptr;
+    hipEvent_t ev_done = nullptr; bool on_roles = false;
     MsmWorkspace ws;
     DevBuf tmp_a, tmp_b, tmp_c, tmp_d;
     PinnedBuf host_stage;
@@ -121,8 +122,27 @@
         host_stage.release();
     }
 };
+struct StreamPlan {
+    bool roles = false; int sets = 0, streams = 0;
+    int w1(int lane) const { return streams >= 3 ? 1 + 2 * (lane % sets) : streams - 1; }
+    int w2(int lane) const { return streams >= 3 ? 2 + 2 * (lane % sets) : streams - 1; }
+};
+static inline StreamPlan stream_plan(int lanes_in_flight, int budget) {
+    StreamPlan p;
+    if (lanes_in_flight <= 1 || 4 * lanes_in_flight <= budget) return p;
+    p.roles = true;
+    p.sets = std::min(std::max((budget - 1) / 2, 1), lanes_in_flight);
+    p.streams = std::min(1 + 2 * p.sets, std::max(budget, 1));
+    return p;
+}
+static inline int env_stream_budget() {
+    const char *e = getenv("GPU_MAX_HW_QUEUES");
+    const long q = e ? strtol(e, nullptr, 10) : 4;
+    return (int)std::min(std::max(q, 1L), 32L) - 1;
+}
 static constexpr int MB_PIPE_LANES = 32;
 static constexpr int MB_DEV_FORK_MAX = 8;
+static constexpr int MB_ROLE_STREAMS = 1 + 2 * MB_DEV_FORK_MAX;
 static constexpr int MB_DEV_HELPER0 = MB_PIPE_LANES + 3 * 16;
 static constexpr int MB_MAX_LANES = MB_DEV_HELPER0 + 3 * MB_DEV_FORK_MAX;
 enum : int { MB_SALT_PSTATE_BODY = 0, MB_SALT_PSTATE, MB_SALT_ACCOUNT, MB_SALT_ZKAPP_ACCOUNT, MB_SALT_ZKAPP_URI, MB_SALT_SIDE_LOADED_VK, MB_N_PREFIX_SALTS };
@@ -159,13 +179,21 @@
     uint64_t search_streams_made = 0;
     int (*state_job_each)(mina_ctx *c, const mina_state_jobs *dev_jobs, uint8_t *verdicts) = nullptr;
     uint32_t dev_fork_made = 0;
+    hipStream_t fork_own[3 * MB_DEV_FORK_MAX] = {}; hipStream_t role[MB_ROLE_STREAMS] = {};
+    int stream_budget = 0, stream_budget_env = -1;
     void use_lane0() { L = &lanes[0]; }
     void next_lane() { L = pinned >= 0 ? &lanes[pinned] : &lanes[rr++ % (unsigned)nlanes]; }
 };
 
+static inline hipError_t mb_ctx_wait_all(mina_ctx *c) {
+    for (int i = 0; i < c->nlanes; ++i) if (c->lanes[i].stream) { hipError_t e = hipStreamSynchronize(c->lanes[i].stream); if (e != hipSuccess) return e; }
+    for (hipStream_t s : c->role) if (s) { hipError_t e = hipStreamSynchronize(s); if (e != hipSuccess) return e; }
+    return hipSuccess;
+}
+
 static inline int mb_ctx_state_dedup(mina_ctx *c, bool on) {
     if (on && !c->state_dedup) {
-        for (int i = 0; i < c->nlanes; ++i) if (c->lanes[i].stream && hipStreamSynchronize(c->lanes[i].stream) != hipSuccess) return MINA_ERR_HIP;
+        if (mb_ctx_wait_all(c) != hipSuccess) return MINA_ERR_HIP;
         int rc = c->dedup_totals.ensure(16);
         if (rc) return rc;
         if (hipMemsetAsync(c->dedup_totals.p, 0, 16, c->lanes[0].stream) != hipSuccess || hipStreamSynchronize(c->lanes[0].stream) != hipSuccess) return MINA_ERR_HIP;
@@ -220,6 +248,7 @@
     size_t hashed_early = 0;
     HashLaunch hash;
     bool acc_first = false;
+    hipStream_t role_h = nullptr, role_w1 = nullptr, role_w2 = nullptr;
     const FoldExport *fold_export = nullptr;
 };
 int mb_state_jobs_on_lane(mina_ctx *c, const mina_state_jobs *j, uint32_t *d_verdicts, uint32_t *d_flags, const StateJobPlan &plan = {});
diff --git a/mina_bridge_amd/lib.py b/mina_bridge_amd/lib.py
--- a/mina_bridge_amd/lib.py
+++ b/mina_bridge_amd/lib.py
@@ -27,7 +27,7 @@
     "mina_protocol_state_pack_dev", "mina_state_frontend_dev", "mina_account_frontend_dev", "mina_account_job_dev",
     "mina_state_jobs_prepare", "mina_state_job_batch_dev", "mina_state_job_batch", "mina_state_job_fold_dev",
     "mina_challenge_to_field_dev", "mina_field_sum_rows_dev", "mina_msm_srs_range_dev", "mina_msm_dev", "mina_points_sum_dev", "mina_point_records_equal_dev",
-    "mina_msm_segments_dev", "mina_b_poly_fold_segments_dev", "mina_state_job_each_dev", "mina_ctx_set_search_groups", "mina_ctx_search_stats", "mina_ctx_lane_streams",
+    "mina_msm_segments_dev", "mina_b_poly_fold_segments_dev", "mina_state_job_each_dev", "mina_ctx_set_search_groups", "mina_ctx_search_stats", "mina_ctx_lane_streams", "mina_ctx_set_stream_budget",
     "mina_step_index_install", "mina_step_index_load_json", "mina_polish_tokens_from_json", "mina_verifier_index_load_json", "mina_pickles_public_input",
     "mina_verifier_index_install", "mina_verifier_index_digest", "mina_kimchi_to_batch", "mina_pickles_public_inputs_batch", "mina_wrap_proof_flatten", "mina_state_proof_split",
     "mina_verify_state", "mina_verify_state_batch", "mina_verify_state_checks", "mina_verify_state_files", "mina_verify_account", "mina_verify_account_batch",
@@ -1046,6 +1046,9 @@
         self._ck(self._lib.mina_ctx_lane_streams(self._h, ctypes.byref(a), ctypes.byref(b)), "mina_ctx_lane_streams")
         return {"live": a.value, "made_by_searches": b.value}
 
+    def set_stream_budget(self, n: int):
+        self._ck(self._lib.mina_ctx_set_stream_budget(self._h, ctypes.c_int(n)), "mina_ctx_set_stream_budget")
+
     def state_job_each_dev(self, jobs, d_verdicts: int, d_flags: int = 0):
         self._ck(self._lib.mina_state_job_each_dev(self._h, ctypes.byref(jobs), ctypes.c_void_p(d_verdicts), ctypes.c_void_p(d_flags or None)), "mina_state_job_each_dev")
 
```

After: 288,200, median of 6. 1.03x the previous value.
